# goalheart/ionic-mpnn

Hardware: AMD Instinct MI355X
Metric: molecule-graph pairs/sec (fwd), batch 4096 per MI355X (higher is better)
Workload: dtype f32 (bf16x9 emulation)

## Files before the change

### ionic_mpnn_amd/csrc/common.h

```cpp
#pragma once

#include <hip/hip_runtime.h>

#include <cstdarg>
#include <cstdint>
#include <cstdio>

#include "../../include/impnn.h"

namespace impnn {

char* error_buffer();
int fail(int code, const char* fmt, ...);

inline hipStream_t as_stream(impnn_stream_t s) { return reinterpret_cast<hipStream_t>(s); }

inline int check_launch(const char* what) {
  hipError_t e = hipGetLastError();
  if (e != hipSuccess) return fail(IMPNN_E_LAUNCH, "%s: %s", what, hipGetErrorString(e));
  return IMPNN_OK;
}

inline bool aligned16(const void* p) { return (reinterpret_cast<uintptr_t>(p) & 15u) == 0; }

// ... 92 lines not shown
struct GatedUpdateCall {
  const char* entry;
  GatedUpdateForm form;
  const float *h, *agg, *Wz, *bz, *Wr, *br, *Wh, *bh, *gamma;
  const float* beta;
  float eps;
  float* out;
  const float* dout;
  float *dh, *dagg, *dparams, *workspace;
  int64_t workspace_floats;
  bool accumulate;
  const int32_t *row_index, *n_rows;
  int64_t rows;
  int D;
  float* saved;
  bool dropout;
  DropoutArgs drop;
  hipStream_t stream;
};

template <class F>
int with_dropout_pack(const GatedUpdateCall& c, F&& f) {
  return c.dropout ? f(c.drop) : f();
}

constexpr int kMaxTypes = 4096;
struct TypedMessageCall {
  const char* entry;
  const float* h;
  const int32_t *bond_ids, *conn;
  const float* type_mats;
  float* messages;
  const float* grad;
  float *dh, *dtype_mats;
  float* edge_scratch;
  void* workspace;
  int64_t workspace_bytes;
  int B, N, E, D, Vb;
  bool sort_ready;
  bool zero_rows_ready;
  bool from_agg;
  hipStream_t stream;
};

struct EdgeSortView {
  int32_t *cnt, *start, *cursor, *segbase, *order;
  EdgeSortView(void* workspace, int Vb)
      : cnt(static_cast<int32_t*>(workspace)), start(cnt + Vb + 1), cursor(start + Vb + 1), segbase(cursor + Vb + 1),
        order(segbase + Vb + 1) {}
};

constexpr int kHeadMaxX = 128;
constexpr int kHeadMaxDim = 64;
inline int head_widths_covered(const char* what, int D, int F, int Mx) {
  if (D > kHeadMaxX || F > kHeadMaxDim || Mx > kHeadMaxDim)
    return fail(IMPNN_E_UNSUPPORTED, "%s: dims D=%d (<= %d) F=%d Mx=%d (<= %d)", what, D, kHeadMaxX, F, Mx, kHeadMaxDim);
  return IMPNN_OK;
}

struct ModelHeadCall {
  const char* entry;
  int kind;
  const float *pc, *pa, *T;
  const float* w;
  const float* const* weights;
  float* const* dweights;
  const float* dout;
  float *out, *dpc, *dpa;
  const float *l2, *y, *dloss;
  const float* sample_weight;
  float *loss, *workspace;
  int64_t workspace_floats;
  int B, D, F, Mx;
  hipStream_t stream;
};
int64_t model_head_loss_workspace_floats(int B);
int64_t model_head_bwd_max_floats();
int launch_model_head(const ModelHeadCall& c);
int launch_model_head_tensors(const ModelHeadCall& c);
int launch_model_head_bwd(const ModelHeadCall& c);

int launch_embed_gather(const int32_t* ids, const float* table, float* out, int64_t rows, int vocab,
                        int dim, hipStream_t s);
int launch_bmm_message(const float* h, const float* bs, const int32_t* conn, const float* W, float* m,
                       float* agg, int B, int N, int E, int D, int K, hipStream_t s);
int launch_bond_type_matrices(const float* tb, const float* W, float* out, int Vb, int K, int D,
                              hipStream_t s);
int launch_bmm_message_typed(const float* h, const int32_t* bond_ids, const int32_t* conn,
                             const float* type_mats, float* m, int B, int N, int E, int D, int Vb,
                             hipStream_t s);
int launch_reduce_scatter_add(const float* m, const int32_t* tgt, int tgt_stride, float* agg, int B,
                              int N, int E, int D, hipStream_t s, int accumulate = 0);
int launch_gated_update(const GatedUpdateCall& c);
int launch_kept_rows(const int32_t* atom_ids, const int32_t* bond_ids, const int32_t* conn, int32_t* rows_out, int B,
                     int N, int E, int Vb, hipStream_t s);
int launch_row_index_fill(const int32_t* r, const int32_t* incl, int32_t* idx, int32_t* count, int B, int N,
                          hipStream_t s);
int launch_global_sum_pool(const float* h, const int32_t* ids, float* out, int B, int N, int D,
                           hipStream_t s);
constexpr int kThTensors = 18;
struct TransferHeadCall {
  const float *pc, *pa;
  const float* const* weights;
  float* const* dweights;
  const float* l2;
  float *moving_mean, *moving_var;
  float bn_momentum, bn_eps;
  bool bn_batch;
  const float* y;
  const float* sample_weight;
  int loss_kind;
  float delta;
  const float* dloss;
  bool dropout;
  DropoutArgs drop;
  float* saved;
  float *out, *loss, *workspace;
  float *dpc, *dpa;
  int B, D, F, Mx;
  hipStream_t stream;
};
int64_t transfer_head_saved_floats(int B, int F, int Mx);
int64_t transfer_head_bwd_workspace_floats(int B, int F, int Mx);
int64_t transfer_head_loss_workspace_floats(int B);
int launch_transfer_head(const TransferHeadCall& c);
int launch_transfer_head_bwd(const TransferHeadCall& c);
int launch_gather_rows(int n, const void* const* src, void* const* dst, const int64_t* row_bytes, const int64_t* rows,
                       int n_rows, hipStream_t s);
int launch_validate_indices(const int32_t* conn, const int32_t* atom_ids, const int32_t* bond_ids,
                            int32_t* counts, int B, int N, int E, int Va, int Vb, hipStream_t s);

int launch_head_ion_mix(int kind, int ion, const float* pooled, const float* w, float* mix, int M, int D, int F, int Mx,
                        hipStream_t s);
int head_grid_max_temperatures();

struct GridOperands {
  int family, kind;
  const float *mix_cat, *mix_an, *T, *w;
  int C, A, nT, D, F, Mx;
  hipStream_t stream;
  int M;
  float kappa;
};
int launch_head_grid(const GridOperands& g, float* out, float* params);

int64_t transfer_grid_image_floats();
int launch_transfer_grid_prepare(const float* const* weights, const float* moving_mean, const float* moving_var,
                                 float bn_eps, float* image, hipStream_t s);
int launch_transfer_ion_half(int ion, const float* pooled, const float* const* weights, float* u, int M, int D, int F,
                             int Mx, hipStream_t s);
int launch_transfer_head_grid(const GridOperands& g, float* out);

constexpr int kSelectMaxK = 1024;
constexpr int kSelectMaxT = 4;
struct GridTopkCall {
  GridOperands g;
  int k, largest;
  float* values;
  int32_t *cation, *anion;
  void* workspace;
  int workgroups;
  bool masked;
  const uint32_t* where;
};
int grid_topk_workgroups(int family, int C, int A, int workgroups);
size_t grid_topk_workspace_bytes(int family, int C, int A, int nT, int k, int workgroups);
int launch_grid_topk(const GridTopkCall& c);
int launch_grid_topk_merge(const unsigned long long* ws, int G, int nT, int k, int largest, int A, float* values,
                           int32_t* cation, int32_t* anion, hipStream_t s);

struct GridMaskCall {
  GridOperands g;
  float lo, hi;
  uint32_t* words;
};
int64_t grid_mask_row_words(int A);
int launch_grid_mask(const GridMaskCall& c);

struct DomainGridCall {
  const float *mix_cat, *mix_an, *ref;
  float* distance;
  int32_t* nearest;
  uint32_t* words;
  float lo, hi;
  int C, A, R, Mx;
  hipStream_t stream;
};
struct DomainRowsCall {
  const float *z, *ref;
  bool exclude_self;
  float* distance;
  int32_t* nearest;
  int Q, R, Mx;
  hipStream_t stream;
};
int domain_reference_chunk();
int launch_domain_grid(const DomainGridCall& c);
int launch_domain_rows(const DomainRowsCall& c);

int ensemble_grid_max_members();
int ensemble_grid_max_temperatures(int kind, int M);
int ensemble_grid_topk_max_temperatures(int M);
int64_t ensemble_grid_tail_floats(int kind, int F, int Mx);
int launch_ensemble_grid(const GridOperands& g, float* mean, float* std, float* score);
int launch_ensemble_grid_mask(const GridMaskCall& c);
int launch_ensemble_grid_topk(const GridTopkCall& c);

constexpr int kPartnersMaxM = 8;
struct GridPartnersCall {
  GridOperands g;
  const uint32_t* where;
  int m, largest;
  float* cat_values;
  int32_t* cat_partner;
  float* an_values;
  int32_t* an_partner;
  void* workspace;
};
size_t grid_partners_workspace_bytes(int family, int C, int A, int nT, int m);
int launch_grid_partners(const GridPartnersCall& c);

constexpr int kRankDigitBits = 8;
constexpr int kRankBins = 1 << kRankDigitBits;
constexpr int64_t kRankMaxPairs = ((int64_t)1 << 32) - 2;
struct GridRankCall {
  GridOperands g;
  int64_t k;
  int largest;
  const uint32_t* where;
  float* values;
  int32_t *cation, *anion;
  int64_t* count;
  uint32_t* mask_words;
  void* workspace;
  int workgroups;
};
int grid_rank_passes(int64_t pairs);
int grid_rank_workgroups(int family, int C, int A, int workgroups);
size_t grid_rank_workspace_bytes(int family, int C, int A, int nT, int workgroups);
int launch_grid_rank(const GridRankCall& c);

int64_t bmm_message_typed_bwd_workspace_ints(int B, int E, int Vb);
int launch_bmm_message_typed_sorted(const TypedMessageCall& c);
int launch_bmm_message_typed_bwd(const TypedMessageCall& c);

int launch_embed_gather_bwd(const int32_t* ids, const float* dout, float* dtable, int64_t rows, int vocab, int dim,
                            hipStream_t s);
int launch_reduce_scatter_bwd(const float* dagg, const int32_t* tgt, int tgt_stride, float* dm, int B, int N, int E,
                              int D, hipStream_t s);
int launch_global_sum_pool_bwd(const float* dp, const int32_t* ids, float* dh, int B, int N, int D, hipStream_t s);
int launch_strided_gemm(const float* A, const float* B, float* out, int64_t rows, int M, int N, int64_t a_rs,
                        int64_t a_cs, int64_t b_rs, int64_t b_cs, hipStream_t s);
int launch_bond_type_matrices_multi(const float* tb, const float* const* W, float* const* out, int n, int Vb, int K,
                                    int D, hipStream_t s);
int launch_bond_type_matrices_multi_bwd(const float* tb, const float* const* W, const float* const* dA,
                                        float* const* dW, float* dtb, int n, int Vb, int K, int D, int accumulate,
                                        hipStream_t s, float* workspace = nullptr);
int64_t bond_type_matrices_multi_bwd_workspace(int n, int Vb, int K, int D);
int launch_bond_type_matrices_bwd(const float* tb, const float* W, const float* dA, float* dW, float* dtb, int Vb,
                                  int K, int D, int accumulate, hipStream_t s);
int gated_update_bwd_blocks(int64_t rows, int D);
int64_t gated_update_param_floats(int D);
int64_t gated_update_bwd_workspace(int64_t rows, int D, bool row_list = false);
int launch_gated_update_bwd(const GatedUpdateCall& c);
int launch_dropout_step(int64_t* counter, int64_t* snapshot, hipStream_t s);
int launch_dropout_mask(const DropoutArgs& d, const int32_t* ridx, const int32_t* nrows_dev, int64_t max_rows, int D,
                        float* out, hipStream_t s);
int launch_adam_clipnorm(const void* table, const void* sizes, int n_vars, int64_t step, int64_t* step_dev, float lr,
                         float b1, float b2, float eps, float clipnorm, hipStream_t s);

int launch_batch_assemble(int n_ions, const int32_t* sample_idx, int B, int M, const int32_t* const* atom_flat,
                          const int32_t* const* atom_off, const int32_t* const* edge_flat,
                          const int32_t* const* bond_flat, const int32_t* const* edge_off, int shift, int N, int L,
                          int32_t* const* atom_ids, int32_t* const* bond_ids, int32_t* const* conn,
                          const float* t_flat, float* t_out, hipStream_t s);

void profile_record_start(hipStream_t s);
void profile_record_stop(hipStream_t s);

void* debug_stamp_buffer(size_t* bytes);

struct EncoderArgs {
  int n_ions;
  const int32_t* atom_ids[2];
  const int32_t* bond_ids[2];
  const int32_t* conn[2];
  const float* weights[2];
  const void* prepared[2];
  int mode;
  int phases;
  int nwg;
  float* pooled[2];
  const float* atom_table;
  const float* bond_table;
  int Va, Vb, B, N, E, D, K, S;
  float ln_eps;
  void* workspace;
  size_t workspace_bytes;
};
bool encoder_fused_supported(int mode, int N, int E, int D, int K, int S, int Vb);
int encoder_workgroups(int n_ions, int B, int requested, int N, int E, int mode);
size_t encoder_fused_workspace_bytes(int mode, int n_ions, int B, int N, int E, int D, int S, int Vb, int nwg);
int launch_encoder_fused(const EncoderArgs& a, hipStream_t s);
int launch_encoder_phase(const EncoderArgs& a, hipStream_t s, bool plan_phase);
size_t encoder_prepared_bytes(int mode, int D, int S, int Vb);
int launch_encoder_prepare(const float* weights, const float* bond_table, int D, int K, int S, int Vb, int mode,
                           void* prepared, hipStream_t s);
size_t encoder_prepared_bytes_atoms(int mode, int D, int S, int Va, int Vb);
int launch_encoder_prepare_atoms(const float* weights, const float* bond_table, const float* atom_table, int Va, int D,
                                 int K, int S, int Vb, int mode, void* prepared, hipStream_t s);
int ensure_lds_limit(const void* kern, int slot);
int device_compute_units();
inline int gu_wide_tile_rows(int64_t rows) { return rows < 8192 ? 16 : 64; }
bool encoder_wide_supported(int N, int E, int D, int K, int S, int Vb);
size_t encoder_wide_workspace_bytes(int n_ions, int B, int N, int E, int D, int S, int Vb, bool x3);
bool encoder_wide_batch_covered(int n_ions, int B, int N, int E, int D, int Vb);
size_t encoder_wide_prepared_bytes(int D, int S, int Vb, bool x3);
int launch_encoder_wide_prepare(const float* weights, const float* bond_table, int D, int K, int S, int Vb, bool x3,
                                void* prepared, hipStream_t s);
int launch_encoder_wide(const EncoderArgs& a, hipStream_t s);

}
```

### ionic_mpnn_amd/csrc/encoder_fused.hip

```cpp
#include <atomic>
#include <cstdlib>

#include "encoder_device.h"
#include "encoder_layout.h"

namespace impnn {
namespace enc {

namespace {

struct H8 {
  half8 hi, lo;
};
__device__ __forceinline__ H8 split8(const float* v) {
  typedef __fp16 h2_t __attribute__((ext_vector_type(2)));
  union U {
    h2_t h;
    unsigned u;
  };
  union {
    half8 v8;
    unsigned u[4];
  } hi, lo;
#pragma unroll
// ... 111 lines not shown
    lds_barrier();
    if (!p.atab_lds || p.S == 0) {
      const int row = tid >> 2, sub = tid & 3;
      const int id = r_rowatom[row];
      f32x4 v0 = {0.f, 0.f, 0.f, 0.f}, v1 = v0;
      if ((unsigned)id < (unsigned)p.Va) {
        if (p.atab_lds) {
          v0 = ld4(atab + id * kHS + 8 * sub);
          v1 = ld4(atab + id * kHS + 8 * sub + 4);
        } else {
          v0 = ld4(p.atom_table + (int64_t)id * kD + 8 * sub);
          v1 = ld4(p.atom_table + (int64_t)id * kD + 8 * sub + 4);
        }
      }
      st4(hbuf + row * kHS + 8 * sub, v0);
      st4(hbuf + row * kHS + 8 * sub + 4, v1);
    }
    if (need_image) {
#pragma unroll
      for (int i = 0; i < kPf; ++i) st4(wimg + 4 * (tid + i * kThreads), pf[i]);
    }
    image_ready = p.S > 0;
    lds_barrier();
    if (stamp && tid == 0) {
      const unsigned long long t = __builtin_amdgcn_s_memtime();
      t_pro += t - t_mark;
      t_mark = t;
    }

    for (int s = 0; s < p.S; ++s) {
      const bool g0 = p.atab_lds && s == 0;
      const int src_shift = g0 ? 20 : 8;
      const int src_base = (g0 ? (int)(atab - smem) : (int)(hbuf - smem)) + 4 * q;
      const int sn = (s + 1) < p.S ? (s + 1) : 0;
      const float* nxt = img_g + (int64_t)sn * kImgSlot;
      bool pf_issued = false;

      int my_tile = -1;
      {
        const int grp = wave & 3, slot = wave >> 2, q4 = ntiles >> 2, r4 = ntiles & 3;
        const int heavy = (4 - r4) * q4;
        if (grp >= r4) {
          if (slot < q4) my_tile = slot * (4 - r4) + (grp - r4);
        } else if (slot <= q4) {
          my_tile = heavy + slot * r4 + grp;
        }
      }
      const bool has_tile = my_tile >= 0 && my_tile < ntiles;
      const int tile = has_tile ? my_tile : 0;
      const int row = tile * 16 + a;
      float G[kKMax][8];
      if (has_tile) {
        __builtin_amdgcn_s_setprio(3);

        const int p0 = r_rowptr[row];
        const int deg = r_rowptr[row + 1] - p0;
        const int maxdeg = __builtin_amdgcn_readfirstlane(r_tilemax[tile]);
        {
          const uint32_t ent = deg > 0 ? r_ent[p0] : 0u;
          const int bid = ent & 0xffu;
          const int soff = (int)(__builtin_amdgcn_ubfe(ent, src_shift, 12) * 4u) + src_base;
          const f32x4 x0 = ld4(smem + soff);
          const f32x4 x1 = ld4(smem + soff + 16);
          f32x4 c0 = ld4(tbl + bid * kKMax);
          f32x4 c1 = ld4(tbl + bid * kKMax + 4);
          if (deg <= 0) {
            c0 = f32x4{0.f, 0.f, 0.f, 0.f};
            c1 = c0;
          }
  #pragma unroll
          for (int k = 0; k < kKMax; ++k) {
            const float ck = k < 4 ? c0[k & 3] : c1[k & 3];
  #pragma unroll
            for (int i = 0; i < 4; ++i) {
              G[k][i] = ck * x0[i];
              G[k][4 + i] = ck * x1[i];
            }
          }
        }
        for (int d = 1; d < maxdeg; ++d) {
          if (d < deg) {
            const uint32_t ent = r_ent[p0 + d];
            const int bid = ent & 0xffu;
            const int soff = (int)(__builtin_amdgcn_ubfe(ent, src_shift, 12) * 4u) + src_base;
            const f32x4 x0 = ld4(smem + soff);
            const f32x4 x1 = ld4(smem + soff + 16);
            const f32x4 c0 = ld4(tbl + bid * kKMax);
            const f32x4 c1 = ld4(tbl + bid * kKMax + 4);
  #pragma unroll
            for (int k = 0; k < kKMax; ++k) {
              const float ck = k < 4 ? c0[k & 3] : c1[k & 3];
  #pragma unroll
              for (int i = 0; i < 4; ++i) {
                G[k][i] = fmaf(ck, x0[i], G[k][i]);
                G[k][4 + i] = fmaf(ck, x1[i], G[k][4 + i]);
              }
            }
          }
        }
        __builtin_amdgcn_s_setprio(2);
        if (!g0) lds_barrier();
        int own = row;
        if (g0) {
          const int id = r_rowatom[row];
          own = (unsigned)id < (unsigned)p.Va ? id : p.Va;
        }
        own = own * kHS + src_base;
        const f32x4 h0 = ld4(smem + own);
        const f32x4 h1 = ld4(smem + own + 16);

        f32x4 agg0 = {0.f, 0.f, 0.f, 0.f}, agg1 = {0.f, 0.f, 0.f, 0.f};
        if constexpr (SPLIT) {
  #pragma unroll
          for (int k = 0; k < kKMax; ++k) {
            if (k < K) {
              const H8 g = split8(G[k]);
              mma3(agg0, hmsg + (k * 2 + 0) * 1024, lane, g);
              mma3(agg1, hmsg + (k * 2 + 1) * 1024, lane, g);
            }
          }
          agg0 *= (kSX / kAcc);
          agg1 *= (kSX / kAcc);
        } else {
  #pragma unroll
          for (int k = 0; k < kKMax; ++k) {
            if (k < K) {
  #pragma unroll
              for (int u = 0; u < 2; ++u) {
                const f32x4 A0 = ld4(wmsg + (k * kD + a) * kMsgRS + 16 * u + 4 * q);
                const f32x4 A1 = ld4(wmsg + (k * kD + 16 + a) * kMsgRS + 16 * u + 4 * q);
  #pragma unroll
                for (int r = 0; r < 4; ++r) {
                  agg0 = mfma4(A0[r], G[k][4 * u + r], agg0);
                  agg1 = mfma4(A1[r], G[k][4 * u + r], agg1);
                }
              }
            }
          }
        }
        __builtin_amdgcn_s_setprio(1);
        if (!pf_issued) {
  #pragma unroll
          for (int i = 0; i < kPf; ++i) pf[i] = ld4(nxt + 4 * (tid + i * kThreads));
          pf_issued = true;
        }

        f32x4 z0 = ld4(wvec + 0 * kD + 4 * q), z1 = ld4(wvec + 0 * kD + 16 + 4 * q);
        f32x4 r0 = ld4(wvec + 1 * kD + 4 * q), r1 = ld4(wvec + 1 * kD + 16 + 4 * q);
        f32x4 t0 = ld4(wvec + 2 * kD + 4 * q), t1 = ld4(wvec + 2 * kD + 16 + 4 * q);
        f32x4 rh0, rh1;
        if constexpr (SPLIT) {
          const f32x4 hs0 = h0 * kSX, hs1 = h1 * kSX;
          const H8 sh = split8(hs0, hs1);
          const H8 sa = split8(agg0, agg1);
          mma3(z0, hupd + ((0 * 2 + 0) * 2 + 0) * 1024, lane, sh);
          mma3(z1, hupd + ((0 * 2 + 1) * 2 + 0) * 1024, lane, sh);
          mma3(r0, hupd + ((1 * 2 + 0) * 2 + 0) * 1024, lane, sh);
          mma3(r1, hupd + ((1 * 2 + 1) * 2 + 0) * 1024, lane, sh);
          mma3(z0, hupd + ((0 * 2 + 0) * 2 + 1) * 1024, lane, sa);
          mma3(z1, hupd + ((0 * 2 + 1) * 2 + 1) * 1024, lane, sa);
          mma3(r0, hupd + ((1 * 2 + 0) * 2 + 1) * 1024, lane, sa);
          mma3(r1, hupd + ((1 * 2 + 1) * 2 + 1) * 1024, lane, sa);
          z0 = sigmoid4<true>(z0);
          z1 = sigmoid4<true>(z1);
          const f32x4 rs0 = sigmoid4<true>(r0) * hs0, rs1 = sigmoid4<true>(r1) * hs1;
          const H8 srh = split8(rs0, rs1);
          mma3(t0, hupd + ((2 * 2 + 0) * 2 + 0) * 1024, lane, srh);
          mma3(t1, hupd + ((2 * 2 + 1) * 2 + 0) * 1024, lane, srh);
          mma3(t0, hupd + ((2 * 2 + 0) * 2 + 1) * 1024, lane, sa);
          mma3(t1, hupd + ((2 * 2 + 1) * 2 + 1) * 1024, lane, sa);
        } else {
  #pragma unroll
          for (int half = 0; half < 2; ++half) {
  #pragma unroll
            for (int u = 0; u < 2; ++u) {
              const int col = 32 * half + 16 * u + 4 * q;
              const f32x4 Az0 = ld4(wupd + (0 * kD + a) * kUpdRS + col);
              const f32x4 Az1 = ld4(wupd + (0 * kD + 16 + a) * kUpdRS + col);
              const f32x4 Ar0 = ld4(wupd + (1 * kD + a) * kUpdRS + col);
              const f32x4 Ar1 = ld4(wupd + (1 * kD + 16 + a) * kUpdRS + col);
              const f32x4 Bv = half == 0 ? (u == 0 ? h0 : h1) : (u == 0 ? agg0 : agg1);
  #pragma unroll
              for (int r = 0; r < 4; ++r) {
                z0 = mfma4(Az0[r], Bv[r], z0);
                z1 = mfma4(Az1[r], Bv[r], z1);
                r0 = mfma4(Ar0[r], Bv[r], r0);
                r1 = mfma4(Ar1[r], Bv[r], r1);
              }
            }
          }
          z0 = sigmoid4<false>(z0);
          z1 = sigmoid4<false>(z1);
          rh0 = sigmoid4<false>(r0) * h0;
          rh1 = sigmoid4<false>(r1) * h1;
  #pragma unroll
          for (int half = 0; half < 2; ++half) {
  #pragma unroll
            for (int u = 0; u < 2; ++u) {
              const int col = 32 * half + 16 * u + 4 * q;
              const f32x4 Ah0 = ld4(wupd + (2 * kD + a) * kUpdRS + col);
              const f32x4 Ah1 = ld4(wupd + (2 * kD + 16 + a) * kUpdRS + col);
              const f32x4 Bv = half == 0 ? (u == 0 ? rh0 : rh1) : (u == 0 ? agg0 : agg1);
  #pragma unroll
              for (int r = 0; r < 4; ++r) {
                t0 = mfma4(Ah0[r], Bv[r], t0);
                t1 = mfma4(Ah1[r], Bv[r], t1);
              }
            }
          }
        }
        __builtin_amdgcn_s_setprio(0);
        f32x4 n0 = z0 * (tanh4<SPLIT>(t0) - h0) + h0;
        f32x4 n1 = z1 * (tanh4<SPLIT>(t1) - h1) + h1;
        const f32x4 s4 = n0 + n1;
        float sum = (s4[0] + s4[1]) + (s4[2] + s4[3]);
        sum += __shfl_xor(sum, 16);
        sum += __shfl_xor(sum, 32);
        const float mean = sum * (1.0f / kD);
        n0 -= mean;
        n1 -= mean;
        const f32x4 q4 = n0 * n0 + n1 * n1;
        float var = (q4[0] + q4[1]) + (q4[2] + q4[3]);
        var += __shfl_xor(var, 16);
        var += __shfl_xor(var, 32);
        const float inv = __builtin_amdgcn_rsqf(var * (1.0f / kD) + p.ln_eps);
        const f32x4 g0 = ld4(wvec + 3 * kD + 4 * q), g1 = ld4(wvec + 3 * kD + 16 + 4 * q);
        const f32x4 b0 = ld4(wvec + 4 * kD + 4 * q), b1 = ld4(wvec + 4 * kD + 16 + 4 * q);
        const f32x4 o0 = n0 * (g0 * inv) + (b0 + h0);
        const f32x4 o1 = n1 * (g1 * inv) + (b1 + h1);
        st4(hbuf + row * kHS + 4 * q, o0);
        st4(hbuf + row * kHS + 16 + 4 * q, o1);

      }
      if (!pf_issued) {
        if (!g0) lds_barrier();
#pragma unroll
        for (int i = 0; i < kPf; ++i) pf[i] = ld4(nxt + 4 * (tid + i * kThreads));
      }
      const bool wstamp = stamp && c == c_begin && s == 1;
      if (wstamp && lane == 0) stamp[16 + wave] = __builtin_amdgcn_s_memtime();
      __syncthreads();
      if (wstamp && tid == 0) stamp[13] = __builtin_amdgcn_s_memtime();
#pragma unroll
      for (int i = 0; i < kPf; ++i) st4(wimg + 4 * (tid + i * kThreads), pf[i]);
      if (stamp && c == c_begin && s < 2 && tid == 0) stamp[14 + s] = __builtin_amdgcn_s_memtime();
    }
    if (stamp && tid == 0) {
      const unsigned long long t = __builtin_amdgcn_s_memtime();
      t_steps += t - t_mark;
      t_mark = t;
    }

    const float* hfin = hbuf;
    float* out_g = p.pooled[g];
    for (int t0 = 0; t0 < M * 64; t0 += kThreads) {
      const int t = t0 + tid;
      const int part = t & 7, f4 = (t >> 3) & 7, m = t >> 6;
      f32x4 acc = {0.f, 0.f, 0.f, 0.f};
      if (m < M) {
        const int nr = r_molrows[m], mo = r_moloff[m];
        for (int n = part; n < nr; n += 8) {
          const int pr = r_poolrow[mo + n];
          if (pr & 0x8000) acc += ld4(hfin + (pr & 0xff) * kHS + 4 * f4);
        }
      }
#pragma unroll
      for (int i = 0; i < 4; ++i) {
        float v = acc[i];
        v += __builtin_bit_cast(float, __builtin_amdgcn_update_dpp(0, __builtin_bit_cast(int, v), 0xb1, 0xf, 0xf, true));
        v += __builtin_bit_cast(float, __builtin_amdgcn_update_dpp(0, __builtin_bit_cast(int, v), 0x4e, 0xf, 0xf, true));
        v += __builtin_bit_cast(float, __builtin_amdgcn_update_dpp(0, __builtin_bit_cast(int, v), 0x141, 0xf, 0xf, true));
        acc[i] = v;
      }
      if (m < M && part == 0) st4(out_g + (int64_t)(m0 + m) * kD + 4 * f4, acc);
    }
    (void)N; (void)ids_g;
    lds_barrier();
    if (stamp && tid == 0) {
      const unsigned long long t = __builtin_amdgcn_s_memtime();
      t_pool += t - t_mark;
      t_mark = t;
    }
  }
  if (stamp && tid == 0) {
    stamp[1] = t_pro;
    stamp[2] = t_steps;
    stamp[3] = t_pool;
    stamp[4] = (unsigned long long)(c_end - c_begin);
    stamp[7] = __builtin_amdgcn_s_memtime();
  }
}

}

}

bool encoder_typed_supported(int N, int E, int D, int S, int Vb);
size_t encoder_typed_prepared_bytes(int S, int Vb, bool x3);
int launch_encoder_typed_prepare(const float* weights, const float* bond_table, int K, int S, int Vb, bool x3,
                                 void* prepared, hipStream_t s);
size_t encoder_typed_prepared_bytes_atoms(int S, int Va, int Vb, bool x3);
int launch_encoder_typed_prepare_atoms(const float* weights, const float* bond_table, const float* atom_table, int Va,
                                       int K, int S, int Vb, bool x3, void* prepared, hipStream_t s);
int launch_encoder_typed_run(const EncoderArgs& a, const enc::Ws& w, hipStream_t s);

bool encoder_fused_supported(int mode, int N, int E, int D, int K, int S, int Vb) {
  using namespace enc;
  if ((mode == 2 || mode == 3) && D != kD) return encoder_wide_supported(N, E, D, K, S, Vb);
  if (mode == 2 || mode == 3) return K >= 1 && encoder_typed_supported(N, E, D, S, Vb);
  if (mode != 0 && mode != 1) return false;
  if (D != kD || K < 1 || K > kKMax || S < 0) return false;
  if (N < 1 || N > 0xffff || E < 0) return false;
  if (Vb < 1 || Vb > 0xffff || (int64_t)Vb * kKMax > kTbCapFloats) return false;
  const int vrmax = vr_max_of(N, E);
  if (vrmax > kRCap / 2) return false;
  return true;
}

int device_compute_units() {
  static std::atomic<int> cache[64];
  int dev = 0;
  if (hipGetDevice(&dev) != hipSuccess || dev < 0 || dev >= 64) dev = 0;
  int n = cache[dev].load(std::memory_order_relaxed);
  if (n == 0) {
    if (hipDeviceGetAttribute(&n, hipDeviceAttributeMultiprocessorCount, dev) != hipSuccess || n <= 0) n = 256;
    n = n > 1024 ? 1024 : n;
    cache[dev].store(n, std::memory_order_relaxed);
  }
  return n;
}

int ensure_lds_limit(const void* kern, int slot) {
  static std::atomic<uint64_t> done[16];
  int dev = 0;
  if (hipGetDevice(&dev) != hipSuccess || dev < 0 || dev >= 64) dev = 0;
  const uint64_t bit = 1ull << dev;
  if (done[slot].load(std::memory_order_acquire) & bit) return IMPNN_OK;
  hipError_t e = hipFuncSetAttribute(kern, hipFuncAttributeMaxDynamicSharedMemorySize, 160 * 1024);
  if (e != hipSuccess) return fail(IMPNN_E_LAUNCH, "encoder: cannot raise LDS limit: %s", hipGetErrorString(e));
  done[slot].fetch_or(bit, std::memory_order_release);
  return IMPNN_OK;
}

int encoder_workgroups(int n_ions, int B, int requested, int N, int E, int mode) {
  int cus = device_compute_units();
  int want = requested;
  if (want <= 0) {
    static const int env_want = [] {
      const char* e = getenv("IMPNN_ENCODER_WORKGROUPS");
      return e ? atoi(e) : 0;
    }();
    want = env_want;
  }
  if (want > 0) cus = want < 16 ? 16 : (want > cus ? cus : want);
  int f = 1;
  while ((int64_t)2 * n_ions * B / ((int64_t)cus * f) + 64 > enc::kShareCap ||
         enc::ws_layout(n_ions, B, N, E, 1, 1, cus * f, mode >= 2, mode == 3).max_sub > enc::kMaxHops)
    ++f;
  return cus * f;
}

size_t encoder_fused_workspace_bytes(int mode, int n_ions, int B, int N, int E, int D, int S, int Vb, int nwg) {
  if (D != enc::kD) return encoder_wide_workspace_bytes(n_ions, B, N, E, D, S, Vb, mode == 3);
  return enc::ws_layout(n_ions, B, N, E, S, Vb, nwg, mode >= 2, mode == 3).total;
}

size_t encoder_prepared_bytes(int mode, int D, int S, int Vb) {
  if (D != enc::kD) return encoder_wide_prepared_bytes(D, S, Vb, mode == 3);
  if (mode >= 2) return encoder_typed_prepared_bytes(S, Vb, mode == 3);
  return (size_t)(S > 0 ? S : 1) * enc::kImgSlot * sizeof(float);
}

int launch_encoder_prepare(const float* weights, const float* bond_table, int D, int K, int S, int Vb, int mode,
                           void* prepared, hipStream_t s) {
  if (S <= 0) return IMPNN_OK;
  if (D != enc::kD) return launch_encoder_wide_prepare(weights, bond_table, D, K, S, Vb, mode == 3, prepared, s);
  if (mode >= 2) return launch_encoder_typed_prepare(weights, bond_table, K, S, Vb, mode == 3, prepared, s);
  enc::ImageParams ip{};
  ip.weights = weights;
  ip.img = static_cast<float*>(prepared);
  ip.K = K;
  ip.mode = mode == 1 ? 1 : 0;
  ip.step_floats = impnn_encoder_step_floats(D, K);
  return enc::launch_weight_image(ip, S, s);
}

size_t encoder_prepared_bytes_atoms(int mode, int D, int S, int Va, int Vb) {
  if (D == enc::kD && mode >= 2) return encoder_typed_prepared_bytes_atoms(S, Va, Vb, mode == 3);
  return encoder_prepared_bytes(mode, D, S, Vb);
}

int launch_encoder_prepare_atoms(const float* weights, const float* bond_table, const float* atom_table, int Va, int D,
                                 int K, int S, int Vb, int mode, void* prepared, hipStream_t s) {
  if (S > 0 && D == enc::kD && mode >= 2)
    return launch_encoder_typed_prepare_atoms(weights, bond_table, atom_table, Va, K, S, Vb, mode == 3, prepared, s);
  return launch_encoder_prepare(weights, bond_table, D, K, S, Vb, mode, prepared, s);
}

int launch_encoder_fused(const EncoderArgs& a, hipStream_t s) {
  if (a.D != enc::kD) return launch_encoder_wide(a, s);
  if (a.phases & 1)
    if (int rc = launch_encoder_phase(a, s, true)) return rc;
  if (a.phases & 2)
    if (int rc = launch_encoder_phase(a, s, false)) return rc;
  return IMPNN_OK;
}

int launch_encoder_phase(const EncoderArgs& a, hipStream_t s, bool plan_phase) {
  using namespace enc;
  const bool typed = a.mode >= 2;
  const Ws w = ws_layout(a.n_ions, a.B, a.N, a.E, a.S, a.Vb, a.nwg, typed, a.mode == 3);
  if (!aligned16(a.workspace)) return fail(IMPNN_E_BADARG, "encoder_fused: workspace must be 16B aligned");
  if (!plan_phase && !aligned16(a.atom_table)) return fail(IMPNN_E_BADARG, "encoder_fused: atom_table must be 16B aligned");
  char* base = static_cast<char*>(a.workspace);
  const int mode = a.mode == 1 ? 1 : 0;
  PlanParams pp{};
  EncParams ep{};
  for (int g = 0; g < a.n_ions; ++g) {
    if (plan_phase && (reinterpret_cast<uintptr_t>(a.conn[g]) & 7u) != 0)
      return fail(IMPNN_E_BADARG, "encoder_fused: connectivity must be 8B aligned");
    pp.atom_ids[g] = ep.atom_ids[g] = a.atom_ids[g];
    pp.bond_ids[g] = a.bond_ids[g];
    pp.conn[g] = a.conn[g];
    ep.pooled[g] = a.pooled[g];
    if (plan_phase || typed) continue;
    if (a.prepared[g]) {
      if (!aligned16(a.prepared[g])) return fail(IMPNN_E_BADARG, "encoder_fused: prepared weights must be 16B aligned");
      ep.img[g] = static_cast<const float*>(a.prepared[g]);
    } else {
      float* img = reinterpret_cast<float*>(base + w.img_off) + (size_t)g * (a.S > 0 ? a.S : 1) * kImgSlot;
      if (int rc = launch_encoder_prepare(a.weights[g], a.bond_table, a.D, a.K, a.S, a.Vb, mode, img, s)) return rc;
      ep.img[g] = img;
    }
  }
  pp.rows = reinterpret_cast<int32_t*>(base + w.rows_off);
  pp.vr = reinterpret_cast<int32_t*>(base + w.vr_off);
  pp.partial = reinterpret_cast<int32_t*>(base + w.partial_off);
  pp.nsub = reinterpret_cast<int32_t*>(base + w.nsub_off);
  pp.desc = reinterpret_cast<int32_t*>(base + w.desc_off);
  pp.rec = reinterpret_cast<unsigned char*>(base + w.rec_off);
  pp.slist = reinterpret_cast<uint32_t*>(base + w.slist_off);
  pp.header = reinterpret_cast<PlanHeader*>(base);
  pp.typed = typed ? 1 : 0;
  pp.ecap = tecap_of(a.E);
  pp.vmin = plan_vmin(a.n_ions, a.B, vr_max_of(a.N, a.E, typed), w.nwg);
  pp.n_ions = a.n_ions; pp.B = a.B; pp.N = a.N; pp.E = a.E; pp.Va = a.Va; pp.Vb = a.Vb;
  {
    const int per_cu = typed ? 4 : 5;
    pp.grid_sub = w.max_sub < per_cu ? w.max_sub : per_cu;
  }
  pp.nwg = w.nwg;
  pp.max_sub = w.max_sub;
  pp.nblk = w.nblk;
  pp.stamps = nullptr;
  {
    size_t sb = 0;
    void* sp = debug_stamp_buffer(&sb);
    if (sp && sb >= ((size_t)w.nwg * 32 + 16) * sizeof(unsigned long long))
      pp.stamps = static_cast<unsigned long long*>(sp) + (size_t)w.nwg * 32;
  }
  if (plan_phase) return launch_plan(pp, s);
  if (typed) return launch_encoder_typed_run(a, w, s);

  ep.atom_table = a.atom_table;
  ep.bond_table = a.bond_table;
  ep.nsub = pp.nsub; ep.desc = pp.desc; ep.rec = pp.rec; ep.max_sub = w.max_sub;
  ep.header = pp.header;
  ep.n_ions = a.n_ions; ep.B = a.B; ep.N = a.N; ep.K = a.K; ep.S = a.S;
  ep.Va = a.Va; ep.Vb = a.Vb; ep.ln_eps = a.ln_eps;
  ep.stamps = nullptr;
  {
    size_t sb = 0;
    void* sp = debug_stamp_buffer(&sb);
    if (sp && sb >= (size_t)w.nwg * 32 * sizeof(unsigned long long)) ep.stamps = static_cast<unsigned long long*>(sp);
  }
  const int variant = (a.K == 8 ? 1 : 0) + 2 * mode;
  void (*kern)(EncParams) = variant == 0   ? encoder_fused_kernel<0, false>
                            : variant == 1 ? encoder_fused_kernel<8, false>
                            : variant == 2 ? encoder_fused_kernel<0, true>
                                           : encoder_fused_kernel<8, true>;
  if (int rc = ensure_lds_limit((const void*)kern, variant)) return rc;
  profile_record_start(s);
  size_t lds = kLdsFixedBytes + align_up((size_t)a.Vb * kKMax * sizeof(float), 512);
  const size_t atab_bytes = ((size_t)a.Va + 1) * kHS * sizeof(float);
  ep.atab_lds = a.Va <= kEntMaxAtom && lds + atab_bytes <= 156 * 1024;
  if (ep.atab_lds) lds += atab_bytes;
  kern<<<w.nwg, kThreads, lds, s>>>(ep);
  profile_record_stop(s);
  return check_launch("encoder_fused");
}

}
```

### ionic_mpnn_amd/csrc/encoder_layout.h

```cpp
#pragma once

#include "common.h"

namespace impnn {
namespace enc {

typedef float f32x4 __attribute__((ext_vector_type(4)));
typedef _Float16 half8 __attribute__((ext_vector_type(8)));

constexpr float kSW = 256.0f;
constexpr float kSX = 16.0f;
constexpr float kAcc = kSW * kSX;

constexpr int kD = 32;
constexpr int kKMax = 8;
constexpr int kRCap = 256;
constexpr int kECap = 1024;
constexpr int kHS = 36;
constexpr int kMsgRS = 36;
constexpr int kUpdRS = 68;
constexpr int kThreads = 1024;
constexpr int kWaves = kThreads / 64;
constexpr int kTbCapFloats = 2048;

__host__ __device__ constexpr int img_msg_floats(int K) { return K * kD * kMsgRS; }
__host__ __device__ constexpr int img_upd_floats() { return 3 * kD * kUpdRS; }
__host__ __device__ constexpr int img_vec_floats() { return 5 * kD; }
__host__ __device__ constexpr int img_floats(int K) {
  return img_msg_floats(K) + img_upd_floats() + img_vec_floats();
}
__host__ __device__ constexpr int img16_msg_halfs(int K) { return K * 2 * 2 * 512; }
__host__ __device__ constexpr int img16_upd_halfs() { return 3 * 2 * 2 * 2 * 512; }
__host__ __device__ constexpr int img16_vec_float_off(int K) { return (img16_msg_halfs(K) + img16_upd_halfs()) / 2; }
__host__ __device__ constexpr int feat_of(int q, int j) { return 16 * (j >> 2) + 4 * q + (j & 3); }
constexpr int kPf = 4;
constexpr int kImgSlot = kPf * kThreads * 4;
static_assert(kThreads == 4 * kRCap, "prologue maps 4 threads to a row");
static_assert(img_floats(kKMax) <= kImgSlot, "weight image does not fit its slot");
static_assert(img16_vec_float_off(kKMax) + img_vec_floats() <= kImgSlot, "split weight image does not fit");

constexpr int kRecRowptr = 0;
constexpr int kRecTilemax = 528;
constexpr int kRecMoloff = 544;
constexpr int kRecMolrows = 1072;
constexpr int kRecPoolrow = 1584;
constexpr int kRecRowatom = 2096;
constexpr int kEntMaxAtom = 454;
constexpr int kRecEnt = 3136;
constexpr int kRecBytes = 8192;
static_assert(kRecEnt + 4 * kECap <= kRecBytes && kRecEnt % 16 == 0, "record layout");

constexpr int kTECap = 512;
constexpr int kTECapBig = 640;
__host__ __device__ constexpr int tecap_of(int E) { return E > kTECap ? kTECapBig : kTECap; }
constexpr int kTVbMax = 256;
constexpr int kTHS = 36;
constexpr int kTAS = 32;
constexpr int kTRecRowdeg = 0;
constexpr int kTRecTilemax = 528;
constexpr int kTRecMoloff = 544;
constexpr int kTRecMolrows = 1072;
constexpr int kTRecPoolrow = 1584;
constexpr int kTRecRowatom = 2096;
constexpr int kTRecCounts = 3120;
constexpr int kTRecJdptr = 3136;
constexpr int kTRecNrun = 3664;
constexpr int kTRecGrp = 3712;
constexpr int kTRunTarget = 32;
__host__ __device__ constexpr int tgrp_cap(int Vb, int ecap) { return ecap / 4 + (Vb < kTVbMax ? Vb : kTVbMax); }
__host__ __device__ constexpr int trec_runs_off(int Vb, int ecap) { return kTRecGrp + 16 * tgrp_cap(Vb, ecap); }
__host__ __device__ constexpr int trec_used_bytes(int Vb, int ecap) {
  return (trec_runs_off(Vb, ecap) + 2 * (Vb + 2 + kTRunTarget) + 15) & ~15;
}
constexpr int kTRecBytes = 12288;
constexpr int kTRecPart1 = 8192;
__host__ __device__ constexpr int trec_lds_bytes(int Vb, int ecap) { return trec_used_bytes(Vb, ecap); }
static_assert(kTRecGrp % 16 == 0 && trec_used_bytes(kTVbMax, kTECapBig) <= kTRecBytes, "typed record layout");
__host__ __device__ constexpr int tmsg_floats(int ecap) { return (ecap + 2) * kD; }
__host__ __device__ constexpr int tmsg_off(int s, int u) { return s * kD + ((u ^ ((s >> 1) & 7)) << 2); }
__host__ __device__ constexpr int tmsg_key(int s) { return s * kD + (((s >> 1) & 7) << 2); }
static_assert(tmsg_key(kTECapBig + 1) < 65536, "message keys travel as 16 bits");
constexpr uint32_t kSrcIdNone = 0xffffffu;
__host__ __device__ constexpr uint32_t tsrc_word(int type, int atom_id) {
  return ((uint32_t)type << 24) | ((uint32_t)atom_id < kSrcIdNone ? (uint32_t)atom_id : kSrcIdNone);
}
static_assert(kTECap % 8 == 0 && kTECapBig % 8 == 0, "the encoder moves step-0 messages in granules of 8 slots");
constexpr int kTUpdBlocks = 24;
constexpr int kTVecFloatOff = kTUpdBlocks * 256;
constexpr int kTUpdFloats = kTVecFloatOff + 5 * kD;
constexpr int kTUpdSlot = 2 * kThreads * 4;
constexpr int kTUpdLds = 6400;
static_assert(kTUpdFloats <= kTUpdLds && kTUpdLds <= kTUpdSlot, "typed update image");
constexpr int kXUpdHalfs = 3 * 2 * 2 * 3 * 512;
constexpr int kXVecFloatOff = kXUpdHalfs / 2;
constexpr int kXUpdFloats = kXVecFloatOff + 5 * kD;
constexpr int kXUpdSlot = 3 * kThreads * 4;
constexpr int kXUpdLds = 9472;
static_assert(kXUpdFloats <= kXUpdLds && kXUpdLds <= kXUpdSlot, "x3 update image");
constexpr int kTMatFloats = kD * kD;
inline size_t typed_prepared_floats(int S, int Vb, bool x3 = false) {
  const size_t s = S > 0 ? S : 1;
  return s * (x3 ? kXUpdSlot : kTUpdSlot) + s * (size_t)Vb * kTMatFloats + (size_t)Vb * kTMatFloats;
}

constexpr int32_t kM0Magic = 0x6d30746d;
constexpr size_t kM0CapBytes = (size_t)2 << 20;
struct M0Header {
  int32_t magic, Va, Vb, S;
};
inline size_t m0_table_floats(int S, int Va, int Vb) {
  if (S < 1 || Va < 1 || Vb < 1) return 0;
  const size_t n = (size_t)Vb * ((size_t)Va + 1) * kD;
  return n * sizeof(float) <= kM0CapBytes ? n : 0;
}

constexpr int kShareCap = kECap;
inline int plan_vmin(int n_ions, int B, int vrmax, int nwg) {
  const int64_t span = 2 * (int64_t)n_ions * B * vrmax / (nwg > 0 ? nwg : 1) + vrmax;
  const int64_t v = (span + kShareCap - 2) / (kShareCap - 1);
  return (int)(v < 1 ? 1 : (v > kRCap ? kRCap : v));
}
constexpr int kMaxHops = 128;

constexpr int kPB = 16;

struct Ws {
  size_t img_off, rows_off, vr_off, partial_off, share_off, nsub_off, desc_off, rec_off, slist_off, total;
  int nwg;
  int max_sub;
  int nblk;
  int rec_bytes;
};

inline size_t align_up(size_t x, size_t a) { return (x + a - 1) / a * a; }

__host__ __device__ constexpr int tvr_of_edges(int edges, int ecap) { return (edges * kRCap + ecap - 1) / ecap; }

inline int vr_max_of(int N, int E, bool typed = false) {
  int v = typed ? (E > 4 * kTECapBig ? kRCap + 1 : tvr_of_edges(E, tecap_of(E))) : (E + 3) / 4;
  int m = N > v ? N : v;
  m = m < 1 ? 1 : m;
  return typed && m > kRCap ? kRCap : m;
}

struct PlanHeader {
  int32_t magic, kind, n_ions, B, N, E, nwg, max_sub;
  int32_t overflow;
};
constexpr int32_t kPlanMagic = 0x696d706e;
constexpr int32_t kPlanBadBit = 1 << 30;

inline Ws ws_layout(int n_ions, int B, int N, int E, int S, int Vb, int nwg, bool typed, bool x3 = false) {
  Ws w{};
  const int vrmax = vr_max_of(N, E, typed);
  w.rec_bytes = typed ? kTRecBytes : kRecBytes;
  const int win = kRCap - vrmax + 1;
  w.nwg = nwg;
  w.nblk = (B + kPB - 1) / kPB;
  const int64_t share_rows = (2 * (int64_t)n_ions * B * vrmax) / nwg + vrmax;
  const int64_t by_win = win >= 1 ? share_rows / win + 2 : (int64_t)1 << 40;
  const int64_t by_pairs = 2 * share_rows / (kRCap + 1) + 2;
  w.max_sub = (int)(by_win < by_pairs ? by_win : by_pairs);
  size_t off = 256;
  w.img_off = off;
  off = align_up(off + (typed ? (size_t)n_ions * typed_prepared_floats(S, Vb, x3)
                              : (size_t)n_ions * (S > 0 ? S : 1) * kImgSlot) * sizeof(float), 256);
  w.rows_off = off;
  off = align_up(off + (size_t)n_ions * B * sizeof(int32_t), 256);
  w.vr_off = off;
  off = align_up(off + (size_t)n_ions * B * sizeof(int32_t), 256);
  w.partial_off = off;
  off = align_up(off + (size_t)n_ions * w.nblk * sizeof(int32_t), 256);
  w.share_off = off;
  off = align_up(off + (size_t)nwg * 4 * sizeof(int32_t), 256);
  w.nsub_off = off;
  off = align_up(off + (size_t)nwg * sizeof(int32_t), 256);
  w.desc_off = off;
  off = align_up(off + (size_t)nwg * w.max_sub * 4 * sizeof(int32_t), 256);
  w.rec_off = off;
  off = align_up(off + (size_t)nwg * w.max_sub * w.rec_bytes, 256);
  w.slist_off = off;
  if (typed) off = align_up(off + (size_t)nwg * w.max_sub * tecap_of(E) * sizeof(uint32_t), 256);
  w.total = off;
  return w;
}

struct PlanParams {
  const int32_t* atom_ids[2];
  const int32_t* bond_ids[2];
  const int32_t* conn[2];
  int32_t* rows;
  int32_t* vr;
  int32_t* partial;
  int32_t* nsub;
  int32_t* desc;
  unsigned char* rec;
  uint32_t* slist;
  int n_ions, B, N, E, Va, Vb, nwg, max_sub, nblk;
  int grid_sub;
  int typed;
  int ecap;
  int vmin;
  PlanHeader* header;
  unsigned long long* stamps;
};

struct ImageParams {
  const float* weights;
  float* img;
  int K, mode;
  int64_t step_floats;
};

struct EncParams {
  const int32_t* atom_ids[2];
  float* pooled[2];
  const float* atom_table;
  const float* bond_table;
  const float* img[2];
  const int32_t* nsub;
  const int32_t* desc;
  const unsigned char* rec;
  const PlanHeader* header;
  int n_ions, B, N, K, S, Va, Vb, max_sub;
  int atab_lds;
  float ln_eps;
  unsigned long long* stamps;
};

struct TImageParams {
  const float* weights;
  const float* bond_table;
  float* prepared;
  int K, S, Vb, x3;
  int64_t step_floats;
};

struct TEncParams {
  float* pooled[2];
  const float* atom_table;
  const float* upd[2];
  const float* tmat[2];
  const float* m0[2];
  const int32_t* nsub;
  const int32_t* desc;
  const unsigned char* rec;
  const uint32_t* slist;
  const PlanHeader* header;
  int n_ions, B, S, Va, Vb, max_sub;
  int atab_lds;
  int upd_slot;
  int rec_lds;
  int ecap;
  float ln_eps;
  unsigned long long* stamps;
};

__device__ __forceinline__ void lds_barrier() {
  asm volatile("s_waitcnt lgkmcnt(0)\n\ts_barrier" ::: "memory");
}

__device__ __forceinline__ int wave_incl_scan(int v) {
  v += __builtin_amdgcn_update_dpp(0, v, 0x111, 0xf, 0xf, true);
  v += __builtin_amdgcn_update_dpp(0, v, 0x112, 0xf, 0xf, true);
  v += __builtin_amdgcn_update_dpp(0, v, 0x114, 0xf, 0xf, true);
  v += __builtin_amdgcn_update_dpp(0, v, 0x118, 0xf, 0xf, true);
  v += __builtin_amdgcn_update_dpp(0, v, 0x142, 0xa, 0xf, true);
  v += __builtin_amdgcn_update_dpp(0, v, 0x143, 0xc, 0xf, true);
  return v;
}

__device__ __forceinline__ bool edge_valid(int s, int t, int bid, int N, int Vb) {
  return (unsigned)s - 1u < (unsigned)(N - 1) && (unsigned)t - 1u < (unsigned)(N - 1) && (unsigned)bid < (unsigned)Vb;
}

int launch_weight_image(const ImageParams& ip, int S, hipStream_t s);
int launch_plan(const PlanParams& pp, hipStream_t s);
int launch_typed_image(const TImageParams& ip, hipStream_t s);

}
}
```

### ionic_mpnn_amd/csrc/encoder_plan.hip

```cpp
#include "encoder_layout.h"

namespace impnn {
namespace enc {

namespace {

__global__ __launch_bounds__(64 * kPB) void plan_stats_kernel(PlanParams p) {
  __shared__ int vsum[kPB], vbad[kPB];
  __builtin_amdgcn_s_setprio(3);
  const int lane = threadIdx.x & 63, wv = threadIdx.x >> 6;
  const int g = blockIdx.x / p.nblk, blk = blockIdx.x - g * p.nblk;
  const int b = blk * kPB + wv;
  const bool have = b < p.B;
  const int64_t item = (int64_t)g * p.B + (have ? b : 0);
  int my_vr = 0, my_bad = 0;
  if (have) {
  const int32_t* ids = p.atom_ids[g] + (int64_t)b * p.N;
  const int32_t* cn = p.conn[g] + (int64_t)b * p.E * 2;
  const int32_t* bd = p.bond_ids[g] + (int64_t)b * p.E;
  int rmax = 0, cnt = 0;
  const int id_first = lane < p.N ? ids[lane] : 0;
  int emax = 0;
  for (int e0 = 0; e0 < p.E; e0 += 256) {
    int2 st[4];
    int bid[4];
#pragma unroll
    for (int u = 0; u < 4; ++u) {
      const int e = e0 + 64 * u + lane;
      st[u] = make_int2(0, 0);
      bid[u] = -1;
      if (e < p.E) {
        st[u] = *reinterpret_cast<const int2*>(cn + 2 * e);
        bid[u] = bd[e];
      }
    }
#pragma unroll
    for (int u = 0; u < 4; ++u) {
      const bool ok = edge_valid(st[u].x, st[u].y, bid[u], p.N, p.Vb);
      if (ok) {
        const int m = st[u].x > st[u].y ? st[u].x : st[u].y;
        emax = emax > m ? emax : m;
      }
      cnt += __builtin_popcountll(__ballot(ok));
    }
  }
  {
    const unsigned long long hit = __ballot(id_first > 0);
    if (hit) rmax = 64 - __builtin_clzll(hit);
  }
  for (int n0 = 64; n0 < p.N; n0 += 64) {
    const int n = n0 + lane;
    const unsigned long long hit = __ballot(n < p.N && ids[n] > 0);
    if (hit) rmax = n0 + 64 - __builtin_clzll(hit);
  }
  if (cnt > 0) {
    bool alive = true;
    int res = 0;
#pragma unroll
    for (int bit = 15; bit >= 0; --bit) {
      const bool one = alive && ((emax >> bit) & 1);
      if (__ballot(one)) {
        res |= 1 << bit;
        alive = one;
      }
    }
    rmax = rmax > res + 1 ? rmax : res + 1;
  }
  {
    int vr = p.typed ? tvr_of_edges(cnt < 0x100000 ? cnt : 0x100000, p.ecap) : (cnt + 3) >> 2;
    vr = vr > rmax ? vr : rmax;
    my_vr = vr < p.vmin ? p.vmin : vr;
    if (my_vr > kRCap) {
      my_vr = kRCap;
      my_bad = 1;
    }
    if (lane == 0) {
      p.rows[item] = rmax;
      p.vr[item] = my_vr;
    }
  }
  }
  if (lane == 0) {
    vsum[wv] = my_vr;
    vbad[wv] = my_bad;
  }
  lds_barrier();
  if (threadIdx.x == 0) {
    int t = 0, bad = 0;
#pragma unroll
    for (int i = 0; i < kPB; ++i) {
      t += vsum[i];
      bad |= vbad[i];
    }
    p.partial[(int64_t)g * p.nblk + blk] = t | (bad ? kPlanBadBit : 0);
    if (blockIdx.x == 0) {
      PlanHeader h;
      h.magic = kPlanMagic; h.kind = p.typed; h.n_ions = p.n_ions; h.B = p.B; h.N = p.N; h.E = p.E;
      h.nwg = p.nwg; h.max_sub = p.max_sub;
      h.overflow = 0;
      *p.header = h;
    }
  }
}


__global__ void weight_image_kernel(ImageParams p) {
  {
    const int s = blockIdx.y;
    const int t_begin = blockIdx.x * blockDim.x + threadIdx.x, t_stride = gridDim.x * blockDim.x;
    const float* w = p.weights + (int64_t)s * p.step_floats;
    const int K = p.K;
    const float* W = w;
    const float* Wz = W + (int64_t)K * kD * kD;
    const float* bz = Wz + 2 * kD * kD;
    const float* Wr = bz + kD;
    const float* br = Wr + 2 * kD * kD;
    const float* Wh = br + kD;
    const float* bh = Wh + 2 * kD * kD;
    const float* gamma = bh + kD;
    const float* beta = gamma + kD;
    float* img = p.img + (int64_t)s * kImgSlot;
    if (p.mode == 1) {
      _Float16* hi_lo = reinterpret_cast<_Float16*>(img);
      const int nm = img16_msg_halfs(K), nu = img16_upd_halfs();
      for (int t = t_begin; t < nm + nu; t += t_stride) {
        const int j = t & 7, ln = (t >> 3) & 63, part = (t >> 9) & 1;
        const int q = ln >> 4, i = ln & 15, f = feat_of(q, j);
        float wv;
        if (t < nm) {
          const int blk = t >> 10;
          const int k = blk >> 1, T = blk & 1;
          wv = W[((int64_t)k * kD + 16 * T + i) * kD + f];
        } else {
          const int blk = (t - nm) >> 10;
          const int half = blk & 1, T = (blk >> 1) & 1, gate = blk >> 2;
          const float* Wg = gate == 0 ? Wz : (gate == 1 ? Wr : Wh);
          wv = Wg[(int64_t)(half * kD + f) * kD + 16 * T + i];
        }
        wv *= kSW;
        const _Float16 hi = __builtin_amdgcn_cvt_pkrtz(wv, 0.f)[0];
        const _Float16 lo = __builtin_amdgcn_cvt_pkrtz(wv - (float)hi, 0.f)[0];
        hi_lo[t] = part == 0 ? hi : lo;
      }
      float* vec = img + img16_vec_float_off(K);
      for (int t = t_begin; t < img_vec_floats(); t += t_stride) {
        const int v = t / kD, i = t - v * kD;
        const float* src = v == 0 ? bz : v == 1 ? br : v == 2 ? bh : v == 3 ? gamma : beta;
        vec[t] = v < 3 ? src[i] * kAcc : src[i];
      }
      for (int t = img16_vec_float_off(K) + img_vec_floats() + t_begin; t < kImgSlot; t += t_stride) img[t] = 0.f;
      return;
    }
    const int nmsg = img_msg_floats(K), nupd = img_upd_floats();
    for (int t = t_begin; t < nmsg; t += t_stride) {
      const int row = t / kMsgRS, j = t - row * kMsgRS;
      img[t] = j < kD ? W[(int64_t)row * kD + j] : 0.f;
    }
    for (int t = t_begin; t < nupd; t += t_stride) {
      const int row = t / kUpdRS, jj = t - row * kUpdRS;
      const int gate = row / kD, io = row - gate * kD;
      const float* Wg = gate == 0 ? Wz : (gate == 1 ? Wr : Wh);
      img[nmsg + t] = jj < 2 * kD ? Wg[(int64_t)jj * kD + io] : 0.f;
    }
    for (int t = t_begin; t < img_vec_floats(); t += t_stride) {
      const int v = t / kD, i = t - v * kD;
      const float* src = v == 0 ? bz : v == 1 ? br : v == 2 ? bh : v == 3 ? gamma : beta;
      img[nmsg + nupd + t] = src[i];
    }
    for (int t = img_floats(K) + t_begin; t < kImgSlot; t += t_stride) img[t] = 0.f;
  }
}


__global__ void typed_image_kernel(TImageParams p, int s) {
  const int t_begin = blockIdx.x * blockDim.x + threadIdx.x, t_stride = gridDim.x * blockDim.x;
  const int S = p.S > 0 ? p.S : 1;
  const size_t uslot = p.x3 ? kXUpdSlot : kTUpdSlot;
  float* upd = p.prepared + (size_t)s * uslot;
  float* tmat = p.prepared + (size_t)S * uslot + (size_t)s * p.Vb * kTMatFloats;
  const float* canon = p.prepared + (size_t)S * uslot + (size_t)S * p.Vb * kTMatFloats;
  const float* w = p.weights + (int64_t)s * p.step_floats;
  const float* Wz = w + (int64_t)p.K * kD * kD;
  const float* bz = Wz + 2 * kD * kD;
  const float* Wr = bz + kD;
  const float* br = Wr + 2 * kD * kD;
  const float* Wh = br + kD;
  const float* bh = Wh + 2 * kD * kD;
  const float* gamma = bh + kD;
  const float* beta = gamma + kD;
  const int nmat = p.Vb * kTMatFloats;
  for (int t = t_begin; t < nmat; t += t_stride) {
    const int v = t >> 10, rem = t & 1023, kq = rem >> 7, r = (rem >> 2) & 31, c = rem & 3;
    tmat[t] = canon[(size_t)v * kTMatFloats + r * kD + 4 * kq + c];
  }
  if (p.x3) {
    unsigned short* planes = reinterpret_cast<unsigned short*>(upd);
    for (int t = t_begin; t < kXUpdHalfs / 3; t += t_stride) {
      const int j = t & 7, ln = (t >> 3) & 63, blk = t >> 9;
      const int q = ln >> 4, i = ln & 15, f = feat_of(q, j);
      const int half = blk & 1, T = (blk >> 1) & 1, gate = blk >> 2;
      const float* Wg = gate == 0 ? Wz : (gate == 1 ? Wr : Wh);
      const float wv = Wg[(int64_t)(half * kD + f) * kD + 16 * T + i];
      const unsigned u0 = __float_as_uint(wv) & 0xffff0000u;
      const float r1 = wv - __uint_as_float(u0);
      const unsigned u1 = __float_as_uint(r1) & 0xffff0000u;
      const float r2 = r1 - __uint_as_float(u1);
      const unsigned u2 = __float_as_uint(r2);
      const int base = (blk * 3) * 512 + ln * 8 + j;
      planes[base] = (unsigned short)(u0 >> 16);
      planes[base + 512] = (unsigned short)(u1 >> 16);
      planes[base + 1024] = (unsigned short)(u2 >> 16);
    }
    for (int t = t_begin; t < kXUpdSlot - kXVecFloatOff; t += t_stride) {
      float val = 0.f;
      if (t < 5 * kD) {
        const int v = t / kD, i = t - v * kD;
        const float* src = v == 0 ? bz : v == 1 ? br : v == 2 ? bh : v == 3 ? gamma : beta;
        val = src[i];
      }
      upd[kXVecFloatOff + t] = val;
    }
    return;
  }
  for (int t = t_begin; t < kTUpdSlot; t += t_stride) {
    float val = 0.f;
    if (t < kTVecFloatOff) {
      const int r = t & 3, ln = (t >> 2) & 63, blk = t >> 8;
      const int a = ln & 15, q = ln >> 4;
      const int u = blk & 1, half = (blk >> 1) & 1, T = (blk >> 2) & 1, gate = blk >> 3;
      const float* Wg = gate == 0 ? Wz : (gate == 1 ? Wr : Wh);
      val = Wg[(int64_t)(32 * half + 16 * u + 4 * q + r) * kD + 16 * T + a];
    } else if (t < kTVecFloatOff + 5 * kD) {
      const int v = (t - kTVecFloatOff) / kD, i = (t - kTVecFloatOff) - v * kD;
      const float* src = v == 0 ? bz : v == 1 ? br : v == 2 ? bh : v == 3 ? gamma : beta;
      val = src[i];
    }
    upd[t] = val;
  }
}

__device__ __forceinline__ int xcd_slot(int j, int nwg) {
#ifdef IMPNN_DIAG_NO_XCD_MAP
  return j;
#else
  const int lo = (nwg >> 3) * 4 + ((nwg & 7) < 4 ? (nwg & 7) : 4);
  const int r = j & 7, qd = j >> 3;
  return r < 4 ? qd * 4 + r : lo + qd * 4 + (r - 4);
#endif
}

__device__ __forceinline__ int share_bound(int tg, int jj, int nwg_g) {
  if (jj <= 0) return 0;
  if (jj >= nwg_g) return tg;
  const int t = (int)((float)tg * (float)jj * __frcp_rn((float)nwg_g));
  return t < 0 ? 0 : (t > tg ? tg : t);
}
__device__ __forceinline__ int ion_split(long long t0, long long t1, int nwg) {
  int n0 = (t0 + t1) > 0 ? (int)((float)nwg * (float)t0 * __frcp_rn((float)(t0 + t1)) + 0.5f) : nwg / 2;
  if (nwg >= 2) n0 = n0 < 1 ? 1 : (n0 > nwg - 1 ? nwg - 1 : n0);
  return n0;
}

#define CSTAMP(i) do { if (p.stamps && blockIdx.x == 0 && threadIdx.x == 0) p.stamps[i] = __builtin_amdgcn_s_memtime(); } while (0)
__device__ __forceinline__ bool resolve_share(const PlanParams& p, int j, int lane, int& g, int& k0, int& bp0,
                                              int& t_lo, int& t_hi, bool& bad) {
  const int nblk = p.nblk;
  bad = false;
  constexpr int kPU = 4;
  const int npass = (nblk + 64 * kPU - 1) / (64 * kPU);
  if (npass == 1) {
    int v[2][kPU];
    int anybad = 0;
#pragma unroll
    for (int gi = 0; gi < 2; ++gi)
#pragma unroll
      for (int i = 0; i < kPU; ++i) {
        const int k = kPU * lane + i;
        const int kk = k < nblk ? k : nblk - 1;
        const int x = gi < p.n_ions ? p.partial[(int64_t)gi * nblk + kk] : 0;
        anybad |= k < nblk ? x : 0;
        v[gi][i] = k < nblk ? (x & ~kPlanBadBit) : 0;
      }
    if (__ballot((anybad & kPlanBadBit) != 0)) bad = true;
    if (bad) return false;
    CSTAMP(10);
    int ex[2], tot[2];
#pragma unroll
    for (int gi = 0; gi < 2; ++gi) {
      const int s4 = v[gi][0] + v[gi][1] + v[gi][2] + v[gi][3];
      const int incl = wave_incl_scan(s4);
      ex[gi] = incl - s4;
      tot[gi] = __builtin_amdgcn_readlane(incl, 63);
    }
    int nwg0 = p.nwg, nwg1 = 0;
    if (p.n_ions == 2) {
      int n0 = ion_split(tot[0], tot[1], p.nwg);
      nwg0 = n0;
      nwg1 = p.nwg - n0;
    }
    const int jp = xcd_slot(j, p.nwg);
    g = jp < nwg0 ? 0 : 1;
    const int jj = jp - (g ? nwg0 : 0);
    const int nwg_g = g ? nwg1 : nwg0;
    const int tg = tot[g];
    t_lo = share_bound(tg, jj, nwg_g);
    t_hi = share_bound(tg, jj + 1, nwg_g);
    k0 = 0;
    bp0 = 0;
    if (t_hi <= t_lo) return false;
    const int e0 = g ? ex[1] : ex[0];
    const int a0 = g ? v[1][0] : v[0][0], a1 = g ? v[1][1] : v[0][1], a2 = g ? v[1][2] : v[0][2], a3 = g ? v[1][3] : v[0][3];
    const unsigned long long hit = __ballot(e0 <= t_lo && t_lo < e0 + a0 + a1 + a2 + a3);
    if (hit == 0ull) return false;
    const int src = __builtin_ctzll(hit);
    const int i_in = t_lo < e0 + a0 ? 0 : (t_lo < e0 + a0 + a1 ? 1 : (t_lo < e0 + a0 + a1 + a2 ? 2 : 3));
    const int st_in = e0 + (i_in > 0 ? a0 : 0) + (i_in > 1 ? a1 : 0) + (i_in > 2 ? a2 : 0);
    k0 = kPU * src + __builtin_amdgcn_readlane(i_in, src);
    bp0 = __builtin_amdgcn_readlane(st_in, src);
    return true;
  }
  long long tot[2] = {0, 0};
  for (int gi = 0; gi < p.n_ions; ++gi) {
    const int32_t* part = p.partial + (int64_t)gi * nblk;
    int acc = 0, anybad = 0;
    for (int k = lane; k < nblk; k += 64) {
      const int x = part[k];
      anybad |= x & kPlanBadBit;
      acc += x & ~kPlanBadBit;
    }
    if (__ballot(anybad != 0)) bad = true;
    tot[gi] = wave_incl_scan(acc);
    tot[gi] = __builtin_amdgcn_readlane((int)tot[gi], 63);
  }
  if (bad) return false;
  int nwg0 = p.nwg, nwg1 = 0;
  if (p.n_ions == 2) {
    int n0 = ion_split(tot[0], tot[1], p.nwg);
    nwg0 = n0;
    nwg1 = p.nwg - n0;
  }
  const int jp = xcd_slot(j, p.nwg);
  g = jp < nwg0 ? 0 : 1;
  const int jj = jp - (g ? nwg0 : 0);
  const int nwg_g = g ? nwg1 : nwg0;
  const int tg = (int)tot[g];
  t_lo = share_bound(tg, jj, nwg_g);
  t_hi = share_bound(tg, jj + 1, nwg_g);
  k0 = 0;
  bp0 = 0;
  if (t_hi <= t_lo) return false;
  const int32_t* part = p.partial + (int64_t)g * nblk;
  int carry = 0;
  bool found = false;
  for (int kbase = 0; kbase < nblk && !found; kbase += 64) {
    const int k = kbase + lane;
    const int v = k < nblk ? (part[k < nblk ? k : nblk - 1] & ~kPlanBadBit) : 0;
    const int incl = wave_incl_scan(v);
    const int st = carry + incl - v;
    const unsigned long long hit = __ballot(k < nblk && st <= t_lo && t_lo < st + v);
    if (hit) {
      const int src = __builtin_ctzll(hit);
      k0 = kbase + src;
      bp0 = __builtin_amdgcn_readlane(st, src);
      found = true;
    }
    carry += __builtin_amdgcn_readlane(incl, 63);
  }
  return found;
}

constexpr int kDegBins = 18;

struct ShareTab {
  int32_t shst[kShareCap + 1];
  int32_t cb[kMaxHops + 1];
  int32_t vwin[256];
  int chunk_s[3];
};

__device__ __forceinline__ int fast_div(int x, int d, float rd) {
  int q = (int)((float)x * rd);
  if (q * d > x) --q;
  if ((q + 1) * d <= x) ++q;
  return q;
}

__device__ __forceinline__ void resolve_chain(const PlanParams& p, int j, int slot_i, int lane, ShareTab& T) {
  int gg = 0, w_lo = 0;
  {
    const int half = p.n_ions == 2 ? (p.nwg >> 1 > 0 ? p.nwg >> 1 : 1) : p.nwg;
    const int jp = xcd_slot(j, p.nwg);
    gg = (p.n_ions == 2 && jp >= half) ? 1 : 0;
    const int jj = jp - (gg ? half : 0);
    const int nw = gg ? (p.nwg - half > 0 ? p.nwg - half : 1) : half;
    w_lo = (int)((float)jj * (float)p.B / (float)nw) - 64;
    w_lo = w_lo < 0 ? 0 : w_lo;
    w_lo &= ~15;
  }
  int vw[4];
  {
    const int32_t* vrg = p.vr + (int64_t)gg * p.B;
#pragma unroll
    for (int i = 0; i < 4; ++i) {
      const int m = w_lo + 64 * i + lane;
      vw[i] = vrg[m < p.B ? m : p.B - 1];
    }
  }
  int g = 0, k0 = 0, bp0 = 0, t_lo = 0, t_hi = 0;
  bool bad = false;
  const bool have = resolve_share(p, j, lane, g, k0, bp0, t_lo, t_hi, bad);
  CSTAMP(11);
#pragma unroll
  for (int i = 0; i < 4; ++i) T.vwin[64 * i + lane] = vw[i];
  if (!have) {
    if (lane == 0) {
      T.chunk_s[0] = -1; T.chunk_s[1] = 0; T.chunk_s[2] = 0;
      if (slot_i == 0) p.nsub[j] = 0;
      if (bad && blockIdx.x == 0) p.header->overflow = 1;
    }
    return;
  }
  const int32_t* vrg = p.vr + (int64_t)g * p.B;
  int run = bp0;
  int first = -1, nsh = 0;
  int end_row = -1;
  __builtin_amdgcn_s_waitcnt(0xc07f);
  auto vr_at = [&](int mbase) {
    const int rel = mbase - w_lo;
    if (g == gg && rel >= 0 && rel + 64 <= 256) return T.vwin[rel + lane];
    const int m = mbase + lane;
    return vrg[m < p.B ? m : p.B - 1];
  };
  int v_n1 = vr_at(k0 * kPB);
  for (int mbase = k0 * kPB; mbase < p.B && end_row < 0; mbase += 64) {
    const int m = mbase + lane;
    const int v = v_n1;
    v_n1 = vr_at(mbase + 64);
    const int vv = m < p.B ? v : 0;
    const int incl = wave_incl_scan(vv);
    const int st = run + incl - vv;
    const bool in = m < p.B && st >= t_lo && st < t_hi;
    const unsigned long long inb = __ballot(in);
    if (inb) {
      if (first < 0) first = mbase + __builtin_ctzll(inb);
      const int pos = nsh + __builtin_popcountll(inb & ((1ull << lane) - 1));
      if (in && pos < kShareCap) T.shst[pos] = st;
      nsh += __builtin_popcountll(inb);
    }
    const unsigned long long ge = __ballot(m < p.B && st >= t_hi);
    if (ge) end_row = __builtin_amdgcn_readlane(st, __builtin_ctzll(ge));
    run += __builtin_amdgcn_readlane(incl, 63);
  }
  if (end_row < 0) end_row = run;
  if (nsh > kShareCap) {
    if (lane == 0) p.header->overflow = 1;
    nsh = kShareCap;
  }
  if (lane == 0) T.shst[nsh] = end_row;
  __builtin_amdgcn_s_waitcnt(0xc07f);
  CSTAMP(12);
  int mb = 0, hop = 0;
  if (nsh < 64) {
    const int st_l = T.shst[lane <= nsh ? lane : nsh];
    while (mb < nsh && hop < kMaxHops) {
      const int lim = __builtin_amdgcn_readlane(st_l, mb) + kRCap;
      const unsigned long long okb = __ballot(lane > mb && lane <= nsh && st_l <= lim);
      if (lane == 0) T.cb[hop] = mb;
      ++hop;
      mb = okb ? 63 - __builtin_clzll(okb) : mb + 1;
    }
  }
  while (mb < nsh && hop < kMaxHops) {
    const int lim = T.shst[mb] + kRCap;
    int e = mb + 1;
    for (int c0 = mb + 1; c0 <= nsh; c0 += 64) {
      const int cidx = c0 + lane;
      const bool ok = cidx <= nsh && T.shst[cidx <= nsh ? cidx : nsh] <= lim;
      const unsigned long long okb = __ballot(ok);
      if (okb == 0) break;
      e = c0 + 63 - __builtin_clzll(okb);
      if (okb != ~0ull) break;
    }
    if (lane == 0) T.cb[hop] = mb;
    ++hop;
    mb = e;
  }
  if (lane == 0) {
    T.cb[hop] = nsh;
    T.chunk_s[0] = first;
    T.chunk_s[1] = hop;
    T.chunk_s[2] = g;
    if (slot_i == 0) p.nsub[j] = hop;
  }
}


__global__ __launch_bounds__(kRCap, 5) void plan_chunks_kernel(PlanParams p) {
  __shared__ int32_t moloff[kRCap + 2], molrows[kRCap], cnt[kRCap], place[kRCap], cursor[kRCap], rowptr[kRCap + 2];
  __shared__ int32_t bins[48], tilemax[16], scratch[8];
  __shared__ uint16_t atomof[kRCap];
  __shared__ uint32_t ent2[kECap + 1];
  __shared__ ShareTab T;
  __builtin_amdgcn_s_setprio(3);
  CSTAMP(0);
  const int j = blockIdx.x / p.grid_sub, slot_i = blockIdx.x - j * p.grid_sub;
  const int tid = threadIdx.x, lane = tid & 63, wave = tid >> 6;
  if (wave == 0) resolve_chain(p, j, slot_i, lane, T);
  lds_barrier();
  CSTAMP(1);
  const int first_mol = T.chunk_s[0], nhop = T.chunk_s[1], g = T.chunk_s[2];
  for (int sl = slot_i; sl < nhop; sl += p.grid_sub) {
  const int mb_local = T.cb[sl], M = T.cb[sl + 1] - mb_local, m0 = first_mol + mb_local;
  const int R = T.shst[mb_local + M] - T.shst[mb_local];
  const int idx = j * p.max_sub + sl;
  if (tid == 0) reinterpret_cast<int4*>(p.desc)[idx] = make_int4(m0, M, 0, R | (g << 16));
  const int N = p.N, E = p.E;
  const int32_t* ids_g = p.atom_ids[g];
  const int32_t* conn_g = p.conn[g];
  const int32_t* bond_g = p.bond_ids[g];
  const int32_t* rows_g = p.rows + (int64_t)g * p.B;
  unsigned char* rec = p.rec + (size_t)idx * kRecBytes;
  uint16_t* r_rowptr = reinterpret_cast<uint16_t*>(rec + kRecRowptr);
  unsigned char* r_tilemax = rec + kRecTilemax;
  uint16_t* r_moloff = reinterpret_cast<uint16_t*>(rec + kRecMoloff);
  uint16_t* r_molrows = reinterpret_cast<uint16_t*>(rec + kRecMolrows);
  uint16_t* r_poolrow = reinterpret_cast<uint16_t*>(rec + kRecPoolrow);
  int32_t* r_rowatom = reinterpret_cast<int32_t*>(rec + kRecRowatom);
  uint32_t* r_ent = reinterpret_cast<uint32_t*>(rec + kRecEnt);

  const int n_slots = M * E;
  constexpr int kSC = 4;
  int sm[kSC], se[kSC], sbid[kSC];
  int2 sst[kSC];
#pragma unroll
  for (int k = 0; k < kSC; ++k) {
    const int slot = tid + k * kRCap;
    sm[k] = 0; se[k] = 0; sbid[k] = -1; sst[k] = make_int2(0, 0);
    if (slot < n_slots) {
      sm[k] = slot / E;
      se[k] = slot - sm[k] * E;
      const int64_t b = m0 + sm[k];
      sst[k] = *reinterpret_cast<const int2*>(conn_g + (b * E + se[k]) * 2);
      sbid[k] = bond_g[b * E + se[k]];
    }
  }
  for (int m = tid; m <= M; m += kRCap) {
    const int off = T.shst[mb_local + m] - T.shst[mb_local];
    moloff[m] = off;
    r_moloff[m] = (uint16_t)off;
    if (m < M) {
      const int rr = rows_g[m0 + m];
      molrows[m] = rr;
      r_molrows[m] = (uint16_t)rr;
    }
  }
  cnt[tid] = 0;
  if (tid < 48) bins[tid] = 0;
  if (tid < 16) tilemax[tid] = 0;
  lds_barrier();
  CSTAMP(2);

#pragma unroll
  for (int k = 0; k < kSC; ++k)
    if (edge_valid(sst[k].x, sst[k].y, sbid[k], N, p.Vb)) atomicAdd(&cnt[moloff[sm[k]] + sst[k].y], 1);
  for (int slot = tid + kSC * kRCap; slot < n_slots; slot += kRCap) {
    const int m = slot / E, e = slot - m * E;
    const int64_t b = m0 + m;
    const int2 st = *reinterpret_cast<const int2*>(conn_g + (b * E + e) * 2);
    if (edge_valid(st.x, st.y, bond_g[b * E + e], N, p.Vb)) atomicAdd(&cnt[moloff[m] + st.y], 1);
  }
  int my_id = -1;
  bool my_real = false;
  if (tid < R) {
    int lo = 0, hi = M - 1;
    while (lo < hi) {
      const int mid = (lo + hi + 1) >> 1;
      if (moloff[mid] <= tid) lo = mid; else hi = mid - 1;
    }
    const int n = tid - moloff[lo];
    if (n < molrows[lo]) {
      my_real = true;
      my_id = ids_g[(int64_t)(m0 + lo) * N + n];
    }
  }
  lds_barrier();
  CSTAMP(3);

  const int my_deg = cnt[tid];
  int pos;
  {
    const int my_bin = tid >= R ? 0 : (my_deg >= 16 ? 1 : 17 - my_deg);
    atomicAdd(&bins[my_bin], 1);
    lds_barrier();
    CSTAMP(4);
    if (wave == 0) {
      const int bidx = lane < kDegBins ? (lane == kDegBins - 1 ? 0 : lane + 1) : 0;
      const int v = lane < kDegBins ? bins[bidx] : 0;
      int incl = v;
#pragma unroll
      for (int o = 1; o < 32; o <<= 1) {
        int t = __shfl_up(incl, o);
        if (lane >= o) incl += t;
      }
      if (lane < kDegBins) bins[24 + bidx] = incl - v;
    }
    lds_barrier();
    CSTAMP(5);
    pos = bins[24 + my_bin] + atomicAdd(&bins[my_bin], -1) - 1;
  }
  lds_barrier();
  place[tid] = pos;
  cursor[pos] = my_deg;
  if (my_deg > 0) atomicMax(&tilemax[pos >> 4], my_deg > 255 ? 255 : my_deg);
  r_rowatom[pos] = my_real ? my_id : -1;
  atomof[pos] = (uint16_t)((my_real && (unsigned)my_id < (unsigned)p.Va) ? my_id : p.Va);
  r_poolrow[tid] = (uint16_t)(pos | ((my_real && my_id > 0) ? 0x8000 : 0));
  lds_barrier();
  CSTAMP(6);

  {
    const int my_cnt = cursor[tid];
    int incl = my_cnt;
#pragma unroll
    for (int o = 1; o < 64; o <<= 1) {
      int t = __shfl_up(incl, o);
      if (lane >= o) incl += t;
    }
    if (lane == 63) scratch[wave] = incl;
    lds_barrier();
  CSTAMP(7);
    int off = 0;
    for (int w = 0; w < wave; ++w) off += scratch[w];
    const int excl = off + incl - my_cnt;
    rowptr[tid] = excl;
    cursor[tid] = excl;
    r_rowptr[tid] = (uint16_t)excl;
    if (tid == kRCap - 1) {
      rowptr[kRCap] = excl + my_cnt;
      r_rowptr[kRCap] = (uint16_t)(excl + my_cnt);
    }
    if (tid < 16) r_tilemax[tid] = (unsigned char)tilemax[tid];
  }
  lds_barrier();
  CSTAMP(8);

#pragma unroll
  for (int k = 0; k < kSC; ++k)
    if (edge_valid(sst[k].x, sst[k].y, sbid[k], N, p.Vb)) {
      const int mo = moloff[sm[k]];
      const int at = atomicAdd(&cursor[place[mo + sst[k].y]], 1);
      ent2[at] = ((uint32_t)se[k] << 16) | ((uint32_t)sbid[k] << 8) | (uint32_t)place[mo + sst[k].x];
    }
  for (int slot = tid + kSC * kRCap; slot < n_slots; slot += kRCap) {
    const int m = slot / E, e = slot - m * E;
    const int64_t b = m0 + m;
    const int2 st = *reinterpret_cast<const int2*>(conn_g + (b * E + e) * 2);
    const int bid = bond_g[b * E + e];
    if (edge_valid(st.x, st.y, bid, N, p.Vb)) {
      const int mo = moloff[m];
      const int at = atomicAdd(&cursor[place[mo + st.y]], 1);
      ent2[at] = ((uint32_t)e << 16) | ((uint32_t)bid << 8) | (uint32_t)place[mo + st.x];
    }
  }
  lds_barrier();
  CSTAMP(9);

  {
    const int total = rowptr[kRCap];
    for (int i = tid; i < total; i += kRCap) {
      int lo = 0, hi = kRCap - 1;
      while (lo < hi) {
        const int mid = (lo + hi + 1) >> 1;
        if (rowptr[mid] <= i) lo = mid; else hi = mid - 1;
      }
      const int b0 = rowptr[lo], b1 = rowptr[lo + 1];
      const uint32_t v = ent2[i];
      int rank = 0;
      for (int jx = b0; jx < b1; ++jx) rank += ent2[jx] < v;
      const uint32_t srow = v & 0xffu, bid = (v >> 8) & 0xffu;
      const uint32_t aid = atomof[srow] < kEntMaxAtom ? atomof[srow] : kEntMaxAtom;
      r_ent[b0 + rank] = ((aid * (kHS / 4)) << 20) | ((srow * (kHS / 4)) << 8) | bid;
    }
  }
  CSTAMP(15);
  lds_barrier();
  }
}

constexpr int kTick = 16;
__global__ __launch_bounds__(kRCap, 4) void plan_chunks_typed_kernel(PlanParams p) {
  __shared__ int32_t moloff[kRCap + 2], molrows[kRCap], cnt[kRCap + 64], place[kRCap];
  __shared__ int32_t idl[kRCap];
  __shared__ __attribute__((aligned(16))) int32_t dbins[kRCap], dstart[kRCap], dcur[kRCap];
  __shared__ __attribute__((aligned(16))) int32_t thist[kTVbMax + 64], tgb[kTVbMax], tcur[kTVbMax + 64];
  __shared__ __attribute__((aligned(16))) int32_t jdp[kRCap + 4];
  __shared__ int32_t misc[4];
  __shared__ __attribute__((aligned(16))) uint16_t tick[kRCap * kTick];
  __shared__ uint2 elist[kTECapBig];
  extern __shared__ uint4 grp[];
  __shared__ ShareTab T;
  __builtin_amdgcn_s_setprio(3);
  CSTAMP(0);
  const int j = blockIdx.x / p.grid_sub, slot_i = blockIdx.x - j * p.grid_sub;
  const int tid = threadIdx.x, lane = tid & 63, wave = tid >> 6;
  if (wave == ((blockIdx.x >> 8) & 3)) resolve_chain(p, j, slot_i, lane, T);
  lds_barrier();
  CSTAMP(1);
  const int first_mol = T.chunk_s[0], nhop = T.chunk_s[1], g = T.chunk_s[2];
  const int N = p.N, E = p.E;
  const float rE = 1.0f / (float)E;
  for (int sl = slot_i; sl < nhop; sl += p.grid_sub) {
  const int mb_local = T.cb[sl], M = T.cb[sl + 1] - mb_local, m0 = first_mol + mb_local;
  const int base = T.shst[mb_local];
  const int R = T.shst[mb_local + M] - base;
  const int idx = j * p.max_sub + sl;
  const int32_t* ids_g = p.atom_ids[g];
  const int32_t* conn_g = p.conn[g];
  const int32_t* bond_g = p.bond_ids[g];
  const int32_t* rows_g = p.rows + (int64_t)g * p.B;
  unsigned char* rec = p.rec + (size_t)idx * kTRecBytes;
  uint32_t* r_slist = p.slist + (size_t)idx * p.ecap;
  uint16_t* r_rowdeg = reinterpret_cast<uint16_t*>(rec + kTRecRowdeg);
  unsigned char* r_tilemax = rec + kTRecTilemax;
  uint16_t* r_moloff = reinterpret_cast<uint16_t*>(rec + kTRecMoloff);
  uint16_t* r_molrows = reinterpret_cast<uint16_t*>(rec + kTRecMolrows);
  uint16_t* r_poolrow = reinterpret_cast<uint16_t*>(rec + kTRecPoolrow);
  int32_t* r_rowatom = reinterpret_cast<int32_t*>(rec + kTRecRowatom);
  uint16_t* r_jd = reinterpret_cast<uint16_t*>(rec + kTRecJdptr);
  uint16_t* r_cw = reinterpret_cast<uint16_t*>(rec + kTRecCounts);

  const int n_slots = M * E;
  constexpr int kSC = 6;
  int sbid[kSC];
  int2 sst[kSC];
  const int32_t* conn_c = conn_g + (int64_t)m0 * E * 2;
  const int32_t* bond_c = bond_g + (int64_t)m0 * E;
#pragma unroll
  for (int k = 0; k < kSC; ++k) {
    const int slot = tid + k * kRCap;
    sbid[k] = -1; sst[k] = make_int2(0, 0);
    if (slot < n_slots) {
      sst[k] = *reinterpret_cast<const int2*>(conn_c + 2 * (int64_t)slot);
      sbid[k] = bond_c[slot];
    }
  }
  constexpr int kIC = 3;
  const int n_ids = M * N;
  const float rN = 1.0f / (float)N;
  const int32_t* ids_c = ids_g + (int64_t)m0 * N;
  int sid[kIC];
#pragma unroll
  for (int k = 0; k < kIC; ++k) {
    const int slot = tid + k * kRCap;
    sid[k] = slot < n_ids ? ids_c[slot] : 0;
  }
  for (int m = tid; m <= M; m += kRCap) {
    const int off = T.shst[mb_local + m] - base;
    moloff[m] = off;
    r_moloff[m] = (uint16_t)off;
    if (m < M) {
      const int rr = rows_g[m0 + m];
      molrows[m] = rr;
      r_molrows[m] = (uint16_t)rr;
    }
  }
  cnt[tid] = 0;
  dbins[tid] = 0;
  dcur[tid] = 0;
  thist[tid] = 0;
  tcur[tid] = 0;
  idl[tid] = -1;
  if (tid == 0) misc[1] = 0;
  {
    const uint4 ones = make_uint4(~0u, ~0u, ~0u, ~0u);
    reinterpret_cast<uint4*>(tick)[2 * tid] = ones;
    reinterpret_cast<uint4*>(tick)[2 * tid + 1] = ones;
  }
  lds_barrier();
  CSTAMP(2);

  auto put_id = [&](int slot, int id) {
    const int m = fast_div(slot, N, rN), n = slot - m * N;
    if (slot < n_ids && n < molrows[m]) idl[moloff[m] + n] = id;
  };
  {
    const int dq = fast_div(kRCap, N, rN), dr = kRCap - dq * N;
    int cm = fast_div(tid, N, rN), cn = tid - cm * N;
    int mr[kIC], mo[kIC], nn[kIC];
#pragma unroll
    for (int k = 0; k < kIC; ++k) {
      const int mm = tid + k * kRCap < n_ids ? cm : 0;
      mr[k] = tid + k * kRCap < n_ids ? molrows[mm] : 0;
      mo[k] = moloff[mm];
      nn[k] = cn;
      cn += dr; cm += dq;
      if (cn >= N) { cn -= N; ++cm; }
    }
#pragma unroll
    for (int k = 0; k < kIC; ++k)
      if (nn[k] < mr[k]) idl[mo[k] + nn[k]] = sid[k];
  }
  for (int slot = tid + kIC * kRCap; slot < n_ids; slot += kRCap) put_id(slot, ids_c[slot]);
  {
    unsigned okm = 0u;
#pragma unroll
    for (int k = 0; k < kSC; ++k) okm |= edge_valid(sst[k].x, sst[k].y, sbid[k], N, p.Vb) ? 1u << k : 0u;
    const int mine = __builtin_popcount(okm);
    const int incl = wave_incl_scan(mine);
    int pos = 0;
    if (lane == 63) pos = atomicAdd(&misc[1], incl);
    pos = __builtin_amdgcn_readlane(pos, 63) + incl - mine;
    const int dq = fast_div(kRCap, E, rE), dr = kRCap - dq * E;
    int cm = fast_div(tid, E, rE), ce = tid - cm * E;
#pragma unroll
    for (int k0 = 0; k0 < kSC; k0 += 3) {
      int row[3], srw[3], tk[3], es[3];
#pragma unroll
      for (int k = 0; k < 3; ++k) {
        const bool ok = (okm >> (k0 + k)) & 1u;
        const int m = cm;
        es[k] = ce;
        ce += dr; cm += dq;
        if (ce >= E) { ce -= E; ++cm; }
        const int mo = moloff[m < M ? m : 0];
        row[k] = mo + (ok ? sst[k0 + k].y : 0);
        srw[k] = mo + (ok ? sst[k0 + k].x : 0);
      }
#pragma unroll
      for (int k = 0; k < 3; ++k) {
        const bool ok = (okm >> (k0 + k)) & 1u;
        tk[k] = atomicAdd(&cnt[ok ? row[k] : kRCap + lane], 1);
        atomicAdd(&thist[ok ? sbid[k0 + k] : kTVbMax + lane], 1);
      }
#pragma unroll
      for (int k = 0; k < 3; ++k) {
        const bool ok = (okm >> (k0 + k)) & 1u;
        if (ok && tk[k] < kTick) tick[row[k] * kTick + tk[k]] = (uint16_t)es[k];
        if (ok) {
          if (pos < kTECapBig)
            elist[pos] = make_uint2((uint32_t)row[k] | ((uint32_t)srw[k] << 8) | ((uint32_t)sbid[k0 + k] << 16), (uint32_t)es[k]);
          ++pos;
        }
      }
    }
  }
  for (int s0 = kSC * kRCap; s0 < n_slots; s0 += kRCap) {
    const int slot = s0 + tid;
    int2 st = make_int2(0, 0);
    int bid = -1;
    if (slot < n_slots) {
      st = *reinterpret_cast<const int2*>(conn_c + 2 * (int64_t)slot);
      bid = bond_c[slot];
    }
    const bool ok = edge_valid(st.x, st.y, bid, N, p.Vb);
    const int m = fast_div(slot, E, rE), e = slot - m * E;
    const int mo = moloff[m < M ? m : 0];
    const int row = mo + (ok ? st.y : 0);
    int tk = kTick;
    if (ok) {
      tk = atomicAdd(&cnt[row], 1);
      atomicAdd(&thist[bid], 1);
    }
    const unsigned long long okb = __ballot(ok);
    int pos0 = 0;
    if (okb != 0ull) {
      if (lane == (int)__builtin_ctzll(okb)) pos0 = atomicAdd(&misc[1], (int)__builtin_popcountll(okb));
      pos0 = __builtin_amdgcn_readlane(pos0, (int)__builtin_ctzll(okb));
    }
    if (tk < kTick) tick[row * kTick + tk] = (uint16_t)e;
    const int pos = pos0 + (int)__builtin_popcountll(okb & ((1ull << lane) - 1));
    if (ok && pos < kTECapBig)
      elist[pos] = make_uint2((uint32_t)row | ((uint32_t)(mo + st.x) << 8) | ((uint32_t)bid << 16), (uint32_t)e);
  }
  lds_barrier();
  CSTAMP(3);

  const int my_deg = cnt[tid];
  const int dcl = my_deg > 255 ? 255 : my_deg;
  if (tid < R) {
    if (my_deg > 255) p.header->overflow = 1;
    atomicAdd(&dbins[255 - dcl], 1);
  }
  lds_barrier();
  CSTAMP(4);

  if (wave == 0) {
    const int4 h = reinterpret_cast<const int4*>(dbins)[lane];
    const int s4 = h.x + h.y + h.z + h.w;
    const int ex = wave_incl_scan(s4) - s4;
    reinterpret_cast<int4*>(dstart)[lane] = make_int4(ex, ex + h.x, ex + h.x + h.y, ex + h.x + h.y + h.z);
    __builtin_amdgcn_s_waitcnt(0xc07f);
    const int4 s = reinterpret_cast<const int4*>(dstart)[63 - lane];
    const int t4 = s.x + s.y + s.z + s.w;
    const int incl = wave_incl_scan(t4);
    const int jx = incl - t4;
    reinterpret_cast<int4*>(jdp)[lane] = make_int4(jx, jx + s.w, jx + s.w + s.z, jx + s.w + s.z + s.y);
    if (lane == 63) { jdp[kRCap] = incl; jdp[kRCap + 1] = incl; }
  } else if (wave == 1) {
    const int4 n = reinterpret_cast<const int4*>(thist)[lane];
    const int4 ng = make_int4((n.x + 3) >> 2, (n.y + 3) >> 2, (n.z + 3) >> 2, (n.w + 3) >> 2);
    const int s4 = ng.x + ng.y + ng.z + ng.w;
    const int incl = wave_incl_scan(s4);
    const int ex = incl - s4;
    reinterpret_cast<int4*>(tgb)[lane] = make_int4(ex, ex + ng.x, ex + ng.x + ng.y, ex + ng.x + ng.y + ng.z);
    const int ngrp_all = __builtin_amdgcn_readlane(incl, 63);
    int gmax = (ngrp_all + kTRunTarget - 1) / kTRunTarget;
    gmax = gmax < 2 ? 2 : gmax;
    const float rgm = 1.0f / (float)gmax;
    const int4 nr = make_int4(fast_div(ng.x + gmax - 1, gmax, rgm), fast_div(ng.y + gmax - 1, gmax, rgm),
                              fast_div(ng.z + gmax - 1, gmax, rgm), fast_div(ng.w + gmax - 1, gmax, rgm));
    const int r4 = nr.x + nr.y + nr.z + nr.w;
    const int rincl = wave_incl_scan(r4);
    int ri = rincl - r4;
    uint16_t* runs = reinterpret_cast<uint16_t*>(rec + trec_runs_off(p.Vb, p.ecap));
    for (int i = 0; i < nr.x; ++i) runs[ri++] = (uint16_t)(ex + i * gmax);
    for (int i = 0; i < nr.y; ++i) runs[ri++] = (uint16_t)(ex + ng.x + i * gmax);
    for (int i = 0; i < nr.z; ++i) runs[ri++] = (uint16_t)(ex + ng.x + ng.y + i * gmax);
    for (int i = 0; i < nr.w; ++i) runs[ri++] = (uint16_t)(ex + ng.x + ng.y + ng.z + i * gmax);
    if (lane == 63) {
      runs[rincl] = (uint16_t)incl;
      *reinterpret_cast<uint16_t*>(rec + kTRecNrun) = (uint16_t)rincl;
      misc[0] = incl;
    }
  }
  lds_barrier();
  CSTAMP(5);

  int pos = tid;
  if (tid < R) pos = dstart[255 - dcl] + atomicAdd(&dcur[255 - dcl], 1);
  place[tid] = pos;
  {
    const int my_id = idl[tid];
    r_rowatom[pos] = my_id;
    r_poolrow[tid] = (uint16_t)(pos | (my_id > 0 ? 0x8000 : 0));
    r_rowdeg[pos] = (uint16_t)my_deg;
    if ((pos & 15) == 0) r_tilemax[pos >> 4] = (unsigned char)dcl;
    r_jd[tid] = (uint16_t)jdp[tid];
    if (tid < 2) r_jd[kRCap + tid] = (uint16_t)jdp[kRCap];
    if (pos == 0) {
      r_cw[0] = (uint16_t)misc[0];
      r_cw[1] = (uint16_t)jdp[kRCap];
      r_cw[2] = (uint16_t)dcl;
    }
    if (tid == 0)
      reinterpret_cast<int4*>(p.desc)[idx] = make_int4(m0, M, jdp[kRCap] < p.ecap ? jdp[kRCap] : p.ecap, R | (g << 16));
  }
  {
    const int n_t = thist[tid];
    const int ng = (n_t + 3) >> 2, gb = tgb[tid];
    const uint32_t dump = (uint32_t)tmsg_key(p.ecap) * 0x10001u;
    for (int jg = 0; jg < ng; ++jg) {
      const int c = n_t - 4 * jg;
      grp[gb + jg] = make_uint4((uint32_t)tid | ((uint32_t)(c < 4 ? c : 4) << 8) | ((uint32_t)(ng - jg) << 24), 0u, dump, dump);
    }
  }
  lds_barrier();
  CSTAMP(6);

  {
    auto below = [](uint4 a, uint32_t ue) {
      return (int)(((a.x & 0xffffu) < ue) + ((a.x >> 16) < ue) + ((a.y & 0xffffu) < ue) + ((a.y >> 16) < ue) +
                   ((a.z & 0xffffu) < ue) + ((a.z >> 16) < ue) + ((a.w & 0xffffu) < ue) + ((a.w >> 16) < ue));
    };
    const int nval = misc[1] < kTECapBig ? misc[1] : kTECapBig;
    for (int i0 = 0; i0 < nval; i0 += 2 * kRCap) {
      bool ok[2];
      uint2 en[2];
      int row[2], srow[2], deg[2], ix[2], gb[2], rank[2];
      uint4 ta[2], tb[2];
#pragma unroll
      for (int k = 0; k < 2; ++k) {
        const int i = i0 + k * kRCap + tid;
        ok[k] = i < nval;
        en[k] = elist[ok[k] ? i : 0];
      }
#pragma unroll
      for (int k = 0; k < 2; ++k) {
        const int rt = (int)(en[k].x & 0xffu), bid = (int)(en[k].x >> 16);
        deg[k] = cnt[rt];
        ta[k] = reinterpret_cast<const uint4*>(tick)[2 * rt];
        tb[k] = reinterpret_cast<const uint4*>(tick)[2 * rt + 1];
        row[k] = place[rt];
        srow[k] = place[(en[k].x >> 8) & 0xffu];
        gb[k] = tgb[bid];
        ix[k] = atomicAdd(&tcur[ok[k] ? bid : kTVbMax + lane], 1);
      }
#pragma unroll
      for (int k = 0; k < 2; ++k) {
        rank[k] = below(ta[k], en[k].y) + below(tb[k], en[k].y);
        if (deg[k] > kTick) {
          const int rt = (int)(en[k].x & 0xffu);
          int lo = 0, hi = M - 1;
          while (lo < hi) {
            const int mid = (lo + hi + 1) >> 1;
            if (moloff[mid] <= rt) lo = mid; else hi = mid - 1;
          }
          const int t = rt - moloff[lo];
          const int32_t* cm = conn_c + 2 * (int64_t)lo * E;
          const int32_t* bm = bond_c + (int64_t)lo * E;
          rank[k] = 0;
          for (int e2 = 0; e2 < (int)en[k].y; ++e2) {
            const int2 s2 = *reinterpret_cast<const int2*>(cm + 2 * e2);
            rank[k] += (s2.y == t && edge_valid(s2.x, s2.y, bm[e2], N, p.Vb)) ? 1 : 0;
          }
        }
        rank[k] = jdp[rank[k] < 256 ? rank[k] : 255];
      }
#pragma unroll
      for (int k = 0; k < 2; ++k) {
        if (ok[k]) {
          unsigned char* ge = reinterpret_cast<unsigned char*>(&grp[gb[k] + (ix[k] >> 2)]);
          ge[4 + (ix[k] & 3)] = (unsigned char)srow[k];
          reinterpret_cast<uint16_t*>(ge + 8)[ix[k] & 3] = (uint16_t)tmsg_key(rank[k] + row[k]);
          if (rank[k] + row[k] < p.ecap)
            r_slist[rank[k] + row[k]] = tsrc_word((int)(en[k].x >> 16), idl[(en[k].x >> 8) & 0xffu]);
        }
      }
    }
  }
  lds_barrier();
  CSTAMP(9);

  {
    const int ngrp = misc[0];
    uint4* r_grp = reinterpret_cast<uint4*>(rec + kTRecGrp);
    for (int i = tid; i < ngrp; i += kRCap) r_grp[i] = grp[i];
  }
  CSTAMP(15);
  lds_barrier();
  }
}
#undef CSTAMP

}

int launch_weight_image(const ImageParams& ip, int S, hipStream_t s) {
  if (S <= 0) return IMPNN_OK;
  weight_image_kernel<<<dim3(16, S), 256, 0, s>>>(ip);
  return check_launch("weight_image");
}

int launch_typed_image(const TImageParams& ip, hipStream_t s) {
  const int S = ip.S > 0 ? ip.S : 1;
  float* canon = ip.prepared + (size_t)S * (ip.x3 ? kXUpdSlot : kTUpdSlot) + (size_t)S * ip.Vb * kTMatFloats;
  for (int st = 0; st < ip.S; ++st) {
    if (int rc = launch_bond_type_matrices(ip.bond_table, ip.weights + (int64_t)st * ip.step_floats, canon, ip.Vb, ip.K,
                                           kD, s))
      return rc;
    typed_image_kernel<<<(ip.Vb * kTMatFloats + kTUpdSlot + 255) / 256 < 256 ? (ip.Vb * kTMatFloats + kTUpdSlot + 255) / 256 : 256,
                         256, 0, s>>>(ip, st);
    if (int rc = check_launch("typed_image")) return rc;
  }
  return IMPNN_OK;
}

int launch_plan(const PlanParams& pp, hipStream_t s) {
  plan_stats_kernel<<<pp.n_ions * pp.nblk, 64 * kPB, 0, s>>>(pp);
  if (int rc = check_launch("plan_stats")) return rc;
  if ((int64_t)2 * pp.n_ions * pp.B / pp.nwg + 64 > kShareCap)
    return fail(IMPNN_E_UNSUPPORTED, "encoder plan: batch of %d molecules per ion is too large", pp.B);
  if (pp.max_sub > kMaxHops)
    return fail(IMPNN_E_UNSUPPORTED, "encoder plan: %d chunk slots per workgroup", pp.max_sub);
  if (pp.typed)
    plan_chunks_typed_kernel<<<pp.nwg * pp.grid_sub, kRCap, sizeof(uint4) * tgrp_cap(pp.Vb, pp.ecap), s>>>(pp);
  else
    plan_chunks_kernel<<<pp.nwg * pp.grid_sub, kRCap, 0, s>>>(pp);
  return check_launch("plan_chunks");
}

}
}
```

### ionic_mpnn_amd/csrc/encoder_typed.hip

```cpp
#include "encoder_device.h"
#include "encoder_layout.h"
#include "kernel_device.h"

namespace impnn {
namespace enc {

namespace {

constexpr int kOffUpd = 0;
constexpr int off_h(bool x3) { return kOffUpd + (x3 ? kXUpdLds : kTUpdLds); }
constexpr int kTHSBig3 = 32;
constexpr int off_msg(bool x3, int hs = kTHS) { return off_h(x3) + kRCap * hs; }
constexpr int off_rec(bool x3, int ecap, int hs = kTHS) { return off_msg(x3, hs) + tmsg_floats(ecap); }
constexpr size_t lds_fixed_bytes(bool x3, int Vb, int ecap, int hs = kTHS) {
  return sizeof(float) * (size_t)off_rec(x3, ecap, hs) + trec_lds_bytes(Vb, ecap);
}
static_assert(lds_fixed_bytes(true, kTVbMax, kTECap) <= 160 * 1024 && lds_fixed_bytes(false, kTVbMax, kTECapBig) <= 160 * 1024 &&
                  lds_fixed_bytes(true, kTVbMax, kTECapBig, kTHSBig3) <= 160 * 1024,
              "LDS budget");

typedef bf16x8_t bf16x8;
struct B3 {
  bf16x8 p0, p1, p2;
};
__device__ __forceinline__ B3 split8x3(f32x4 a, f32x4 b) {
  union {
    bf16x8 v;
    unsigned u[4];
  } q0, q1, q2;
  split_pair(a[0], a[1], q0.u[0], q1.u[0], q2.u[0]);
  split_pair(a[2], a[3], q0.u[1], q1.u[1], q2.u[1]);
  split_pair(b[0], b[1], q0.u[2], q1.u[2], q2.u[2]);
  split_pair(b[2], b[3], q0.u[3], q1.u[3], q2.u[3]);
  B3 r;
  r.p0 = q0.v;
  r.p1 = q1.v;
  r.p2 = q2.v;
  return r;
}
__device__ __forceinline__ void mma9x2(f32x4& c0, f32x4& c1, const __bf16* blk0, const __bf16* blk1, int lane, const B3& b) {
  const bf16x8 a00 = *reinterpret_cast<const bf16x8*>(blk0 + lane * 8);
  const bf16x8 a01 = *reinterpret_cast<const bf16x8*>(blk0 + 512 + lane * 8);
  const bf16x8 a02 = *reinterpret_cast<const bf16x8*>(blk0 + 1024 + lane * 8);
  const bf16x8 a10 = *reinterpret_cast<const bf16x8*>(blk1 + lane * 8);
  const bf16x8 a11 = *reinterpret_cast<const bf16x8*>(blk1 + 512 + lane * 8);
  const bf16x8 a12 = *reinterpret_cast<const bf16x8*>(blk1 + 1024 + lane * 8);
  c0 = mfma_bf16(a02, b.p2, c0);  c1 = mfma_bf16(a12, b.p2, c1);
  c0 = mfma_bf16(a01, b.p2, c0);  c1 = mfma_bf16(a11, b.p2, c1);
  c0 = mfma_bf16(a02, b.p1, c0);  c1 = mfma_bf16(a12, b.p1, c1);
  c0 = mfma_bf16(a00, b.p2, c0);  c1 = mfma_bf16(a10, b.p2, c1);
  c0 = mfma_bf16(a02, b.p0, c0);  c1 = mfma_bf16(a12, b.p0, c1);
  c0 = mfma_bf16(a01, b.p1, c0);  c1 = mfma_bf16(a11, b.p1, c1);
  c0 = mfma_bf16(a00, b.p1, c0);  c1 = mfma_bf16(a10, b.p1, c1);
  c0 = mfma_bf16(a01, b.p0, c0);  c1 = mfma_bf16(a11, b.p0, c1);
  c0 = mfma_bf16(a00, b.p0, c0);  c1 = mfma_bf16(a10, b.p0, c1);
}

template <int ABID>
__device__ __forceinline__ f32x4 mfma1(float a, float b, f32x4 c) {
  return __builtin_amdgcn_mfma_f32_4x4x1f32(a, b, c, 3, ABID, 0);
}

typedef float f32x2v __attribute__((ext_vector_type(2)));
typedef __attribute__((address_space(3))) void* lds_ptr_t;
__device__ __forceinline__ void glds16(const void* gsrc, const float* dst) {
  const unsigned lds_dst = __builtin_amdgcn_readfirstlane((unsigned)(uintptr_t)(lds_ptr_t)dst);
  unsigned keep;
  asm volatile("s_mov_b32 %0, m0\n\ts_mov_b32 m0, %2\n\ts_nop 0\n\tglobal_load_lds_dwordx4 %1, off\n\ts_mov_b32 m0, %0"
               : "=&s"(keep)
               : "v"(gsrc), "s"(lds_dst)
               : "memory");
}
struct Grp {
  uint4 ge;
  f32x2v aq;
};
struct Run {
  f32x4 bq[4];
  Grp first;
};

__device__ __forceinline__ void group_messages(const f32x2v aq, const f32x4 (&bq)[4], float& m01, float& m23) {
  f32x4 acc0 = {0.f, 0.f, 0.f, 0.f}, acc1 = acc0;
#ifndef IMPNN_DIAG_NO_MSG_MFMA
  acc0 = mfma1<0>(aq[0], bq[0][0], acc0);
  acc1 = mfma1<0>(aq[1], bq[0][1], acc1);
  acc0 = mfma1<1>(aq[0], bq[0][2], acc0);
  acc1 = mfma1<1>(aq[1], bq[0][3], acc1);
  acc0 = mfma1<2>(aq[0], bq[1][0], acc0);
  acc1 = mfma1<2>(aq[1], bq[1][1], acc1);
  acc0 = mfma1<3>(aq[0], bq[1][2], acc0);
  acc1 = mfma1<3>(aq[1], bq[1][3], acc1);
  acc0 = mfma1<4>(aq[0], bq[2][0], acc0);
  acc1 = mfma1<4>(aq[1], bq[2][1], acc1);
  acc0 = mfma1<5>(aq[0], bq[2][2], acc0);
  acc1 = mfma1<5>(aq[1], bq[2][3], acc1);
  acc0 = mfma1<6>(aq[0], bq[3][0], acc0);
  acc1 = mfma1<6>(aq[1], bq[3][1], acc1);
  acc0 = mfma1<7>(aq[0], bq[3][2], acc0);
  acc1 = mfma1<7>(aq[1], bq[3][3], acc1);
#else
  acc0[0] = aq[0] + bq[0][0] + bq[3][3];
  acc1[1] = aq[1] + bq[1][1] + bq[2][2];
#endif
  float x0 = acc0[0] + acc1[0], x1 = acc0[1] + acc1[1], x2 = acc0[2] + acc1[2], x3 = acc0[3] + acc1[3];
  asm volatile("s_nop 1\n\tv_permlane32_swap_b32 %0, %1\n\tv_permlane32_swap_b32 %2, %3"
               : "+v"(x0), "+v"(x1), "+v"(x2), "+v"(x3));
  m01 = x0 + x1;
  m23 = x2 + x3;
}

__global__ __launch_bounds__(256) void typed_m0_kernel(const float* tmat0, const float* atom_table, float* m0,
                                                       M0Header* hdr, int Va, int Vb, int S) {
  const int lane = threadIdx.x & 63;
  const int w = __builtin_amdgcn_readfirstlane(blockIdx.x * 4 + (threadIdx.x >> 6));
  const int nga = (Va + 4) >> 2;
  if (w < Vb * nga) {
    const int v = w / nga, a0 = 4 * (w - v * nga);
    const int kh = lane >> 5, f = lane & 31;
    const int ai = a0 + (lane & 3);
    f32x2v aq = {0.f, 0.f};
    if (ai < Va) aq = *reinterpret_cast<const f32x2v*>(atom_table + (size_t)ai * kD + 16 * kh + 2 * ((lane >> 2) & 7));
    const float* bp = tmat0 + (size_t)v * kTMatFloats + kh * 512 + f * 4;
    f32x4 bq[4];
#pragma unroll
    for (int i = 0; i < 4; ++i) bq[i] = ld4(bp + i * 128);
    float m01, m23;
    group_messages(aq, bq, m01, m23);
    float* row = m0 + (size_t)v * (Va + 1) * kD + f;
    if (a0 + kh <= Va) row[(size_t)(a0 + kh) * kD] = m01;
    if (a0 + 2 + kh <= Va) row[(size_t)(a0 + 2 + kh) * kD] = m23;
  }
  if (blockIdx.x == 0 && threadIdx.x == 0) *hdr = M0Header{kM0Magic, Va, Vb, S};
}

#ifndef IMPNN_T_PF
#define IMPNN_T_PF 0
#endif
#ifndef IMPNN_T_EARLY
#define IMPNN_T_EARLY 0
#endif
constexpr int kPfWhere = IMPNN_T_PF, kRunsEarly = IMPNN_T_EARLY;
template <int N, bool LANES>
__device__ __forceinline__ void reduce_ranks(const float* msg, const uint16_t* jdptr, int d0, int deg, int row, int q,
                                             int zero_slot, f32x4& agg0, f32x4& agg1) {
  const uint2 jd = *reinterpret_cast<const uint2*>(jdptr + d0);
  const int first[4] = {(int)(jd.x & 0xffffu), (int)(jd.x >> 16), (int)(jd.y & 0xffffu), (int)(jd.y >> 16)};
  f32x4 m0v[N], m1v[N];
#pragma unroll
  for (int j = 0; j < N; ++j) {
    const int o = tmsg_off(d0 + j < deg ? first[j] + row : zero_slot, q);
    m0v[j] = ld4(msg + o);
    m1v[j] = ld4(msg + (o ^ 16));
  }
#pragma unroll
  for (int j = 0; j < N; ++j) {
    if constexpr (LANES) {
#pragma unroll
      for (int i = 0; i < 4; ++i) {
        agg0[i] = lane1(agg0[i] + m0v[j][i]);
        agg1[i] = lane1(agg1[i] + m1v[j][i]);
      }
    } else {
      agg0 += m0v[j];
      agg1 += m1v[j];
    }
  }
}

__device__ __forceinline__ float keep1(float v) { return lane1(v); }
__device__ __forceinline__ f32x4 keep1(f32x4 v) { return v; }
template <bool LANES, class F, class... A>
__device__ __forceinline__ f32x4 quad(F f, A... a) {
  if constexpr (LANES) {
    f32x4 r;
#pragma unroll
    for (int i = 0; i < 4; ++i) r[i] = f(a[i]...);
    return r;
  } else {
    return f(a...);
  }
}

template <bool STAMPS, bool X3, int HS = kTHS>
__global__ __launch_bounds__(kThreads, kThreads / 256) void encoder_typed_kernel(TEncParams p) {
  extern __shared__ __align__(16) float smem[];
  constexpr int kUpdLds = X3 ? kXUpdLds : kTUpdLds, kUpdSlot = X3 ? kXUpdSlot : kTUpdSlot;
  constexpr int kNPf = X3 ? 3 : 2;
  float* const wupd = smem + kOffUpd;
  float* const wvec = wupd + (X3 ? kXVecFloatOff : kTVecFloatOff);
  float* const hbuf = smem + off_h(X3);
  float* const msg = smem + off_msg(X3, HS);
  const int zero_slot = p.ecap + 1;
  unsigned char* const recl = reinterpret_cast<unsigned char*>(smem + off_rec(X3, p.ecap, HS));
  const int rec_lds = p.rec_lds;
  float* const atab = reinterpret_cast<float*>(recl + rec_lds);
  const uint16_t* const r_rowdeg = reinterpret_cast<const uint16_t*>(recl + kTRecRowdeg);
  const unsigned char* const r_tilemax = recl + kTRecTilemax;
  const uint16_t* const r_moloff = reinterpret_cast<const uint16_t*>(recl + kTRecMoloff);
  const uint16_t* const r_molrows = reinterpret_cast<const uint16_t*>(recl + kTRecMolrows);
  const uint16_t* const r_poolrow = reinterpret_cast<const uint16_t*>(recl + kTRecPoolrow);
  const int32_t* const r_rowatom = reinterpret_cast<const int32_t*>(recl + kTRecRowatom);
  const uint16_t* const r_jdptr = reinterpret_cast<const uint16_t*>(recl + kTRecJdptr);
  const uint16_t* const r_runs = reinterpret_cast<const uint16_t*>(recl + trec_runs_off(p.Vb, p.ecap));
  int* const run_ctr = reinterpret_cast<int*>(recl + kTRecCounts + 8);
  const uint4* const r_grp = reinterpret_cast<const uint4*>(recl + kTRecGrp);

  const int tid = threadIdx.x, lane = tid & 63;
  const int wave = __builtin_amdgcn_readfirstlane(tid >> 6);
  const int a = lane & 15, q = lane >> 4;
  unsigned long long* stamp = STAMPS && p.stamps ? p.stamps + (size_t)blockIdx.x * 32 : nullptr;
  if (stamp && tid == 0) stamp[0] = __builtin_amdgcn_s_memtime();

  {
    const PlanHeader hd = *p.header;
    if (hd.magic != kPlanMagic || hd.kind != 1 || hd.nwg != (int)gridDim.x || hd.max_sub != p.max_sub ||
        hd.B != p.B || hd.n_ions != p.n_ions || hd.overflow != 0) {
      const float nan = __builtin_nanf("");
      for (int g = 0; g < p.n_ions; ++g)
        for (int64_t t = (int64_t)blockIdx.x * kThreads + tid; t < (int64_t)p.B * kD; t += (int64_t)gridDim.x * kThreads)
          p.pooled[g][t] = nan;
      return;
    }
  }
  const int c_begin = blockIdx.x * p.max_sub;
  const int c_end = c_begin + __builtin_amdgcn_readfirstlane(p.nsub[blockIdx.x]);
  if (c_begin >= c_end) return;

  if (p.atab_lds)
    for (int t = tid; t < (p.Va + 1) * (kTAS / 4); t += kThreads)
      st4(atab + 4 * t, t < p.Va * (kD / 4) ? ld4(p.atom_table + 4 * t) : f32x4{0.f, 0.f, 0.f, 0.f});
  if (tid < kD) msg[zero_slot * kD + tid] = 0.f;
  unsigned long long t_pro = 0, t_steps = 0, t_pool = 0, t_mark = 0, t_msg = 0;
  if (stamp && tid == 0) t_mark = __builtin_amdgcn_s_memtime();

  auto pool = [&](int M, int m0, int g) {
    float* out_g = p.pooled[g];
    for (int t0 = 0; t0 < M * 64; t0 += kThreads) {
      const int t = t0 + tid;
      const int part = t & 7, f4 = (t >> 3) & 7, m = t >> 6;
      f32x4 acc = {0.f, 0.f, 0.f, 0.f};
      if (m < M) {
        const int nr = r_molrows[m], mo = r_moloff[m];
        for (int n = part; n < nr; n += 8) {
          const int pr = r_poolrow[mo + n];
          if (pr & 0x8000) acc += ld4(hbuf + (pr & 0xff) * HS + 4 * f4);
        }
      }
#pragma unroll
      for (int i = 0; i < 4; ++i) {
        float v = acc[i];
        v += __builtin_bit_cast(float, __builtin_amdgcn_update_dpp(0, __builtin_bit_cast(int, v), 0xb1, 0xf, 0xf, true));
        v += __builtin_bit_cast(float, __builtin_amdgcn_update_dpp(0, __builtin_bit_cast(int, v), 0x4e, 0xf, 0xf, true));
        v += __builtin_bit_cast(float, __builtin_amdgcn_update_dpp(0, __builtin_bit_cast(int, v), 0x141, 0xf, 0xf, true));
        acc[i] = v;
      }
      if (m < M && part == 0) st4(out_g + (int64_t)(m0 + m) * kD + 4 * f4, acc);
    }
  };
  auto fill_h0 = [&]() {
    const int row = tid >> 2, sub = tid & 3;
    const int id = r_rowatom[row];
    f32x4 v0 = {0.f, 0.f, 0.f, 0.f}, v1 = v0;
    if ((unsigned)id < (unsigned)p.Va) {
      if (p.atab_lds) {
        v0 = ld4(atab + id * kTAS + 8 * sub);
        v1 = ld4(atab + id * kTAS + 8 * sub + 4);
      } else {
        int sb = sub;
        asm volatile("" : "+v"(sb));
        v0 = ld4(p.atom_table + (int64_t)id * kD + 8 * sb);
        v1 = ld4(p.atom_table + (int64_t)id * kD + 8 * sb + 4);
      }
    }
    st4(hbuf + row * HS + 8 * sub, v0);
    st4(hbuf + row * HS + 8 * sub + 4, v1);
  };

  if (p.S == 0) {
    for (int c = c_begin; c < c_end; ++c) {
      const unsigned char* rc = p.rec + (size_t)c * kTRecBytes;
      if (8 * tid < rec_lds) reinterpret_cast<uint2*>(recl)[tid] = reinterpret_cast<const uint2*>(rc)[tid];
      const int4 dsc = reinterpret_cast<const int4*>(p.desc)[c];
      lds_barrier();
      fill_h0();
      lds_barrier();
      pool(__builtin_amdgcn_readfirstlane(dsc.y), __builtin_amdgcn_readfirstlane(dsc.x),
           __builtin_amdgcn_readfirstlane(dsc.w) >> 16);
      lds_barrier();
    }
    return;
  }

  unsigned tabmask = 0;
  {
    const M0Header t0 = *reinterpret_cast<const M0Header*>(p.upd[0] + kUpdLds);
    if (t0.magic == kM0Magic && t0.Va == p.Va && t0.Vb == p.Vb && t0.S == p.S) tabmask |= 1u;
    if (p.n_ions > 1) {
      const M0Header t1 = *reinterpret_cast<const M0Header*>(p.upd[1] + kUpdLds);
      if (t1.magic == kM0Magic && t1.Va == p.Va && t1.Vb == p.Vb && t1.S == p.S) tabmask |= 2u;
    }
  }

  const bool rec_big = rec_lds > kTRecPart1;
  const unsigned char* rec_c = p.rec + (size_t)c_begin * kTRecBytes;
  uint2 rec_n8 = reinterpret_cast<const uint2*>(rec_c)[tid];
  uint32_t rec_n4 = rec_big ? reinterpret_cast<const uint32_t*>(rec_c + kTRecPart1)[tid] : 0u;
  int4 dsc_next = reinterpret_cast<const int4*>(p.desc)[c_begin];

  auto fetch_step0 = [&](const int4 dn, int cn) {
    const int gn = __builtin_amdgcn_readfirstlane(dn.w) >> 16;
    const float* const ug = p.upd[gn];
    static_assert(kUpdLds % 256 == 0, "whole 64-lane transfers");
    int ln = lane, wv = wave;
    asm volatile("" : "+v"(ln), "+s"(wv));
    const bool tabn = (tabmask >> gn) & 1u;
    int edges = __builtin_amdgcn_readfirstlane(dn.z);
    edges = tabn ? (edges < p.ecap ? edges : p.ecap) : 0;
    constexpr int kIt = (kTECapBig / 8 + kWaves - 1) / kWaves;
    uint32_t sw[kIt];
    if (tabn) {
      const uint32_t* const lst = p.slist + (size_t)cn * p.ecap;
#pragma unroll
      for (int i = 0; i < kIt; ++i) {
        const int sl = 8 * (wv + i * kWaves) + (ln >> 3);
        const uint32_t word = lst[sl < edges ? sl : 0];
        sw[i] = sl < edges ? word : 0u;
      }
    } else {
#pragma unroll
      for (int i = 0; i < kIt; ++i) sw[i] = 0u;
    }
    constexpr int kUIt = (kUpdLds / 256 + kWaves - 1) / kWaves;
#pragma unroll
    for (int i = 0; i < kUIt; ++i) {
      const int ub = 64 * (wv + i * kWaves);
      if (ub < kUpdLds / 4) glds16(ug + 4 * (ub + ln), wupd + 4 * ub);
    }
    static_assert(kIt == 5, "the list words are landed by name");
    asm volatile("" : "+v"(sw[0]), "+v"(sw[1]), "+v"(sw[2]), "+v"(sw[3]), "+v"(sw[4]) : : "memory");
    const float* const m0_g = p.m0[gn];
#pragma unroll
    for (int i = 0; i < kIt; ++i) {
      const int base = 8 * (wv + i * kWaves);
      if (base < edges) {
        const int sl = base + (ln >> 3);
        const unsigned type = min(sw[i] >> 24, (unsigned)p.Vb - 1u), col = min(sw[i] & kSrcIdNone, (unsigned)p.Va);
        const unsigned off = (type * (unsigned)(p.Va + 1) + col) * kD + 4u * ((ln & 7) ^ ((sl >> 1) & 7));
        glds16(m0_g + off, msg + kD * base);
      }
    }
  };
  fetch_step0(dsc_next, c_begin);

  const uint32_t* const grp_x = reinterpret_cast<const uint32_t*>(r_grp);
  const int kh = lane >> 5, f = lane & 31;
  const int boff = kh * 512 + f * 4;
  const int ysh = 8 * (lane & 3), zsh = 16 * kh;
  const int acol = 16 * kh + 2 * ((lane >> 2) & 7);

  for (int c = c_begin; c < c_end; ++c) {
    const int4 dsc = dsc_next;
    const int m0 = __builtin_amdgcn_readfirstlane(dsc.x), M = __builtin_amdgcn_readfirstlane(dsc.y);
    const int rg = __builtin_amdgcn_readfirstlane(dsc.w);
    const int R = rg & 0xffff, g = rg >> 16;
    const int ntiles = (R + 15) >> 4;
    const float* upd_g = p.upd[g];
    const float* tmat_g = p.tmat[g];
    const bool tab0 = (tabmask >> g) & 1u;
    if (8 * tid < rec_lds) reinterpret_cast<uint2*>(recl)[tid] = rec_n8;
    if (rec_big && kTRecPart1 + 4 * tid < rec_lds) reinterpret_cast<uint32_t*>(recl + kTRecPart1)[tid] = rec_n4;
    lds_barrier();
    fill_h0();
    if (tid == 0) *run_ctr = 2 * kWaves;
    asm volatile("s_waitcnt vmcnt(0) lgkmcnt(0)\n\ts_barrier" ::: "memory");
    {
      const int cn = (c + 1) < c_end ? (c + 1) : c;
      const unsigned char* rn = p.rec + (size_t)cn * kTRecBytes;
      rec_n8 = reinterpret_cast<const uint2*>(rn)[tid];
      if (rec_big) rec_n4 = reinterpret_cast<const uint32_t*>(rn + kTRecPart1)[tid];
      dsc_next = reinterpret_cast<const int4*>(p.desc)[cn];
    }
    if (stamp && tid == 0) {
      const unsigned long long t = __builtin_amdgcn_s_memtime();
      t_pro += t - t_mark;
      t_mark = t;
    }
    const int nrun = __builtin_amdgcn_readfirstlane(*reinterpret_cast<const uint16_t*>(recl + kTRecNrun));

    Run P, Q;
    int gP = 0, nP = 0, gQ = 0, nQ = 0;
    bool haveP = false, haveQ = false;
    const bool sP = wave < nrun, sQ = wave + kWaves < nrun;
    const int sgP = __builtin_amdgcn_readfirstlane(r_runs[sP ? wave : 0]);
    const int snP = __builtin_amdgcn_readfirstlane(r_runs[(sP ? wave : 0) + 1]) - sgP;
    const int sgQ = __builtin_amdgcn_readfirstlane(r_runs[sQ ? wave + kWaves : 0]);
    const int snQ = __builtin_amdgcn_readfirstlane(r_runs[(sQ ? wave + kWaves : 0) + 1]) - sgQ;
    const int soP = sP ? (__builtin_amdgcn_readfirstlane(grp_x[4 * sgP]) & 0xff) * kTMatFloats : 0;
    const int soQ = sQ ? (__builtin_amdgcn_readfirstlane(grp_x[4 * sgQ]) & 0xff) * kTMatFloats : 0;
    const int lboffP = sP ? boff : 0, lboffQ = sQ ? boff : 0;
    f32x4 pf[kNPf];
    auto fetch_pf = [&](int s_) {
#pragma unroll
      for (int i = 0; i < kNPf; ++i) pf[i] = ld4(upd_g + (int64_t)s_ * kUpdSlot + 4 * (tid + i * kThreads));
    };
    auto fetch_P = [&](int s_) {
      const float* tm = tmat_g + (size_t)s_ * p.Vb * kTMatFloats;
#pragma unroll
      for (int i = 0; i < 4; ++i) P.bq[i] = ld4(tm + soP + lboffP + i * 128);
    };
    auto fetch_Q = [&](int s_) {
      const float* tm = tmat_g + (size_t)s_ * p.Vb * kTMatFloats;
#pragma unroll
      for (int i = 0; i < 4; ++i) Q.bq[i] = ld4(tm + soQ + lboffQ + i * 128);
    };
    if (kRunsEarly >= 1) fetch_P(0);
    if (kRunsEarly >= 2) fetch_Q(0);
    if (stamp && c == c_begin && tid == 0) stamp[13] = __builtin_amdgcn_s_memtime();
    for (int s = 0; s < p.S; ++s) {
      const float* tm_s = tmat_g + (size_t)s * p.Vb * kTMatFloats;
      __builtin_amdgcn_s_setprio(2);
      const bool from_tab = tab0 && s == 0;
      if (kPfWhere == 0) {
        if (s > 0) {
          fetch_pf(s);
        } else {
#pragma unroll
          for (int i = 0; i < kNPf; ++i) pf[i] = f32x4{0.f, 0.f, 0.f, 0.f};
        }
      }
      if (!from_tab) {
        const float* const abase = hbuf + acol;
        auto load_group = [&](int e, Grp& G) {
          G.ge = r_grp[e];
          const int src = __builtin_amdgcn_ubfe(G.ge.y, ysh, 8);
          G.aq = *reinterpret_cast<const f32x2v*>(abase + src * HS);
        };
        auto compute = [&](const Grp& G, const f32x4 (&bq)[4]) {
          float m01, m23;
          group_messages(G.aq, bq, m01, m23);
          msg[__builtin_amdgcn_ubfe(G.ge.z, zsh, 16) ^ f] = m01;
          msg[__builtin_amdgcn_ubfe(G.ge.w, zsh, 16) ^ f] = m23;
        };
        auto run_type = [&](int g_, int n_, Run& Rn) {
          const int end = g_ + n_;
          Grp T;
          int e = g_;
          while (true) {
            if (e + 1 < end) load_group(e + 1, T);
            compute(Rn.first, Rn.bq);
            if (++e >= end) break;
            if (e + 1 < end) load_group(e + 1, Rn.first);
            compute(T, Rn.bq);
            if (++e >= end) break;
          }
        };
        auto fetch = [&](bool have, int r, int& g_, int& n_, Run& Rn, const float* tm) {
          const int rc = have ? r : 0;
          g_ = __builtin_amdgcn_readfirstlane(r_runs[rc]);
          n_ = __builtin_amdgcn_readfirstlane(r_runs[rc + 1]) - g_;
          const int type = have ? (__builtin_amdgcn_readfirstlane(grp_x[4 * g_]) & 0xff) : 0;
          const float* bp = tm + (size_t)type * kTMatFloats + (have ? boff : 0);
#pragma unroll
          for (int i = 0; i < 4; ++i) Rn.bq[i] = ld4(bp + i * 128);
        };
        auto next_run = [&]() {
          int r = 0;
          if (lane == 0) r = atomicAdd(run_ctr, 1);
          return __builtin_amdgcn_readfirstlane(r);
        };
        auto take = [&](int r, int& g_, int& n_, Run& Rn) {
          fetch(true, r, g_, n_, Rn, tm_s);
          load_group(g_, Rn.first);
        };
        auto landed = [](f32x4 (&b)[4]) {
          asm volatile("" : "+v"(b[0]), "+v"(b[1]), "+v"(b[2]), "+v"(b[3]) : : "memory");
        };
        if (kRunsEarly < 1) fetch_P(s);
        if (kRunsEarly < 2) fetch_Q(s);
        haveP = sP; gP = sgP; nP = snP;
        haveQ = sQ; gQ = sgQ; nQ = snQ;
        if (haveP) load_group(gP, P.first);
        if (haveQ) load_group(gQ, Q.first);
        if (haveP) {
          if (!haveQ) {
            landed(P.bq);
            run_type(gP, nP, P);
          } else {
            while (true) {
              landed(P.bq);
              run_type(gP, nP, P);
              const int rP = next_run();
              if (rP >= nrun) {
                landed(Q.bq);
                run_type(gQ, nQ, Q);
                break;
              }
              take(rP, gP, nP, P);
              landed(Q.bq);
              run_type(gQ, nQ, Q);
              const int rQ = next_run();
              if (rQ >= nrun) {
                landed(P.bq);
                run_type(gP, nP, P);
                break;
              }
              take(rQ, gQ, nQ, Q);
            }
          }
        }
        landed(P.bq);
        landed(Q.bq);
      }
      if (s > 0) {
#pragma unroll
        for (int i = 0; i < kNPf; ++i)
          if (4 * (tid + i * kThreads) < kUpdLds) st4(wupd + 4 * (tid + i * kThreads), pf[i]);
      }
      const bool mstamp = stamp && c == c_begin && s == 1;
      if (mstamp && lane == 0) stamp[16 + wave] = __builtin_amdgcn_s_memtime();
      lds_barrier();
      if (tid == 0) *run_ctr = 2 * kWaves;
      if (mstamp && tid == 0) stamp[12] = __builtin_amdgcn_s_memtime();
      if (stamp && tid == 0 && c == c_begin && s == 1) t_msg = __builtin_amdgcn_s_memtime();

      int my_tile = -1;
      {
        const int grp = wave & 3, slot = wave >> 2, q4 = ntiles >> 2, r4 = ntiles & 3;
        const int heavy = (4 - r4) * q4;
        if (grp >= r4) {
          if (slot < q4) my_tile = slot * (4 - r4) + (grp - r4);
        } else if (slot <= q4) {
          my_tile = heavy + slot * r4 + grp;
        }
      }
      const bool has_tile = my_tile >= 0 && my_tile < ntiles;
      if (has_tile) {
        const int tile = my_tile;
        const int row = tile * 16 + a;
        const int deg = r_rowdeg[row];
        const int maxdeg = __builtin_amdgcn_readfirstlane(r_tilemax[tile]);
        f32x4 h0, h1, z0, z1, r0, r1;
        [[maybe_unused]] const __bf16* const wb = reinterpret_cast<const __bf16*>(wupd);
        if constexpr (X3) {
          h0 = ld4(hbuf + row * HS + 4 * q);
          h1 = ld4(hbuf + row * HS + 16 + 4 * q);
          z0 = ld4(wvec + 0 * kD + 4 * q), z1 = ld4(wvec + 0 * kD + 16 + 4 * q);
          r0 = ld4(wvec + 1 * kD + 4 * q), r1 = ld4(wvec + 1 * kD + 16 + 4 * q);
          const B3 sh = split8x3(h0, h1);
          mma9x2(z0, z1, wb + ((0 * 2 + 0) * 2 + 0) * 1536, wb + ((0 * 2 + 1) * 2 + 0) * 1536, lane, sh);
          mma9x2(r0, r1, wb + ((1 * 2 + 0) * 2 + 0) * 1536, wb + ((1 * 2 + 1) * 2 + 0) * 1536, lane, sh);
        }
        f32x4 agg0 = {0.f, 0.f, 0.f, 0.f}, agg1 = agg0;
        if (maxdeg <= 2) {
          if (maxdeg == 1) reduce_ranks<1, X3>(msg, r_jdptr, 0, deg, row, q, zero_slot, agg0, agg1);
          if (maxdeg == 2) reduce_ranks<2, X3>(msg, r_jdptr, 0, deg, row, q, zero_slot, agg0, agg1);
        } else {
          for (int d0 = 0; d0 < maxdeg; d0 += 4) reduce_ranks<4, X3>(msg, r_jdptr, d0, deg, row, q, zero_slot, agg0, agg1);
        }
        if (mstamp && wave == 1 && lane == 0) stamp[8] = __builtin_amdgcn_s_memtime();
        __builtin_amdgcn_s_setprio(1);
        if (s + 1 < p.S) {
          if (kPfWhere == 1) fetch_pf(s + 1);
          if (kRunsEarly >= 1) fetch_P(s + 1);
          if (kRunsEarly >= 2) fetch_Q(s + 1);
        }
        if constexpr (!X3) {
          h0 = ld4(hbuf + row * HS + 4 * q);
          h1 = ld4(hbuf + row * HS + 16 + 4 * q);
          z0 = ld4(wvec + 0 * kD + 4 * q), z1 = ld4(wvec + 0 * kD + 16 + 4 * q);
          r0 = ld4(wvec + 1 * kD + 4 * q), r1 = ld4(wvec + 1 * kD + 16 + 4 * q);
        }
        f32x4 t0 = ld4(wvec + 2 * kD + 4 * q), t1 = ld4(wvec + 2 * kD + 16 + 4 * q);
        if constexpr (X3) {
          const B3 sa = split8x3(agg0, agg1);
          mma9x2(z0, z1, wb + ((0 * 2 + 0) * 2 + 1) * 1536, wb + ((0 * 2 + 1) * 2 + 1) * 1536, lane, sa);
          mma9x2(r0, r1, wb + ((1 * 2 + 0) * 2 + 1) * 1536, wb + ((1 * 2 + 1) * 2 + 1) * 1536, lane, sa);
          z0 = sigmoid4_lanes(z0);
          z1 = sigmoid4_lanes(z1);
          const f32x4 rh0 = mul4_lanes(sigmoid4_lanes(r0), h0);
          const f32x4 rh1 = mul4_lanes(sigmoid4_lanes(r1), h1);
          const B3 srh = split8x3(rh0, rh1);
          mma9x2(t0, t1, wb + ((2 * 2 + 0) * 2 + 0) * 1536, wb + ((2 * 2 + 1) * 2 + 0) * 1536, lane, srh);
          mma9x2(t0, t1, wb + ((2 * 2 + 0) * 2 + 1) * 1536, wb + ((2 * 2 + 1) * 2 + 1) * 1536, lane, sa);
        } else {
          const float* wl = wupd + 4 * lane;
#pragma unroll
          for (int half = 0; half < 2; ++half) {
#pragma unroll
            for (int u = 0; u < 2; ++u) {
              const int hu = half * 2 + u;
              const f32x4 Az0 = ld4(wl + ((0 * 2 + 0) * 4 + hu) * 256);
              const f32x4 Az1 = ld4(wl + ((0 * 2 + 1) * 4 + hu) * 256);
              const f32x4 Ar0 = ld4(wl + ((1 * 2 + 0) * 4 + hu) * 256);
              const f32x4 Ar1 = ld4(wl + ((1 * 2 + 1) * 4 + hu) * 256);
              const f32x4 Bv = half == 0 ? (u == 0 ? h0 : h1) : (u == 0 ? agg0 : agg1);
#pragma unroll
              for (int r = 0; r < 4; ++r) {
                z0 = mfma4(Az0[r], Bv[r], z0);
                z1 = mfma4(Az1[r], Bv[r], z1);
                r0 = mfma4(Ar0[r], Bv[r], r0);
                r1 = mfma4(Ar1[r], Bv[r], r1);
              }
            }
          }
          z0 = sigmoid4<false>(z0);
          z1 = sigmoid4<false>(z1);
          const f32x4 rh0 = sigmoid4<false>(r0) * h0;
          const f32x4 rh1 = sigmoid4<false>(r1) * h1;
#pragma unroll
          for (int half = 0; half < 2; ++half) {
#pragma unroll
            for (int u = 0; u < 2; ++u) {
              const int hu = half * 2 + u;
              const f32x4 Ah0 = ld4(wl + ((2 * 2 + 0) * 4 + hu) * 256);
              const f32x4 Ah1 = ld4(wl + ((2 * 2 + 1) * 4 + hu) * 256);
              const f32x4 Bv = half == 0 ? (u == 0 ? rh0 : rh1) : (u == 0 ? agg0 : agg1);
#pragma unroll
              for (int r = 0; r < 4; ++r) {
                t0 = mfma4(Ah0[r], Bv[r], t0);
                t1 = mfma4(Ah1[r], Bv[r], t1);
              }
            }
          }
        }
        __builtin_amdgcn_s_setprio(0);
        if (kPfWhere == 2 && s + 1 < p.S) {
          asm volatile("" ::: "memory");
          fetch_pf(s + 1);
        }
        if (mstamp && wave == 1 && lane == 0) stamp[9] = __builtin_amdgcn_s_memtime();
        const f32x4 gm0 = ld4(wvec + 3 * kD + 4 * q), gm1 = ld4(wvec + 3 * kD + 16 + 4 * q);
        const f32x4 bt0 = ld4(wvec + 4 * kD + 4 * q), bt1 = ld4(wvec + 4 * kD + 16 + 4 * q);
        __builtin_amdgcn_sched_barrier(0);
        const f32x4 th0 = X3 ? tanh4_lanes(t0) : tanh4<false>(t0), th1 = X3 ? tanh4_lanes(t1) : tanh4<false>(t1);
        const auto blend = [](auto z, auto th, auto h) { return keep1(z * (th - h) + h); };
        f32x4 n0 = quad<X3>(blend, z0, th0, h0), n1 = quad<X3>(blend, z1, th1, h1);
        const f32x4 s4 = quad<X3>([](auto x, auto y) { return keep1(x + y); }, n0, n1);
        const float sum = sum_xor16_xor32((s4[0] + s4[1]) + (s4[2] + s4[3]));
        const float mean = sum * (1.0f / kD);
        const auto center = [mean](auto n) { return keep1(n - mean); };
        n0 = quad<X3>(center, n0);
        n1 = quad<X3>(center, n1);
        const f32x4 q4 = quad<X3>([](auto x, auto y) { return keep1(x * x + y * y); }, n0, n1);
        const float var = sum_xor16_xor32((q4[0] + q4[1]) + (q4[2] + q4[3]));
        const float inv = __builtin_amdgcn_rsqf(var * (1.0f / kD) + p.ln_eps);
        const auto affine = [inv](auto n, auto gm, auto bt, auto h) { return keep1(n * keep1(gm * inv) + keep1(bt + h)); };
        const f32x4 o0 = quad<X3>(affine, n0, gm0, bt0, h0), o1 = quad<X3>(affine, n1, gm1, bt1, h1);
        st4(hbuf + row * HS + 4 * q, o0);
        st4(hbuf + row * HS + 16 + 4 * q, o1);
        if (mstamp && wave == 1 && lane == 0) stamp[10] = __builtin_amdgcn_s_memtime();
      }
      if (!has_tile && s + 1 < p.S) {
        if (kPfWhere != 0) fetch_pf(s + 1);
        if (kRunsEarly >= 1) fetch_P(s + 1);
        if (kRunsEarly >= 2) fetch_Q(s + 1);
      }
      if (mstamp && wave == 1 && lane == 0) stamp[11] = __builtin_amdgcn_s_memtime();
      lds_barrier();
      if (stamp && c == c_begin && s < 2 && tid == 0) stamp[14 + s] = __builtin_amdgcn_s_memtime();
    }
    if (stamp && tid == 0) {
      const unsigned long long t = __builtin_amdgcn_s_memtime();
      t_steps += t - t_mark;
      t_mark = t;
    }

    asm volatile(""
                 : "+v"(rec_n8.x), "+v"(rec_n8.y), "+v"(rec_n4), "+v"(dsc_next.x), "+v"(dsc_next.y), "+v"(dsc_next.z),
                   "+v"(dsc_next.w)
                 :
                 : "memory");
    if (c + 1 < c_end) fetch_step0(dsc_next, c + 1);
    pool(M, m0, g);
    lds_barrier();
    if (stamp && tid == 0) {
      const unsigned long long t = __builtin_amdgcn_s_memtime();
      t_pool += t - t_mark;
      t_mark = t;
    }
  }
  if (stamp && tid == 0) {
    stamp[1] = t_pro;
    stamp[2] = t_steps;
    stamp[3] = t_pool;
    stamp[4] = (unsigned long long)(c_end - c_begin);
    stamp[5] = t_msg;
    stamp[7] = __builtin_amdgcn_s_memtime();
  }
}

}
}

bool encoder_typed_supported(int N, int E, int D, int S, int Vb) {
  using namespace enc;
  if (D != kD || S < 0) return false;
  if (N < 1 || N > 0xffff || E < 0 || E > 0xffff) return false;
  if (Vb < 1 || Vb > kTVbMax) return false;
  return true;
}

size_t encoder_typed_prepared_bytes(int S, int Vb, bool x3) {
  return enc::typed_prepared_floats(S, Vb, x3) * sizeof(float);
}

int launch_encoder_typed_prepare(const float* weights, const float* bond_table, int K, int S, int Vb, bool x3,
                                 void* prepared, hipStream_t s) {
  if (S <= 0) return IMPNN_OK;
  enc::TImageParams ip{};
  ip.weights = weights;
  ip.bond_table = bond_table;
  ip.prepared = static_cast<float*>(prepared);
  ip.K = K;
  ip.S = S;
  ip.Vb = Vb;
  ip.x3 = x3 ? 1 : 0;
  ip.step_floats = impnn_encoder_step_floats(enc::kD, K);
  return enc::launch_typed_image(ip, s);
}

size_t encoder_typed_prepared_bytes_atoms(int S, int Va, int Vb, bool x3) {
  return (enc::typed_prepared_floats(S, Vb, x3) + enc::m0_table_floats(S, Va, Vb)) * sizeof(float);
}

int launch_encoder_typed_prepare_atoms(const float* weights, const float* bond_table, const float* atom_table, int Va,
                                       int K, int S, int Vb, bool x3, void* prepared, hipStream_t s) {
  using namespace enc;
  if (int rc = launch_encoder_typed_prepare(weights, bond_table, K, S, Vb, x3, prepared, s)) return rc;
  if (m0_table_floats(S, Va, Vb) == 0) return IMPNN_OK;
  float* img = static_cast<float*>(prepared);
  const size_t uslot = x3 ? kXUpdSlot : kTUpdSlot;
  const int waves = Vb * ((Va + 4) >> 2);
  typed_m0_kernel<<<(waves + 3) / 4, 256, 0, s>>>(img + (size_t)S * uslot, atom_table, img + typed_prepared_floats(S, Vb, x3),
                                                  reinterpret_cast<M0Header*>(img + (x3 ? kXUpdLds : kTUpdLds)), Va, Vb, S);
  return check_launch("typed_m0");
}

int launch_encoder_typed_run(const EncoderArgs& a, const enc::Ws& w, hipStream_t s) {
  using namespace enc;
  char* base = static_cast<char*>(a.workspace);
  TEncParams ep{};
  const size_t S1 = a.S > 0 ? a.S : 1;
  const bool x3 = a.mode == 3;
  const size_t uslot = x3 ? kXUpdSlot : kTUpdSlot;
  for (int g = 0; g < a.n_ions; ++g) {
    const float* prep;
    if (a.prepared[g]) {
      if (!aligned16(a.prepared[g])) return fail(IMPNN_E_BADARG, "encoder_fused: prepared weights must be 16B aligned");
      prep = static_cast<const float*>(a.prepared[g]);
    } else {
      float* img = reinterpret_cast<float*>(base + w.img_off) + (size_t)g * typed_prepared_floats(a.S, a.Vb, x3);
      if (int rc = launch_encoder_typed_prepare(a.weights[g], a.bond_table, a.K, a.S, a.Vb, x3, img, s)) return rc;
      prep = img;
    }
    ep.upd[g] = prep;
    ep.tmat[g] = prep + S1 * uslot;
    ep.m0[g] = prep + typed_prepared_floats(a.S, a.Vb, x3);
    ep.pooled[g] = a.pooled[g];
  }
  ep.atom_table = a.atom_table;
  ep.nsub = reinterpret_cast<const int32_t*>(base + w.nsub_off);
  ep.desc = reinterpret_cast<const int32_t*>(base + w.desc_off);
  ep.rec = reinterpret_cast<const unsigned char*>(base + w.rec_off);
  ep.slist = reinterpret_cast<const uint32_t*>(base + w.slist_off);
  ep.header = reinterpret_cast<const PlanHeader*>(base);
  ep.n_ions = a.n_ions; ep.B = a.B; ep.S = a.S; ep.Va = a.Va; ep.Vb = a.Vb; ep.max_sub = w.max_sub;
  ep.ln_eps = a.ln_eps;
  ep.stamps = nullptr;
  {
    size_t sb = 0;
    void* sp = debug_stamp_buffer(&sb);
    if (sp && sb >= (size_t)w.nwg * 32 * sizeof(unsigned long long)) ep.stamps = static_cast<unsigned long long*>(sp);
  }
  ep.upd_slot = (int)uslot;
  ep.ecap = tecap_of(a.E);
  ep.rec_lds = trec_lds_bytes(a.Vb, ep.ecap);
  const bool big3 = x3 && ep.ecap == kTECapBig;
  void (*kern)(TEncParams) =
      big3 ? (ep.stamps ? encoder_typed_kernel<true, true, kTHSBig3> : encoder_typed_kernel<false, true, kTHSBig3>)
      : x3 ? (ep.stamps ? encoder_typed_kernel<true, true> : encoder_typed_kernel<false, true>)
           : (ep.stamps ? encoder_typed_kernel<true, false> : encoder_typed_kernel<false, false>);
  if (int rc = ensure_lds_limit((const void*)kern, big3 ? (ep.stamps ? 10 : 9) : (ep.stamps ? 5 : 4) + (x3 ? 2 : 0))) return rc;
  size_t lds = lds_fixed_bytes(x3, a.Vb, ep.ecap, big3 ? kTHSBig3 : kTHS);
  const size_t atab_bytes = ((size_t)a.Va + 1) * kTAS * sizeof(float);
  ep.atab_lds = lds + atab_bytes <= 160 * 1024;
  if (ep.atab_lds) lds += atab_bytes;
  profile_record_start(s);
  kern<<<w.nwg, kThreads, lds, s>>>(ep);
  profile_record_stop(s);
  return check_launch("encoder_typed");
}

}
```

Measured before the change: 39.59 million.

## Fuse per-chunk plan construction into the typed encoder kernel preamble

When both phases run in typed mode, the separate plan-chunks kernel is replaced by a stats-only plan launch. Each encoder workgroup then resolves its own chain and builds its chunk records in LDS before running the encoder. This removes a kernel launch and the global-memory handoff of plan data between the two kernels. In exchange the encoder kernel carries a larger preamble and possibly a bigger LDS requirement, which may lower occupancy, and the planning work is serialised inside each workgroup ahead of the main compute.

```diff
diff --git a/ionic_mpnn_amd/csrc/common.h b/ionic_mpnn_amd/csrc/common.h
--- a/ionic_mpnn_amd/csrc/common.h
+++ b/ionic_mpnn_amd/csrc/common.h
@@ -418,7 +418,7 @@
 int encoder_workgroups(int n_ions, int B, int requested, int N, int E, int mode);
 size_t encoder_fused_workspace_bytes(int mode, int n_ions, int B, int N, int E, int D, int S, int Vb, int nwg);
 int launch_encoder_fused(const EncoderArgs& a, hipStream_t s);
-int launch_encoder_phase(const EncoderArgs& a, hipStream_t s, bool plan_phase);
+int launch_encoder_phase(const EncoderArgs& a, hipStream_t s, bool plan_phase, bool plan_in_encoder = false);
 size_t encoder_prepared_bytes(int mode, int D, int S, int Vb);
 int launch_encoder_prepare(const float* weights, const float* bond_table, int D, int K, int S, int Vb, int mode,
                            void* prepared, hipStream_t s);
diff --git a/ionic_mpnn_amd/csrc/encoder_fused.hip b/ionic_mpnn_amd/csrc/encoder_fused.hip
--- a/ionic_mpnn_amd/csrc/encoder_fused.hip
+++ b/ionic_mpnn_amd/csrc/encoder_fused.hip
@@ -437,7 +437,7 @@
 size_t encoder_typed_prepared_bytes_atoms(int S, int Va, int Vb, bool x3);
 int launch_encoder_typed_prepare_atoms(const float* weights, const float* bond_table, const float* atom_table, int Va,
                                        int K, int S, int Vb, bool x3, void* prepared, hipStream_t s);
-int launch_encoder_typed_run(const EncoderArgs& a, const enc::Ws& w, hipStream_t s);
+int launch_encoder_typed_run(const EncoderArgs& a, const enc::Ws& w, hipStream_t s, const enc::PlanParams* plan = nullptr);
 
 bool encoder_fused_supported(int mode, int N, int E, int D, int K, int S, int Vb) {
   using namespace enc;
@@ -532,8 +532,17 @@
   return launch_encoder_prepare(weights, bond_table, D, K, S, Vb, mode, prepared, s);
 }
 
+static bool plan_fused_enabled() {
+  static const bool on = [] {
+    const char* e = getenv("IMPNN_PLAN_FUSED");
+    return !(e && e[0] == '0' && e[1] == 0);
+  }();
+  return on;
+}
+
 int launch_encoder_fused(const EncoderArgs& a, hipStream_t s) {
   if (a.D != enc::kD) return launch_encoder_wide(a, s);
+  if ((a.phases & 3) == 3 && a.mode >= 2 && plan_fused_enabled()) return launch_encoder_phase(a, s, true, true);
   if (a.phases & 1)
     if (int rc = launch_encoder_phase(a, s, true)) return rc;
   if (a.phases & 2)
@@ -541,12 +550,13 @@
   return IMPNN_OK;
 }
 
-int launch_encoder_phase(const EncoderArgs& a, hipStream_t s, bool plan_phase) {
+int launch_encoder_phase(const EncoderArgs& a, hipStream_t s, bool plan_phase, bool plan_in_encoder) {
   using namespace enc;
   const bool typed = a.mode >= 2;
+  const bool running = !plan_phase || plan_in_encoder;
   const Ws w = ws_layout(a.n_ions, a.B, a.N, a.E, a.S, a.Vb, a.nwg, typed, a.mode == 3);
   if (!aligned16(a.workspace)) return fail(IMPNN_E_BADARG, "encoder_fused: workspace must be 16B aligned");
-  if (!plan_phase && !aligned16(a.atom_table)) return fail(IMPNN_E_BADARG, "encoder_fused: atom_table must be 16B aligned");
+  if (running && !aligned16(a.atom_table)) return fail(IMPNN_E_BADARG, "encoder_fused: atom_table must be 16B aligned");
   char* base = static_cast<char*>(a.workspace);
   const int mode = a.mode == 1 ? 1 : 0;
   PlanParams pp{};
@@ -594,6 +604,10 @@
     if (sp && sb >= ((size_t)w.nwg * 32 + 16) * sizeof(unsigned long long))
       pp.stamps = static_cast<unsigned long long*>(sp) + (size_t)w.nwg * 32;
   }
+  if (plan_in_encoder) {
+    if (int rc = launch_plan(pp, s, true)) return rc;
+    return launch_encoder_typed_run(a, w, s, &pp);
+  }
   if (plan_phase) return launch_plan(pp, s);
   if (typed) return launch_encoder_typed_run(a, w, s);
 
diff --git a/ionic_mpnn_amd/csrc/encoder_layout.h b/ionic_mpnn_amd/csrc/encoder_layout.h
--- a/ionic_mpnn_amd/csrc/encoder_layout.h
+++ b/ionic_mpnn_amd/csrc/encoder_layout.h
@@ -252,6 +252,7 @@
   int upd_slot;
   int rec_lds;
   int ecap;
+  int plan_here;
   float ln_eps;
   unsigned long long* stamps;
 };
@@ -275,7 +276,7 @@
 }
 
 int launch_weight_image(const ImageParams& ip, int S, hipStream_t s);
-int launch_plan(const PlanParams& pp, hipStream_t s);
+int launch_plan(const PlanParams& pp, hipStream_t s, bool stats_only = false);
 int launch_typed_image(const TImageParams& ip, hipStream_t s);
 
 }
diff --git a/ionic_mpnn_amd/csrc/encoder_plan.hip b/ionic_mpnn_amd/csrc/encoder_plan.hip
--- a/ionic_mpnn_amd/csrc/encoder_plan.hip
+++ b/ionic_mpnn_amd/csrc/encoder_plan.hip
@@ -1,4 +1,5 @@
 #include "encoder_layout.h"
+#include "encoder_plan_device.h"
 
 namespace impnn {
 namespace enc {
@@ -239,260 +240,6 @@
   }
 }
 
-__device__ __forceinline__ int xcd_slot(int j, int nwg) {
-#ifdef IMPNN_DIAG_NO_XCD_MAP
-  return j;
-#else
-  const int lo = (nwg >> 3) * 4 + ((nwg & 7) < 4 ? (nwg & 7) : 4);
-  const int r = j & 7, qd = j >> 3;
-  return r < 4 ? qd * 4 + r : lo + qd * 4 + (r - 4);
-#endif
-}
-
-__device__ __forceinline__ int share_bound(int tg, int jj, int nwg_g) {
-  if (jj <= 0) return 0;
-  if (jj >= nwg_g) return tg;
-  const int t = (int)((float)tg * (float)jj * __frcp_rn((float)nwg_g));
-  return t < 0 ? 0 : (t > tg ? tg : t);
-}
-__device__ __forceinline__ int ion_split(long long t0, long long t1, int nwg) {
-  int n0 = (t0 + t1) > 0 ? (int)((float)nwg * (float)t0 * __frcp_rn((float)(t0 + t1)) + 0.5f) : nwg / 2;
-  if (nwg >= 2) n0 = n0 < 1 ? 1 : (n0 > nwg - 1 ? nwg - 1 : n0);
-  return n0;
-}
-
-#define CSTAMP(i) do { if (p.stamps && blockIdx.x == 0 && threadIdx.x == 0) p.stamps[i] = __builtin_amdgcn_s_memtime(); } while (0)
-__device__ __forceinline__ bool resolve_share(const PlanParams& p, int j, int lane, int& g, int& k0, int& bp0,
-                                              int& t_lo, int& t_hi, bool& bad) {
-  const int nblk = p.nblk;
-  bad = false;
-  constexpr int kPU = 4;
-  const int npass = (nblk + 64 * kPU - 1) / (64 * kPU);
-  if (npass == 1) {
-    int v[2][kPU];
-    int anybad = 0;
-#pragma unroll
-    for (int gi = 0; gi < 2; ++gi)
-#pragma unroll
-      for (int i = 0; i < kPU; ++i) {
-        const int k = kPU * lane + i;
-        const int kk = k < nblk ? k : nblk - 1;
-        const int x = gi < p.n_ions ? p.partial[(int64_t)gi * nblk + kk] : 0;
-        anybad |= k < nblk ? x : 0;
-        v[gi][i] = k < nblk ? (x & ~kPlanBadBit) : 0;
-      }
-    if (__ballot((anybad & kPlanBadBit) != 0)) bad = true;
-    if (bad) return false;
-    CSTAMP(10);
-    int ex[2], tot[2];
-#pragma unroll
-    for (int gi = 0; gi < 2; ++gi) {
-      const int s4 = v[gi][0] + v[gi][1] + v[gi][2] + v[gi][3];
-      const int incl = wave_incl_scan(s4);
-      ex[gi] = incl - s4;
-      tot[gi] = __builtin_amdgcn_readlane(incl, 63);
-    }
-    int nwg0 = p.nwg, nwg1 = 0;
-    if (p.n_ions == 2) {
-      int n0 = ion_split(tot[0], tot[1], p.nwg);
-      nwg0 = n0;
-      nwg1 = p.nwg - n0;
-    }
-    const int jp = xcd_slot(j, p.nwg);
-    g = jp < nwg0 ? 0 : 1;
-    const int jj = jp - (g ? nwg0 : 0);
-    const int nwg_g = g ? nwg1 : nwg0;
-    const int tg = tot[g];
-    t_lo = share_bound(tg, jj, nwg_g);
-    t_hi = share_bound(tg, jj + 1, nwg_g);
-    k0 = 0;
-    bp0 = 0;
-    if (t_hi <= t_lo) return false;
-    const int e0 = g ? ex[1] : ex[0];
-    const int a0 = g ? v[1][0] : v[0][0], a1 = g ? v[1][1] : v[0][1], a2 = g ? v[1][2] : v[0][2], a3 = g ? v[1][3] : v[0][3];
-    const unsigned long long hit = __ballot(e0 <= t_lo && t_lo < e0 + a0 + a1 + a2 + a3);
-    if (hit == 0ull) return false;
-    const int src = __builtin_ctzll(hit);
-    const int i_in = t_lo < e0 + a0 ? 0 : (t_lo < e0 + a0 + a1 ? 1 : (t_lo < e0 + a0 + a1 + a2 ? 2 : 3));
-    const int st_in = e0 + (i_in > 0 ? a0 : 0) + (i_in > 1 ? a1 : 0) + (i_in > 2 ? a2 : 0);
-    k0 = kPU * src + __builtin_amdgcn_readlane(i_in, src);
-    bp0 = __builtin_amdgcn_readlane(st_in, src);
-    return true;
-  }
-  long long tot[2] = {0, 0};
-  for (int gi = 0; gi < p.n_ions; ++gi) {
-    const int32_t* part = p.partial + (int64_t)gi * nblk;
-    int acc = 0, anybad = 0;
-    for (int k = lane; k < nblk; k += 64) {
-      const int x = part[k];
-      anybad |= x & kPlanBadBit;
-      acc += x & ~kPlanBadBit;
-    }
-    if (__ballot(anybad != 0)) bad = true;
-    tot[gi] = wave_incl_scan(acc);
-    tot[gi] = __builtin_amdgcn_readlane((int)tot[gi], 63);
-  }
-  if (bad) return false;
-  int nwg0 = p.nwg, nwg1 = 0;
-  if (p.n_ions == 2) {
-    int n0 = ion_split(tot[0], tot[1], p.nwg);
-    nwg0 = n0;
-    nwg1 = p.nwg - n0;
-  }
-  const int jp = xcd_slot(j, p.nwg);
-  g = jp < nwg0 ? 0 : 1;
-  const int jj = jp - (g ? nwg0 : 0);
-  const int nwg_g = g ? nwg1 : nwg0;
-  const int tg = (int)tot[g];
-  t_lo = share_bound(tg, jj, nwg_g);
-  t_hi = share_bound(tg, jj + 1, nwg_g);
-  k0 = 0;
-  bp0 = 0;
-  if (t_hi <= t_lo) return false;
-  const int32_t* part = p.partial + (int64_t)g * nblk;
-  int carry = 0;
-  bool found = false;
-  for (int kbase = 0; kbase < nblk && !found; kbase += 64) {
-    const int k = kbase + lane;
-    const int v = k < nblk ? (part[k < nblk ? k : nblk - 1] & ~kPlanBadBit) : 0;
-    const int incl = wave_incl_scan(v);
-    const int st = carry + incl - v;
-    const unsigned long long hit = __ballot(k < nblk && st <= t_lo && t_lo < st + v);
-    if (hit) {
-      const int src = __builtin_ctzll(hit);
-      k0 = kbase + src;
-      bp0 = __builtin_amdgcn_readlane(st, src);
-      found = true;
-    }
-    carry += __builtin_amdgcn_readlane(incl, 63);
-  }
-  return found;
-}
-
-constexpr int kDegBins = 18;
-
-struct ShareTab {
-  int32_t shst[kShareCap + 1];
-  int32_t cb[kMaxHops + 1];
-  int32_t vwin[256];
-  int chunk_s[3];
-};
-
-__device__ __forceinline__ int fast_div(int x, int d, float rd) {
-  int q = (int)((float)x * rd);
-  if (q * d > x) --q;
-  if ((q + 1) * d <= x) ++q;
-  return q;
-}
-
-__device__ __forceinline__ void resolve_chain(const PlanParams& p, int j, int slot_i, int lane, ShareTab& T) {
-  int gg = 0, w_lo = 0;
-  {
-    const int half = p.n_ions == 2 ? (p.nwg >> 1 > 0 ? p.nwg >> 1 : 1) : p.nwg;
-    const int jp = xcd_slot(j, p.nwg);
-    gg = (p.n_ions == 2 && jp >= half) ? 1 : 0;
-    const int jj = jp - (gg ? half : 0);
-    const int nw = gg ? (p.nwg - half > 0 ? p.nwg - half : 1) : half;
-    w_lo = (int)((float)jj * (float)p.B / (float)nw) - 64;
-    w_lo = w_lo < 0 ? 0 : w_lo;
-    w_lo &= ~15;
-  }
-  int vw[4];
-  {
-    const int32_t* vrg = p.vr + (int64_t)gg * p.B;
-#pragma unroll
-    for (int i = 0; i < 4; ++i) {
-      const int m = w_lo + 64 * i + lane;
-      vw[i] = vrg[m < p.B ? m : p.B - 1];
-    }
-  }
-  int g = 0, k0 = 0, bp0 = 0, t_lo = 0, t_hi = 0;
-  bool bad = false;
-  const bool have = resolve_share(p, j, lane, g, k0, bp0, t_lo, t_hi, bad);
-  CSTAMP(11);
-#pragma unroll
-  for (int i = 0; i < 4; ++i) T.vwin[64 * i + lane] = vw[i];
-  if (!have) {
-    if (lane == 0) {
-      T.chunk_s[0] = -1; T.chunk_s[1] = 0; T.chunk_s[2] = 0;
-      if (slot_i == 0) p.nsub[j] = 0;
-      if (bad && blockIdx.x == 0) p.header->overflow = 1;
-    }
-    return;
-  }
-  const int32_t* vrg = p.vr + (int64_t)g * p.B;
-  int run = bp0;
-  int first = -1, nsh = 0;
-  int end_row = -1;
-  __builtin_amdgcn_s_waitcnt(0xc07f);
-  auto vr_at = [&](int mbase) {
-    const int rel = mbase - w_lo;
-    if (g == gg && rel >= 0 && rel + 64 <= 256) return T.vwin[rel + lane];
-    const int m = mbase + lane;
-    return vrg[m < p.B ? m : p.B - 1];
-  };
-  int v_n1 = vr_at(k0 * kPB);
-  for (int mbase = k0 * kPB; mbase < p.B && end_row < 0; mbase += 64) {
-    const int m = mbase + lane;
-    const int v = v_n1;
-    v_n1 = vr_at(mbase + 64);
-    const int vv = m < p.B ? v : 0;
-    const int incl = wave_incl_scan(vv);
-    const int st = run + incl - vv;
-    const bool in = m < p.B && st >= t_lo && st < t_hi;
-    const unsigned long long inb = __ballot(in);
-    if (inb) {
-      if (first < 0) first = mbase + __builtin_ctzll(inb);
-      const int pos = nsh + __builtin_popcountll(inb & ((1ull << lane) - 1));
-      if (in && pos < kShareCap) T.shst[pos] = st;
-      nsh += __builtin_popcountll(inb);
-    }
-    const unsigned long long ge = __ballot(m < p.B && st >= t_hi);
-    if (ge) end_row = __builtin_amdgcn_readlane(st, __builtin_ctzll(ge));
-    run += __builtin_amdgcn_readlane(incl, 63);
-  }
-  if (end_row < 0) end_row = run;
-  if (nsh > kShareCap) {
-    if (lane == 0) p.header->overflow = 1;
-    nsh = kShareCap;
-  }
-  if (lane == 0) T.shst[nsh] = end_row;
-  __builtin_amdgcn_s_waitcnt(0xc07f);
-  CSTAMP(12);
-  int mb = 0, hop = 0;
-  if (nsh < 64) {
-    const int st_l = T.shst[lane <= nsh ? lane : nsh];
-    while (mb < nsh && hop < kMaxHops) {
-      const int lim = __builtin_amdgcn_readlane(st_l, mb) + kRCap;
-      const unsigned long long okb = __ballot(lane > mb && lane <= nsh && st_l <= lim);
-      if (lane == 0) T.cb[hop] = mb;
-      ++hop;
-      mb = okb ? 63 - __builtin_clzll(okb) : mb + 1;
-    }
-  }
-  while (mb < nsh && hop < kMaxHops) {
-    const int lim = T.shst[mb] + kRCap;
-    int e = mb + 1;
-    for (int c0 = mb + 1; c0 <= nsh; c0 += 64) {
-      const int cidx = c0 + lane;
-      const bool ok = cidx <= nsh && T.shst[cidx <= nsh ? cidx : nsh] <= lim;
-      const unsigned long long okb = __ballot(ok);
-      if (okb == 0) break;
-      e = c0 + 63 - __builtin_clzll(okb);
-      if (okb != ~0ull) break;
-    }
-    if (lane == 0) T.cb[hop] = mb;
-    ++hop;
-    mb = e;
-  }
-  if (lane == 0) {
-    T.cb[hop] = nsh;
-    T.chunk_s[0] = first;
-    T.chunk_s[1] = hop;
-    T.chunk_s[2] = g;
-    if (slot_i == 0) p.nsub[j] = hop;
-  }
-}
 
 
 __global__ __launch_bounds__(kRCap, 5) void plan_chunks_kernel(PlanParams p) {
@@ -502,10 +249,11 @@
   __shared__ uint32_t ent2[kECap + 1];
   __shared__ ShareTab T;
   __builtin_amdgcn_s_setprio(3);
+  unsigned long long* const st = p.stamps && blockIdx.x == 0 && threadIdx.x == 0 ? p.stamps : nullptr;
   CSTAMP(0);
   const int j = blockIdx.x / p.grid_sub, slot_i = blockIdx.x - j * p.grid_sub;
   const int tid = threadIdx.x, lane = tid & 63, wave = tid >> 6;
-  if (wave == 0) resolve_chain(p, j, slot_i, lane, T);
+  if (wave == 0) resolve_chain(p, j, slot_i == 0, blockIdx.x == 0, lane, T, st);
   lds_barrier();
   CSTAMP(1);
   const int first_mol = T.chunk_s[0], nhop = T.chunk_s[1], g = T.chunk_s[2];
@@ -687,350 +435,23 @@
   }
 }
 
-constexpr int kTick = 16;
 __global__ __launch_bounds__(kRCap, 4) void plan_chunks_typed_kernel(PlanParams p) {
-  __shared__ int32_t moloff[kRCap + 2], molrows[kRCap], cnt[kRCap + 64], place[kRCap];
-  __shared__ int32_t idl[kRCap];
-  __shared__ __attribute__((aligned(16))) int32_t dbins[kRCap], dstart[kRCap], dcur[kRCap];
-  __shared__ __attribute__((aligned(16))) int32_t thist[kTVbMax + 64], tgb[kTVbMax], tcur[kTVbMax + 64];
-  __shared__ __attribute__((aligned(16))) int32_t jdp[kRCap + 4];
-  __shared__ int32_t misc[4];
-  __shared__ __attribute__((aligned(16))) uint16_t tick[kRCap * kTick];
-  __shared__ uint2 elist[kTECapBig];
+  __shared__ PlanTabs L;
   extern __shared__ uint4 grp[];
   __shared__ ShareTab T;
   __builtin_amdgcn_s_setprio(3);
+  unsigned long long* const st = p.stamps && blockIdx.x == 0 && threadIdx.x == 0 ? p.stamps : nullptr;
   CSTAMP(0);
   const int j = blockIdx.x / p.grid_sub, slot_i = blockIdx.x - j * p.grid_sub;
   const int tid = threadIdx.x, lane = tid & 63, wave = tid >> 6;
-  if (wave == ((blockIdx.x >> 8) & 3)) resolve_chain(p, j, slot_i, lane, T);
+  if (wave == ((blockIdx.x >> 8) & 3)) resolve_chain(p, j, slot_i == 0, blockIdx.x == 0, lane, T, st);
   lds_barrier();
   CSTAMP(1);
-  const int first_mol = T.chunk_s[0], nhop = T.chunk_s[1], g = T.chunk_s[2];
-  const int N = p.N, E = p.E;
-  const float rE = 1.0f / (float)E;
-  for (int sl = slot_i; sl < nhop; sl += p.grid_sub) {
-  const int mb_local = T.cb[sl], M = T.cb[sl + 1] - mb_local, m0 = first_mol + mb_local;
-  const int base = T.shst[mb_local];
-  const int R = T.shst[mb_local + M] - base;
-  const int idx = j * p.max_sub + sl;
-  const int32_t* ids_g = p.atom_ids[g];
-  const int32_t* conn_g = p.conn[g];
-  const int32_t* bond_g = p.bond_ids[g];
-  const int32_t* rows_g = p.rows + (int64_t)g * p.B;
-  unsigned char* rec = p.rec + (size_t)idx * kTRecBytes;
-  uint32_t* r_slist = p.slist + (size_t)idx * p.ecap;
-  uint16_t* r_rowdeg = reinterpret_cast<uint16_t*>(rec + kTRecRowdeg);
-  unsigned char* r_tilemax = rec + kTRecTilemax;
-  uint16_t* r_moloff = reinterpret_cast<uint16_t*>(rec + kTRecMoloff);
-  uint16_t* r_molrows = reinterpret_cast<uint16_t*>(rec + kTRecMolrows);
-  uint16_t* r_poolrow = reinterpret_cast<uint16_t*>(rec + kTRecPoolrow);
-  int32_t* r_rowatom = reinterpret_cast<int32_t*>(rec + kTRecRowatom);
-  uint16_t* r_jd = reinterpret_cast<uint16_t*>(rec + kTRecJdptr);
-  uint16_t* r_cw = reinterpret_cast<uint16_t*>(rec + kTRecCounts);
-
-  const int n_slots = M * E;
-  constexpr int kSC = 6;
-  int sbid[kSC];
-  int2 sst[kSC];
-  const int32_t* conn_c = conn_g + (int64_t)m0 * E * 2;
-  const int32_t* bond_c = bond_g + (int64_t)m0 * E;
-#pragma unroll
-  for (int k = 0; k < kSC; ++k) {
-    const int slot = tid + k * kRCap;
-    sbid[k] = -1; sst[k] = make_int2(0, 0);
-    if (slot < n_slots) {
-      sst[k] = *reinterpret_cast<const int2*>(conn_c + 2 * (int64_t)slot);
-      sbid[k] = bond_c[slot];
-    }
-  }
-  constexpr int kIC = 3;
-  const int n_ids = M * N;
-  const float rN = 1.0f / (float)N;
-  const int32_t* ids_c = ids_g + (int64_t)m0 * N;
-  int sid[kIC];
-#pragma unroll
-  for (int k = 0; k < kIC; ++k) {
-    const int slot = tid + k * kRCap;
-    sid[k] = slot < n_ids ? ids_c[slot] : 0;
-  }
-  for (int m = tid; m <= M; m += kRCap) {
-    const int off = T.shst[mb_local + m] - base;
-    moloff[m] = off;
-    r_moloff[m] = (uint16_t)off;
-    if (m < M) {
-      const int rr = rows_g[m0 + m];
-      molrows[m] = rr;
-      r_molrows[m] = (uint16_t)rr;
-    }
-  }
-  cnt[tid] = 0;
-  dbins[tid] = 0;
-  dcur[tid] = 0;
-  thist[tid] = 0;
-  tcur[tid] = 0;
-  idl[tid] = -1;
-  if (tid == 0) misc[1] = 0;
-  {
-    const uint4 ones = make_uint4(~0u, ~0u, ~0u, ~0u);
-    reinterpret_cast<uint4*>(tick)[2 * tid] = ones;
-    reinterpret_cast<uint4*>(tick)[2 * tid + 1] = ones;
-  }
-  lds_barrier();
-  CSTAMP(2);
-
-  auto put_id = [&](int slot, int id) {
-    const int m = fast_div(slot, N, rN), n = slot - m * N;
-    if (slot < n_ids && n < molrows[m]) idl[moloff[m] + n] = id;
-  };
-  {
-    const int dq = fast_div(kRCap, N, rN), dr = kRCap - dq * N;
-    int cm = fast_div(tid, N, rN), cn = tid - cm * N;
-    int mr[kIC], mo[kIC], nn[kIC];
-#pragma unroll
-    for (int k = 0; k < kIC; ++k) {
-      const int mm = tid + k * kRCap < n_ids ? cm : 0;
-      mr[k] = tid + k * kRCap < n_ids ? molrows[mm] : 0;
-      mo[k] = moloff[mm];
-      nn[k] = cn;
-      cn += dr; cm += dq;
-      if (cn >= N) { cn -= N; ++cm; }
-    }
-#pragma unroll
-    for (int k = 0; k < kIC; ++k)
-      if (nn[k] < mr[k]) idl[mo[k] + nn[k]] = sid[k];
-  }
-  for (int slot = tid + kIC * kRCap; slot < n_ids; slot += kRCap) put_id(slot, ids_c[slot]);
-  {
-    unsigned okm = 0u;
-#pragma unroll
-    for (int k = 0; k < kSC; ++k) okm |= edge_valid(sst[k].x, sst[k].y, sbid[k], N, p.Vb) ? 1u << k : 0u;
-    const int mine = __builtin_popcount(okm);
-    const int incl = wave_incl_scan(mine);
-    int pos = 0;
-    if (lane == 63) pos = atomicAdd(&misc[1], incl);
-    pos = __builtin_amdgcn_readlane(pos, 63) + incl - mine;
-    const int dq = fast_div(kRCap, E, rE), dr = kRCap - dq * E;
-    int cm = fast_div(tid, E, rE), ce = tid - cm * E;
-#pragma unroll
-    for (int k0 = 0; k0 < kSC; k0 += 3) {
-      int row[3], srw[3], tk[3], es[3];
-#pragma unroll
-      for (int k = 0; k < 3; ++k) {
-        const bool ok = (okm >> (k0 + k)) & 1u;
-        const int m = cm;
-        es[k] = ce;
-        ce += dr; cm += dq;
-        if (ce >= E) { ce -= E; ++cm; }
-        const int mo = moloff[m < M ? m : 0];
-        row[k] = mo + (ok ? sst[k0 + k].y : 0);
-        srw[k] = mo + (ok ? sst[k0 + k].x : 0);
-      }
-#pragma unroll
-      for (int k = 0; k < 3; ++k) {
-        const bool ok = (okm >> (k0 + k)) & 1u;
-        tk[k] = atomicAdd(&cnt[ok ? row[k] : kRCap + lane], 1);
-        atomicAdd(&thist[ok ? sbid[k0 + k] : kTVbMax + lane], 1);
-      }
-#pragma unroll
-      for (int k = 0; k < 3; ++k) {
-        const bool ok = (okm >> (k0 + k)) & 1u;
-        if (ok && tk[k] < kTick) tick[row[k] * kTick + tk[k]] = (uint16_t)es[k];
-        if (ok) {
-          if (pos < kTECapBig)
-            elist[pos] = make_uint2((uint32_t)row[k] | ((uint32_t)srw[k] << 8) | ((uint32_t)sbid[k0 + k] << 16), (uint32_t)es[k]);
-          ++pos;
-        }
-      }
-    }
-  }
-  for (int s0 = kSC * kRCap; s0 < n_slots; s0 += kRCap) {
-    const int slot = s0 + tid;
-    int2 st = make_int2(0, 0);
-    int bid = -1;
-    if (slot < n_slots) {
-      st = *reinterpret_cast<const int2*>(conn_c + 2 * (int64_t)slot);
-      bid = bond_c[slot];
-    }
-    const bool ok = edge_valid(st.x, st.y, bid, N, p.Vb);
-    const int m = fast_div(slot, E, rE), e = slot - m * E;
-    const int mo = moloff[m < M ? m : 0];
-    const int row = mo + (ok ? st.y : 0);
-    int tk = kTick;
-    if (ok) {
-      tk = atomicAdd(&cnt[row], 1);
-      atomicAdd(&thist[bid], 1);
-    }
-    const unsigned long long okb = __ballot(ok);
-    int pos0 = 0;
-    if (okb != 0ull) {
-      if (lane == (int)__builtin_ctzll(okb)) pos0 = atomicAdd(&misc[1], (int)__builtin_popcountll(okb));
-      pos0 = __builtin_amdgcn_readlane(pos0, (int)__builtin_ctzll(okb));
-    }
-    if (tk < kTick) tick[row * kTick + tk] = (uint16_t)e;
-    const int pos = pos0 + (int)__builtin_popcountll(okb & ((1ull << lane) - 1));
-    if (ok && pos < kTECapBig)
-      elist[pos] = make_uint2((uint32_t)row | ((uint32_t)(mo + st.x) << 8) | ((uint32_t)bid << 16), (uint32_t)e);
-  }
-  lds_barrier();
-  CSTAMP(3);
-
-  const int my_deg = cnt[tid];
-  const int dcl = my_deg > 255 ? 255 : my_deg;
-  if (tid < R) {
-    if (my_deg > 255) p.header->overflow = 1;
-    atomicAdd(&dbins[255 - dcl], 1);
-  }
-  lds_barrier();
-  CSTAMP(4);
-
-  if (wave == 0) {
-    const int4 h = reinterpret_cast<const int4*>(dbins)[lane];
-    const int s4 = h.x + h.y + h.z + h.w;
-    const int ex = wave_incl_scan(s4) - s4;
-    reinterpret_cast<int4*>(dstart)[lane] = make_int4(ex, ex + h.x, ex + h.x + h.y, ex + h.x + h.y + h.z);
-    __builtin_amdgcn_s_waitcnt(0xc07f);
-    const int4 s = reinterpret_cast<const int4*>(dstart)[63 - lane];
-    const int t4 = s.x + s.y + s.z + s.w;
-    const int incl = wave_incl_scan(t4);
-    const int jx = incl - t4;
-    reinterpret_cast<int4*>(jdp)[lane] = make_int4(jx, jx + s.w, jx + s.w + s.z, jx + s.w + s.z + s.y);
-    if (lane == 63) { jdp[kRCap] = incl; jdp[kRCap + 1] = incl; }
-  } else if (wave == 1) {
-    const int4 n = reinterpret_cast<const int4*>(thist)[lane];
-    const int4 ng = make_int4((n.x + 3) >> 2, (n.y + 3) >> 2, (n.z + 3) >> 2, (n.w + 3) >> 2);
-    const int s4 = ng.x + ng.y + ng.z + ng.w;
-    const int incl = wave_incl_scan(s4);
-    const int ex = incl - s4;
-    reinterpret_cast<int4*>(tgb)[lane] = make_int4(ex, ex + ng.x, ex + ng.x + ng.y, ex + ng.x + ng.y + ng.z);
-    const int ngrp_all = __builtin_amdgcn_readlane(incl, 63);
-    int gmax = (ngrp_all + kTRunTarget - 1) / kTRunTarget;
-    gmax = gmax < 2 ? 2 : gmax;
-    const float rgm = 1.0f / (float)gmax;
-    const int4 nr = make_int4(fast_div(ng.x + gmax - 1, gmax, rgm), fast_div(ng.y + gmax - 1, gmax, rgm),
-                              fast_div(ng.z + gmax - 1, gmax, rgm), fast_div(ng.w + gmax - 1, gmax, rgm));
-    const int r4 = nr.x + nr.y + nr.z + nr.w;
-    const int rincl = wave_incl_scan(r4);
-    int ri = rincl - r4;
-    uint16_t* runs = reinterpret_cast<uint16_t*>(rec + trec_runs_off(p.Vb, p.ecap));
-    for (int i = 0; i < nr.x; ++i) runs[ri++] = (uint16_t)(ex + i * gmax);
-    for (int i = 0; i < nr.y; ++i) runs[ri++] = (uint16_t)(ex + ng.x + i * gmax);
-    for (int i = 0; i < nr.z; ++i) runs[ri++] = (uint16_t)(ex + ng.x + ng.y + i * gmax);
-    for (int i = 0; i < nr.w; ++i) runs[ri++] = (uint16_t)(ex + ng.x + ng.y + ng.z + i * gmax);
-    if (lane == 63) {
-      runs[rincl] = (uint16_t)incl;
-      *reinterpret_cast<uint16_t*>(rec + kTRecNrun) = (uint16_t)rincl;
-      misc[0] = incl;
-    }
-  }
-  lds_barrier();
-  CSTAMP(5);
-
-  int pos = tid;
-  if (tid < R) pos = dstart[255 - dcl] + atomicAdd(&dcur[255 - dcl], 1);
-  place[tid] = pos;
-  {
-    const int my_id = idl[tid];
-    r_rowatom[pos] = my_id;
-    r_poolrow[tid] = (uint16_t)(pos | (my_id > 0 ? 0x8000 : 0));
-    r_rowdeg[pos] = (uint16_t)my_deg;
-    if ((pos & 15) == 0) r_tilemax[pos >> 4] = (unsigned char)dcl;
-    r_jd[tid] = (uint16_t)jdp[tid];
-    if (tid < 2) r_jd[kRCap + tid] = (uint16_t)jdp[kRCap];
-    if (pos == 0) {
-      r_cw[0] = (uint16_t)misc[0];
-      r_cw[1] = (uint16_t)jdp[kRCap];
-      r_cw[2] = (uint16_t)dcl;
-    }
-    if (tid == 0)
-      reinterpret_cast<int4*>(p.desc)[idx] = make_int4(m0, M, jdp[kRCap] < p.ecap ? jdp[kRCap] : p.ecap, R | (g << 16));
-  }
-  {
-    const int n_t = thist[tid];
-    const int ng = (n_t + 3) >> 2, gb = tgb[tid];
-    const uint32_t dump = (uint32_t)tmsg_key(p.ecap) * 0x10001u;
-    for (int jg = 0; jg < ng; ++jg) {
-      const int c = n_t - 4 * jg;
-      grp[gb + jg] = make_uint4((uint32_t)tid | ((uint32_t)(c < 4 ? c : 4) << 8) | ((uint32_t)(ng - jg) << 24), 0u, dump, dump);
-    }
-  }
-  lds_barrier();
-  CSTAMP(6);
-
-  {
-    auto below = [](uint4 a, uint32_t ue) {
-      return (int)(((a.x & 0xffffu) < ue) + ((a.x >> 16) < ue) + ((a.y & 0xffffu) < ue) + ((a.y >> 16) < ue) +
-                   ((a.z & 0xffffu) < ue) + ((a.z >> 16) < ue) + ((a.w & 0xffffu) < ue) + ((a.w >> 16) < ue));
-    };
-    const int nval = misc[1] < kTECapBig ? misc[1] : kTECapBig;
-    for (int i0 = 0; i0 < nval; i0 += 2 * kRCap) {
-      bool ok[2];
-      uint2 en[2];
-      int row[2], srow[2], deg[2], ix[2], gb[2], rank[2];
-      uint4 ta[2], tb[2];
-#pragma unroll
-      for (int k = 0; k < 2; ++k) {
-        const int i = i0 + k * kRCap + tid;
-        ok[k] = i < nval;
-        en[k] = elist[ok[k] ? i : 0];
-      }
-#pragma unroll
-      for (int k = 0; k < 2; ++k) {
-        const int rt = (int)(en[k].x & 0xffu), bid = (int)(en[k].x >> 16);
-        deg[k] = cnt[rt];
-        ta[k] = reinterpret_cast<const uint4*>(tick)[2 * rt];
-        tb[k] = reinterpret_cast<const uint4*>(tick)[2 * rt + 1];
-        row[k] = place[rt];
-        srow[k] = place[(en[k].x >> 8) & 0xffu];
-        gb[k] = tgb[bid];
-        ix[k] = atomicAdd(&tcur[ok[k] ? bid : kTVbMax + lane], 1);
-      }
-#pragma unroll
-      for (int k = 0; k < 2; ++k) {
-        rank[k] = below(ta[k], en[k].y) + below(tb[k], en[k].y);
-        if (deg[k] > kTick) {
-          const int rt = (int)(en[k].x & 0xffu);
-          int lo = 0, hi = M - 1;
-          while (lo < hi) {
-            const int mid = (lo + hi + 1) >> 1;
-            if (moloff[mid] <= rt) lo = mid; else hi = mid - 1;
-          }
-          const int t = rt - moloff[lo];
-          const int32_t* cm = conn_c + 2 * (int64_t)lo * E;
-          const int32_t* bm = bond_c + (int64_t)lo * E;
-          rank[k] = 0;
-          for (int e2 = 0; e2 < (int)en[k].y; ++e2) {
-            const int2 s2 = *reinterpret_cast<const int2*>(cm + 2 * e2);
-            rank[k] += (s2.y == t && edge_valid(s2.x, s2.y, bm[e2], N, p.Vb)) ? 1 : 0;
-          }
-        }
-        rank[k] = jdp[rank[k] < 256 ? rank[k] : 255];
-      }
-#pragma unroll
-      for (int k = 0; k < 2; ++k) {
-        if (ok[k]) {
-          unsigned char* ge = reinterpret_cast<unsigned char*>(&grp[gb[k] + (ix[k] >> 2)]);
-          ge[4 + (ix[k] & 3)] = (unsigned char)srow[k];
-          reinterpret_cast<uint16_t*>(ge + 8)[ix[k] & 3] = (uint16_t)tmsg_key(rank[k] + row[k]);
-          if (rank[k] + row[k] < p.ecap)
-            r_slist[rank[k] + row[k]] = tsrc_word((int)(en[k].x >> 16), idl[(en[k].x >> 8) & 0xffu]);
-        }
-      }
-    }
-  }
-  lds_barrier();
-  CSTAMP(9);
-
-  {
-    const int ngrp = misc[0];
-    uint4* r_grp = reinterpret_cast<uint4*>(rec + kTRecGrp);
-    for (int i = tid; i < ngrp; i += kRCap) r_grp[i] = grp[i];
-  }
-  CSTAMP(15);
-  lds_barrier();
-  }
+  const int nhop = T.chunk_s[1];
+  for (int sl = slot_i; sl < nhop; sl += p.grid_sub) plan_chunk_typed(p, j, sl, true, tid, L, grp, T, st);
 }
 #undef CSTAMP
+
 
 }
 
@@ -1054,13 +475,14 @@
   return IMPNN_OK;
 }
 
-int launch_plan(const PlanParams& pp, hipStream_t s) {
-  plan_stats_kernel<<<pp.n_ions * pp.nblk, 64 * kPB, 0, s>>>(pp);
-  if (int rc = check_launch("plan_stats")) return rc;
+int launch_plan(const PlanParams& pp, hipStream_t s, bool stats_only) {
   if ((int64_t)2 * pp.n_ions * pp.B / pp.nwg + 64 > kShareCap)
     return fail(IMPNN_E_UNSUPPORTED, "encoder plan: batch of %d molecules per ion is too large", pp.B);
   if (pp.max_sub > kMaxHops)
     return fail(IMPNN_E_UNSUPPORTED, "encoder plan: %d chunk slots per workgroup", pp.max_sub);
+  plan_stats_kernel<<<pp.n_ions * pp.nblk, 64 * kPB, 0, s>>>(pp);
+  if (int rc = check_launch("plan_stats")) return rc;
+  if (stats_only) return IMPNN_OK;
   if (pp.typed)
     plan_chunks_typed_kernel<<<pp.nwg * pp.grid_sub, kRCap, sizeof(uint4) * tgrp_cap(pp.Vb, pp.ecap), s>>>(pp);
   else
diff --git a/ionic_mpnn_amd/csrc/encoder_plan_device.h b/ionic_mpnn_amd/csrc/encoder_plan_device.h
--- /dev/null
+++ b/ionic_mpnn_amd/csrc/encoder_plan_device.h
@@ -0,0 +1,623 @@
+#pragma once
+
+#include "encoder_layout.h"
+
+namespace impnn {
+namespace enc {
+namespace {
+
+__device__ __forceinline__ int xcd_slot(int j, int nwg) {
+#ifdef IMPNN_DIAG_NO_XCD_MAP
+  return j;
+#else
+  const int lo = (nwg >> 3) * 4 + ((nwg & 7) < 4 ? (nwg & 7) : 4);
+  const int r = j & 7, qd = j >> 3;
+  return r < 4 ? qd * 4 + r : lo + qd * 4 + (r - 4);
+#endif
+}
+
+__device__ __forceinline__ int share_bound(int tg, int jj, int nwg_g) {
+  if (jj <= 0) return 0;
+  if (jj >= nwg_g) return tg;
+  const int t = (int)((float)tg * (float)jj * __frcp_rn((float)nwg_g));
+  return t < 0 ? 0 : (t > tg ? tg : t);
+}
+__device__ __forceinline__ int ion_split(long long t0, long long t1, int nwg) {
+  int n0 = (t0 + t1) > 0 ? (int)((float)nwg * (float)t0 * __frcp_rn((float)(t0 + t1)) + 0.5f) : nwg / 2;
+  if (nwg >= 2) n0 = n0 < 1 ? 1 : (n0 > nwg - 1 ? nwg - 1 : n0);
+  return n0;
+}
+
+#define CSTAMP(i) do { if (st) st[i] = __builtin_amdgcn_s_memtime(); } while (0)
+__device__ __forceinline__ bool resolve_share(const PlanParams& p, int j, int lane, int& g, int& k0, int& bp0,
+                                              int& t_lo, int& t_hi, bool& bad, unsigned long long* st) {
+  const int nblk = p.nblk;
+  bad = false;
+  constexpr int kPU = 4;
+  const int npass = (nblk + 64 * kPU - 1) / (64 * kPU);
+  if (npass == 1) {
+    int v[2][kPU];
+    int anybad = 0;
+#pragma unroll
+    for (int gi = 0; gi < 2; ++gi)
+#pragma unroll
+      for (int i = 0; i < kPU; ++i) {
+        const int k = kPU * lane + i;
+        const int kk = k < nblk ? k : nblk - 1;
+        const int x = gi < p.n_ions ? p.partial[(int64_t)gi * nblk + kk] : 0;
+        anybad |= k < nblk ? x : 0;
+        v[gi][i] = k < nblk ? (x & ~kPlanBadBit) : 0;
+      }
+    if (__ballot((anybad & kPlanBadBit) != 0)) bad = true;
+    if (bad) return false;
+    CSTAMP(10);
+    int ex[2], tot[2];
+#pragma unroll
+    for (int gi = 0; gi < 2; ++gi) {
+      const int s4 = v[gi][0] + v[gi][1] + v[gi][2] + v[gi][3];
+      const int incl = wave_incl_scan(s4);
+      ex[gi] = incl - s4;
+      tot[gi] = __builtin_amdgcn_readlane(incl, 63);
+    }
+    int nwg0 = p.nwg, nwg1 = 0;
+    if (p.n_ions == 2) {
+      int n0 = ion_split(tot[0], tot[1], p.nwg);
+      nwg0 = n0;
+      nwg1 = p.nwg - n0;
+    }
+    const int jp = xcd_slot(j, p.nwg);
+    g = jp < nwg0 ? 0 : 1;
+    const int jj = jp - (g ? nwg0 : 0);
+    const int nwg_g = g ? nwg1 : nwg0;
+    const int tg = tot[g];
+    t_lo = share_bound(tg, jj, nwg_g);
+    t_hi = share_bound(tg, jj + 1, nwg_g);
+    k0 = 0;
+    bp0 = 0;
+    if (t_hi <= t_lo) return false;
+    const int e0 = g ? ex[1] : ex[0];
+    const int a0 = g ? v[1][0] : v[0][0], a1 = g ? v[1][1] : v[0][1], a2 = g ? v[1][2] : v[0][2], a3 = g ? v[1][3] : v[0][3];
+    const unsigned long long hit = __ballot(e0 <= t_lo && t_lo < e0 + a0 + a1 + a2 + a3);
+    if (hit == 0ull) return false;
+    const int src = __builtin_ctzll(hit);
+    const int i_in = t_lo < e0 + a0 ? 0 : (t_lo < e0 + a0 + a1 ? 1 : (t_lo < e0 + a0 + a1 + a2 ? 2 : 3));
+    const int st_in = e0 + (i_in > 0 ? a0 : 0) + (i_in > 1 ? a1 : 0) + (i_in > 2 ? a2 : 0);
+    k0 = kPU * src + __builtin_amdgcn_readlane(i_in, src);
+    bp0 = __builtin_amdgcn_readlane(st_in, src);
+    return true;
+  }
+  long long tot[2] = {0, 0};
+  for (int gi = 0; gi < p.n_ions; ++gi) {
+    const int32_t* part = p.partial + (int64_t)gi * nblk;
+    int acc = 0, anybad = 0;
+    for (int k = lane; k < nblk; k += 64) {
+      const int x = part[k];
+      anybad |= x & kPlanBadBit;
+      acc += x & ~kPlanBadBit;
+    }
+    if (__ballot(anybad != 0)) bad = true;
+    tot[gi] = wave_incl_scan(acc);
+    tot[gi] = __builtin_amdgcn_readlane((int)tot[gi], 63);
+  }
+  if (bad) return false;
+  int nwg0 = p.nwg, nwg1 = 0;
+  if (p.n_ions == 2) {
+    int n0 = ion_split(tot[0], tot[1], p.nwg);
+    nwg0 = n0;
+    nwg1 = p.nwg - n0;
+  }
+  const int jp = xcd_slot(j, p.nwg);
+  g = jp < nwg0 ? 0 : 1;
+  const int jj = jp - (g ? nwg0 : 0);
+  const int nwg_g = g ? nwg1 : nwg0;
+  const int tg = (int)tot[g];
+  t_lo = share_bound(tg, jj, nwg_g);
+  t_hi = share_bound(tg, jj + 1, nwg_g);
+  k0 = 0;
+  bp0 = 0;
+  if (t_hi <= t_lo) return false;
+  const int32_t* part = p.partial + (int64_t)g * nblk;
+  int carry = 0;
+  bool found = false;
+  for (int kbase = 0; kbase < nblk && !found; kbase += 64) {
+    const int k = kbase + lane;
+    const int v = k < nblk ? (part[k < nblk ? k : nblk - 1] & ~kPlanBadBit) : 0;
+    const int incl = wave_incl_scan(v);
+    const int st = carry + incl - v;
+    const unsigned long long hit = __ballot(k < nblk && st <= t_lo && t_lo < st + v);
+    if (hit) {
+      const int src = __builtin_ctzll(hit);
+      k0 = kbase + src;
+      bp0 = __builtin_amdgcn_readlane(st, src);
+      found = true;
+    }
+    carry += __builtin_amdgcn_readlane(incl, 63);
+  }
+  return found;
+}
+
+constexpr int kDegBins = 18;
+
+struct ShareTab {
+  int32_t shst[kShareCap + 1];
+  int32_t cb[kMaxHops + 1];
+  int32_t vwin[256];
+  int chunk_s[4];
+};
+
+__device__ __forceinline__ int fast_div(int x, int d, float rd) {
+  int q = (int)((float)x * rd);
+  if (q * d > x) --q;
+  if ((q + 1) * d <= x) ++q;
+  return q;
+}
+
+__device__ __forceinline__ void resolve_chain(const PlanParams& p, int j, bool write_nsub, bool flag_bad, int lane,
+                                              ShareTab& T, unsigned long long* st) {
+  int gg = 0, w_lo = 0;
+  {
+    const int half = p.n_ions == 2 ? (p.nwg >> 1 > 0 ? p.nwg >> 1 : 1) : p.nwg;
+    const int jp = xcd_slot(j, p.nwg);
+    gg = (p.n_ions == 2 && jp >= half) ? 1 : 0;
+    const int jj = jp - (gg ? half : 0);
+    const int nw = gg ? (p.nwg - half > 0 ? p.nwg - half : 1) : half;
+    w_lo = (int)((float)jj * (float)p.B / (float)nw) - 64;
+    w_lo = w_lo < 0 ? 0 : w_lo;
+    w_lo &= ~15;
+  }
+  int vw[4];
+  {
+    const int32_t* vrg = p.vr + (int64_t)gg * p.B;
+#pragma unroll
+    for (int i = 0; i < 4; ++i) {
+      const int m = w_lo + 64 * i + lane;
+      vw[i] = vrg[m < p.B ? m : p.B - 1];
+    }
+  }
+  int g = 0, k0 = 0, bp0 = 0, t_lo = 0, t_hi = 0;
+  bool bad = false;
+  const bool have = resolve_share(p, j, lane, g, k0, bp0, t_lo, t_hi, bad, st);
+  CSTAMP(11);
+#pragma unroll
+  for (int i = 0; i < 4; ++i) T.vwin[64 * i + lane] = vw[i];
+  if (!have) {
+    if (lane == 0) {
+      T.chunk_s[0] = -1; T.chunk_s[1] = 0; T.chunk_s[2] = 0; T.chunk_s[3] = bad ? 1 : 0;
+      if (write_nsub) p.nsub[j] = 0;
+      if (bad && flag_bad) p.header->overflow = 1;
+    }
+    return;
+  }
+  const int32_t* vrg = p.vr + (int64_t)g * p.B;
+  int run = bp0;
+  int first = -1, nsh = 0;
+  int end_row = -1;
+  __builtin_amdgcn_s_waitcnt(0xc07f);
+  auto vr_at = [&](int mbase) {
+    const int rel = mbase - w_lo;
+    if (g == gg && rel >= 0 && rel + 64 <= 256) return T.vwin[rel + lane];
+    const int m = mbase + lane;
+    return vrg[m < p.B ? m : p.B - 1];
+  };
+  int v_n1 = vr_at(k0 * kPB);
+  for (int mbase = k0 * kPB; mbase < p.B && end_row < 0; mbase += 64) {
+    const int m = mbase + lane;
+    const int v = v_n1;
+    v_n1 = vr_at(mbase + 64);
+    const int vv = m < p.B ? v : 0;
+    const int incl = wave_incl_scan(vv);
+    const int st = run + incl - vv;
+    const bool in = m < p.B && st >= t_lo && st < t_hi;
+    const unsigned long long inb = __ballot(in);
+    if (inb) {
+      if (first < 0) first = mbase + __builtin_ctzll(inb);
+      const int pos = nsh + __builtin_popcountll(inb & ((1ull << lane) - 1));
+      if (in && pos < kShareCap) T.shst[pos] = st;
+      nsh += __builtin_popcountll(inb);
+    }
+    const unsigned long long ge = __ballot(m < p.B && st >= t_hi);
+    if (ge) end_row = __builtin_amdgcn_readlane(st, __builtin_ctzll(ge));
+    run += __builtin_amdgcn_readlane(incl, 63);
+  }
+  if (end_row < 0) end_row = run;
+  if (nsh > kShareCap) {
+    if (lane == 0) p.header->overflow = 1;
+    nsh = kShareCap;
+  }
+  if (lane == 0) T.shst[nsh] = end_row;
+  __builtin_amdgcn_s_waitcnt(0xc07f);
+  CSTAMP(12);
+  int mb = 0, hop = 0;
+  if (nsh < 64) {
+    const int st_l = T.shst[lane <= nsh ? lane : nsh];
+    while (mb < nsh && hop < kMaxHops) {
+      const int lim = __builtin_amdgcn_readlane(st_l, mb) + kRCap;
+      const unsigned long long okb = __ballot(lane > mb && lane <= nsh && st_l <= lim);
+      if (lane == 0) T.cb[hop] = mb;
+      ++hop;
+      mb = okb ? 63 - __builtin_clzll(okb) : mb + 1;
+    }
+  }
+  while (mb < nsh && hop < kMaxHops) {
+    const int lim = T.shst[mb] + kRCap;
+    int e = mb + 1;
+    for (int c0 = mb + 1; c0 <= nsh; c0 += 64) {
+      const int cidx = c0 + lane;
+      const bool ok = cidx <= nsh && T.shst[cidx <= nsh ? cidx : nsh] <= lim;
+      const unsigned long long okb = __ballot(ok);
+      if (okb == 0) break;
+      e = c0 + 63 - __builtin_clzll(okb);
+      if (okb != ~0ull) break;
+    }
+    if (lane == 0) T.cb[hop] = mb;
+    ++hop;
+    mb = e;
+  }
+  if (lane == 0) {
+    T.cb[hop] = nsh;
+    T.chunk_s[0] = first;
+    T.chunk_s[1] = hop;
+    T.chunk_s[2] = g;
+    T.chunk_s[3] = 0;
+    if (write_nsub) p.nsub[j] = hop;
+  }
+}
+
+constexpr int kTick = 16;
+struct PlanTabs {
+  int32_t moloff[kRCap + 2], molrows[kRCap], cnt[kRCap + 64], place[kRCap];
+  int32_t idl[kRCap];
+  __attribute__((aligned(16))) int32_t dbins[kRCap];
+  int32_t dstart[kRCap], dcur[kRCap];
+  __attribute__((aligned(16))) int32_t thist[kTVbMax + 64];
+  int32_t tgb[kTVbMax], tcur[kTVbMax + 64];
+  __attribute__((aligned(16))) int32_t jdp[kRCap + 4];
+  int32_t misc[4];
+  __attribute__((aligned(16))) uint16_t tick[kRCap * kTick];
+  uint2 elist[kTECapBig];
+};
+static_assert(sizeof(PlanTabs) % 16 == 0, "the group table follows the tables in the encoder's overlay");
+constexpr int kPlanChunkBarriers = 7;
+
+__device__ __forceinline__ void plan_chunk_typed(const PlanParams& p, int j, int sl, bool have, int tid, PlanTabs& L,
+                                                 uint4* grp, ShareTab& T, unsigned long long* st) {
+  if (!have) {
+#pragma unroll
+    for (int i = 0; i < kPlanChunkBarriers; ++i) lds_barrier();
+    return;
+  }
+  auto& moloff = L.moloff; auto& molrows = L.molrows; auto& cnt = L.cnt; auto& place = L.place; auto& idl = L.idl;
+  auto& dbins = L.dbins; auto& dstart = L.dstart; auto& dcur = L.dcur; auto& thist = L.thist; auto& tgb = L.tgb;
+  auto& tcur = L.tcur; auto& jdp = L.jdp; auto& misc = L.misc; auto& tick = L.tick; auto& elist = L.elist;
+  const int lane = tid & 63, wave = tid >> 6;
+  const int first_mol = T.chunk_s[0], g = T.chunk_s[2];
+  const int N = p.N, E = p.E;
+  const float rE = 1.0f / (float)E;
+  {
+  const int mb_local = T.cb[sl], M = T.cb[sl + 1] - mb_local, m0 = first_mol + mb_local;
+  const int base = T.shst[mb_local];
+  const int R = T.shst[mb_local + M] - base;
+  const int idx = j * p.max_sub + sl;
+  const int32_t* ids_g = p.atom_ids[g];
+  const int32_t* conn_g = p.conn[g];
+  const int32_t* bond_g = p.bond_ids[g];
+  const int32_t* rows_g = p.rows + (int64_t)g * p.B;
+  unsigned char* rec = p.rec + (size_t)idx * kTRecBytes;
+  uint32_t* r_slist = p.slist + (size_t)idx * p.ecap;
+  uint16_t* r_rowdeg = reinterpret_cast<uint16_t*>(rec + kTRecRowdeg);
+  unsigned char* r_tilemax = rec + kTRecTilemax;
+  uint16_t* r_moloff = reinterpret_cast<uint16_t*>(rec + kTRecMoloff);
+  uint16_t* r_molrows = reinterpret_cast<uint16_t*>(rec + kTRecMolrows);
+  uint16_t* r_poolrow = reinterpret_cast<uint16_t*>(rec + kTRecPoolrow);
+  int32_t* r_rowatom = reinterpret_cast<int32_t*>(rec + kTRecRowatom);
+  uint16_t* r_jd = reinterpret_cast<uint16_t*>(rec + kTRecJdptr);
+  uint16_t* r_cw = reinterpret_cast<uint16_t*>(rec + kTRecCounts);
+
+  const int n_slots = M * E;
+  constexpr int kSC = 6;
+  int sbid[kSC];
+  int2 sst[kSC];
+  const int32_t* conn_c = conn_g + (int64_t)m0 * E * 2;
+  const int32_t* bond_c = bond_g + (int64_t)m0 * E;
+#pragma unroll
+  for (int k = 0; k < kSC; ++k) {
+    const int slot = tid + k * kRCap;
+    sbid[k] = -1; sst[k] = make_int2(0, 0);
+    if (slot < n_slots) {
+      sst[k] = *reinterpret_cast<const int2*>(conn_c + 2 * (int64_t)slot);
+      sbid[k] = bond_c[slot];
+    }
+  }
+  constexpr int kIC = 3;
+  const int n_ids = M * N;
+  const float rN = 1.0f / (float)N;
+  const int32_t* ids_c = ids_g + (int64_t)m0 * N;
+  int sid[kIC];
+#pragma unroll
+  for (int k = 0; k < kIC; ++k) {
+    const int slot = tid + k * kRCap;
+    sid[k] = slot < n_ids ? ids_c[slot] : 0;
+  }
+  for (int m = tid; m <= M; m += kRCap) {
+    const int off = T.shst[mb_local + m] - base;
+    moloff[m] = off;
+    r_moloff[m] = (uint16_t)off;
+    if (m < M) {
+      const int rr = rows_g[m0 + m];
+      molrows[m] = rr;
+      r_molrows[m] = (uint16_t)rr;
+    }
+  }
+  cnt[tid] = 0;
+  dbins[tid] = 0;
+  dcur[tid] = 0;
+  thist[tid] = 0;
+  tcur[tid] = 0;
+  idl[tid] = -1;
+  if (tid == 0) misc[1] = 0;
+  {
+    const uint4 ones = make_uint4(~0u, ~0u, ~0u, ~0u);
+    reinterpret_cast<uint4*>(tick)[2 * tid] = ones;
+    reinterpret_cast<uint4*>(tick)[2 * tid + 1] = ones;
+  }
+  lds_barrier();
+  CSTAMP(2);
+
+  auto put_id = [&](int slot, int id) {
+    const int m = fast_div(slot, N, rN), n = slot - m * N;
+    if (slot < n_ids && n < molrows[m]) idl[moloff[m] + n] = id;
+  };
+  {
+    const int dq = fast_div(kRCap, N, rN), dr = kRCap - dq * N;
+    int cm = fast_div(tid, N, rN), cn = tid - cm * N;
+    int mr[kIC], mo[kIC], nn[kIC];
+#pragma unroll
+    for (int k = 0; k < kIC; ++k) {
+      const int mm = tid + k * kRCap < n_ids ? cm : 0;
+      mr[k] = tid + k * kRCap < n_ids ? molrows[mm] : 0;
+      mo[k] = moloff[mm];
+      nn[k] = cn;
+      cn += dr; cm += dq;
+      if (cn >= N) { cn -= N; ++cm; }
+    }
+#pragma unroll
+    for (int k = 0; k < kIC; ++k)
+      if (nn[k] < mr[k]) idl[mo[k] + nn[k]] = sid[k];
+  }
+  for (int slot = tid + kIC * kRCap; slot < n_ids; slot += kRCap) put_id(slot, ids_c[slot]);
+  {
+    unsigned okm = 0u;
+#pragma unroll
+    for (int k = 0; k < kSC; ++k) okm |= edge_valid(sst[k].x, sst[k].y, sbid[k], N, p.Vb) ? 1u << k : 0u;
+    const int mine = __builtin_popcount(okm);
+    const int incl = wave_incl_scan(mine);
+    int pos = 0;
+    if (lane == 63) pos = atomicAdd(&misc[1], incl);
+    pos = __builtin_amdgcn_readlane(pos, 63) + incl - mine;
+    const int dq = fast_div(kRCap, E, rE), dr = kRCap - dq * E;
+    int cm = fast_div(tid, E, rE), ce = tid - cm * E;
+#pragma unroll
+    for (int k0 = 0; k0 < kSC; k0 += 3) {
+      int row[3], srw[3], tk[3], es[3];
+#pragma unroll
+      for (int k = 0; k < 3; ++k) {
+        const bool ok = (okm >> (k0 + k)) & 1u;
+        const int m = cm;
+        es[k] = ce;
+        ce += dr; cm += dq;
+        if (ce >= E) { ce -= E; ++cm; }
+        const int mo = moloff[m < M ? m : 0];
+        row[k] = mo + (ok ? sst[k0 + k].y : 0);
+        srw[k] = mo + (ok ? sst[k0 + k].x : 0);
+      }
+#pragma unroll
+      for (int k = 0; k < 3; ++k) {
+        const bool ok = (okm >> (k0 + k)) & 1u;
+        tk[k] = atomicAdd(&cnt[ok ? row[k] : kRCap + lane], 1);
+        atomicAdd(&thist[ok ? sbid[k0 + k] : kTVbMax + lane], 1);
+      }
+#pragma unroll
+      for (int k = 0; k < 3; ++k) {
+        const bool ok = (okm >> (k0 + k)) & 1u;
+        if (ok && tk[k] < kTick) tick[row[k] * kTick + tk[k]] = (uint16_t)es[k];
+        if (ok) {
+          if (pos < kTECapBig)
+            elist[pos] = make_uint2((uint32_t)row[k] | ((uint32_t)srw[k] << 8) | ((uint32_t)sbid[k0 + k] << 16), (uint32_t)es[k]);
+          ++pos;
+        }
+      }
+    }
+  }
+  for (int s0 = kSC * kRCap; s0 < n_slots; s0 += kRCap) {
+    const int slot = s0 + tid;
+    int2 st = make_int2(0, 0);
+    int bid = -1;
+    if (slot < n_slots) {
+      st = *reinterpret_cast<const int2*>(conn_c + 2 * (int64_t)slot);
+      bid = bond_c[slot];
+    }
+    const bool ok = edge_valid(st.x, st.y, bid, N, p.Vb);
+    const int m = fast_div(slot, E, rE), e = slot - m * E;
+    const int mo = moloff[m < M ? m : 0];
+    const int row = mo + (ok ? st.y : 0);
+    int tk = kTick;
+    if (ok) {
+      tk = atomicAdd(&cnt[row], 1);
+      atomicAdd(&thist[bid], 1);
+    }
+    const unsigned long long okb = __ballot(ok);
+    int pos0 = 0;
+    if (okb != 0ull) {
+      if (lane == (int)__builtin_ctzll(okb)) pos0 = atomicAdd(&misc[1], (int)__builtin_popcountll(okb));
+      pos0 = __builtin_amdgcn_readlane(pos0, (int)__builtin_ctzll(okb));
+    }
+    if (tk < kTick) tick[row * kTick + tk] = (uint16_t)e;
+    const int pos = pos0 + (int)__builtin_popcountll(okb & ((1ull << lane) - 1));
+    if (ok && pos < kTECapBig)
+      elist[pos] = make_uint2((uint32_t)row | ((uint32_t)(mo + st.x) << 8) | ((uint32_t)bid << 16), (uint32_t)e);
+  }
+  lds_barrier();
+  CSTAMP(3);
+
+  const int my_deg = cnt[tid];
+  const int dcl = my_deg > 255 ? 255 : my_deg;
+  if (tid < R) {
+    if (my_deg > 255) {
+      p.header->overflow = 1;
+      T.chunk_s[3] = 1;
+    }
+    atomicAdd(&dbins[255 - dcl], 1);
+  }
+  lds_barrier();
+  CSTAMP(4);
+
+  if (wave == 0) {
+    const int4 h = reinterpret_cast<const int4*>(dbins)[lane];
+    const int s4 = h.x + h.y + h.z + h.w;
+    const int ex = wave_incl_scan(s4) - s4;
+    reinterpret_cast<int4*>(dstart)[lane] = make_int4(ex, ex + h.x, ex + h.x + h.y, ex + h.x + h.y + h.z);
+    __builtin_amdgcn_s_waitcnt(0xc07f);
+    const int4 s = reinterpret_cast<const int4*>(dstart)[63 - lane];
+    const int t4 = s.x + s.y + s.z + s.w;
+    const int incl = wave_incl_scan(t4);
+    const int jx = incl - t4;
+    reinterpret_cast<int4*>(jdp)[lane] = make_int4(jx, jx + s.w, jx + s.w + s.z, jx + s.w + s.z + s.y);
+    if (lane == 63) { jdp[kRCap] = incl; jdp[kRCap + 1] = incl; }
+  } else if (wave == 1) {
+    const int4 n = reinterpret_cast<const int4*>(thist)[lane];
+    const int4 ng = make_int4((n.x + 3) >> 2, (n.y + 3) >> 2, (n.z + 3) >> 2, (n.w + 3) >> 2);
+    const int s4 = ng.x + ng.y + ng.z + ng.w;
+    const int incl = wave_incl_scan(s4);
+    const int ex = incl - s4;
+    reinterpret_cast<int4*>(tgb)[lane] = make_int4(ex, ex + ng.x, ex + ng.x + ng.y, ex + ng.x + ng.y + ng.z);
+    const int ngrp_all = __builtin_amdgcn_readlane(incl, 63);
+    int gmax = (ngrp_all + kTRunTarget - 1) / kTRunTarget;
+    gmax = gmax < 2 ? 2 : gmax;
+    const float rgm = 1.0f / (float)gmax;
+    const int4 nr = make_int4(fast_div(ng.x + gmax - 1, gmax, rgm), fast_div(ng.y + gmax - 1, gmax, rgm),
+                              fast_div(ng.z + gmax - 1, gmax, rgm), fast_div(ng.w + gmax - 1, gmax, rgm));
+    const int r4 = nr.x + nr.y + nr.z + nr.w;
+    const int rincl = wave_incl_scan(r4);
+    int ri = rincl - r4;
+    uint16_t* runs = reinterpret_cast<uint16_t*>(rec + trec_runs_off(p.Vb, p.ecap));
+    for (int i = 0; i < nr.x; ++i) runs[ri++] = (uint16_t)(ex + i * gmax);
+    for (int i = 0; i < nr.y; ++i) runs[ri++] = (uint16_t)(ex + ng.x + i * gmax);
+    for (int i = 0; i < nr.z; ++i) runs[ri++] = (uint16_t)(ex + ng.x + ng.y + i * gmax);
+    for (int i = 0; i < nr.w; ++i) runs[ri++] = (uint16_t)(ex + ng.x + ng.y + ng.z + i * gmax);
+    if (lane == 63) {
+      runs[rincl] = (uint16_t)incl;
+      *reinterpret_cast<uint16_t*>(rec + kTRecNrun) = (uint16_t)rincl;
+      misc[0] = incl;
+    }
+  }
+  lds_barrier();
+  CSTAMP(5);
+
+  int pos = tid;
+  if (tid < R) pos = dstart[255 - dcl] + atomicAdd(&dcur[255 - dcl], 1);
+  place[tid] = pos;
+  {
+    const int my_id = idl[tid];
+    r_rowatom[pos] = my_id;
+    r_poolrow[tid] = (uint16_t)(pos | (my_id > 0 ? 0x8000 : 0));
+    r_rowdeg[pos] = (uint16_t)my_deg;
+    if ((pos & 15) == 0) r_tilemax[pos >> 4] = (unsigned char)dcl;
+    r_jd[tid] = (uint16_t)jdp[tid];
+    if (tid < 2) r_jd[kRCap + tid] = (uint16_t)jdp[kRCap];
+    if (pos == 0) {
+      r_cw[0] = (uint16_t)misc[0];
+      r_cw[1] = (uint16_t)jdp[kRCap];
+      r_cw[2] = (uint16_t)dcl;
+    }
+    if (tid == 0)
+      reinterpret_cast<int4*>(p.desc)[idx] = make_int4(m0, M, jdp[kRCap] < p.ecap ? jdp[kRCap] : p.ecap, R | (g << 16));
+  }
+  {
+    const int n_t = thist[tid];
+    const int ng = (n_t + 3) >> 2, gb = tgb[tid];
+    const uint32_t dump = (uint32_t)tmsg_key(p.ecap) * 0x10001u;
+    for (int jg = 0; jg < ng; ++jg) {
+      const int c = n_t - 4 * jg;
+      grp[gb + jg] = make_uint4((uint32_t)tid | ((uint32_t)(c < 4 ? c : 4) << 8) | ((uint32_t)(ng - jg) << 24), 0u, dump, dump);
+    }
+  }
+  lds_barrier();
+  CSTAMP(6);
+
+  {
+    auto below = [](uint4 a, uint32_t ue) {
+      return (int)(((a.x & 0xffffu) < ue) + ((a.x >> 16) < ue) + ((a.y & 0xffffu) < ue) + ((a.y >> 16) < ue) +
+                   ((a.z & 0xffffu) < ue) + ((a.z >> 16) < ue) + ((a.w & 0xffffu) < ue) + ((a.w >> 16) < ue));
+    };
+    const int nval = misc[1] < kTECapBig ? misc[1] : kTECapBig;
+    for (int i0 = 0; i0 < nval; i0 += 2 * kRCap) {
+      bool ok[2];
+      uint2 en[2];
+      int row[2], srow[2], deg[2], ix[2], gb[2], rank[2];
+      uint4 ta[2], tb[2];
+#pragma unroll
+      for (int k = 0; k < 2; ++k) {
+        const int i = i0 + k * kRCap + tid;
+        ok[k] = i < nval;
+        en[k] = elist[ok[k] ? i : 0];
+      }
+#pragma unroll
+      for (int k = 0; k < 2; ++k) {
+        const int rt = (int)(en[k].x & 0xffu), bid = (int)(en[k].x >> 16);
+        deg[k] = cnt[rt];
+        ta[k] = reinterpret_cast<const uint4*>(tick)[2 * rt];
+        tb[k] = reinterpret_cast<const uint4*>(tick)[2 * rt + 1];
+        row[k] = place[rt];
+        srow[k] = place[(en[k].x >> 8) & 0xffu];
+        gb[k] = tgb[bid];
+        ix[k] = atomicAdd(&tcur[ok[k] ? bid : kTVbMax + lane], 1);
+      }
+#pragma unroll
+      for (int k = 0; k < 2; ++k) {
+        rank[k] = below(ta[k], en[k].y) + below(tb[k], en[k].y);
+        if (deg[k] > kTick) {
+          const int rt = (int)(en[k].x & 0xffu);
+          int lo = 0, hi = M - 1;
+          while (lo < hi) {
+            const int mid = (lo + hi + 1) >> 1;
+            if (moloff[mid] <= rt) lo = mid; else hi = mid - 1;
+          }
+          const int t = rt - moloff[lo];
+          const int32_t* cm = conn_c + 2 * (int64_t)lo * E;
+          const int32_t* bm = bond_c + (int64_t)lo * E;
+          rank[k] = 0;
+          for (int e2 = 0; e2 < (int)en[k].y; ++e2) {
+            const int2 s2 = *reinterpret_cast<const int2*>(cm + 2 * e2);
+            rank[k] += (s2.y == t && edge_valid(s2.x, s2.y, bm[e2], N, p.Vb)) ? 1 : 0;
+          }
+        }
+        rank[k] = jdp[rank[k] < 256 ? rank[k] : 255];
+      }
+#pragma unroll
+      for (int k = 0; k < 2; ++k) {
+        if (ok[k]) {
+          unsigned char* ge = reinterpret_cast<unsigned char*>(&grp[gb[k] + (ix[k] >> 2)]);
+          ge[4 + (ix[k] & 3)] = (unsigned char)srow[k];
+          reinterpret_cast<uint16_t*>(ge + 8)[ix[k] & 3] = (uint16_t)tmsg_key(rank[k] + row[k]);
+          if (rank[k] + row[k] < p.ecap)
+            r_slist[rank[k] + row[k]] = tsrc_word((int)(en[k].x >> 16), idl[(en[k].x >> 8) & 0xffu]);
+        }
+      }
+    }
+  }
+  lds_barrier();
+  CSTAMP(9);
+
+  {
+    const int ngrp = misc[0];
+    uint4* r_grp = reinterpret_cast<uint4*>(rec + kTRecGrp);
+    for (int i = tid; i < ngrp; i += kRCap) r_grp[i] = grp[i];
+  }
+  CSTAMP(15);
+  lds_barrier();
+  }
+}
+
+}
+}
+}
diff --git a/ionic_mpnn_amd/csrc/encoder_typed.hip b/ionic_mpnn_amd/csrc/encoder_typed.hip
--- a/ionic_mpnn_amd/csrc/encoder_typed.hip
+++ b/ionic_mpnn_amd/csrc/encoder_typed.hip
@@ -1,5 +1,6 @@
 #include "encoder_device.h"
 #include "encoder_layout.h"
+#include "encoder_plan_device.h"
 #include "kernel_device.h"
 
 namespace impnn {
@@ -18,6 +19,12 @@
 static_assert(lds_fixed_bytes(true, kTVbMax, kTECap) <= 160 * 1024 && lds_fixed_bytes(false, kTVbMax, kTECapBig) <= 160 * 1024 &&
                   lds_fixed_bytes(true, kTVbMax, kTECapBig, kTHSBig3) <= 160 * 1024,
               "LDS budget");
+
+constexpr int kPlanSubs = kThreads / kRCap;
+constexpr int kPlanShareBytes = (int)((sizeof(ShareTab) + 15) & ~(size_t)15);
+constexpr int plan_set_bytes(int Vb, int ecap) { return (int)sizeof(PlanTabs) + 16 * tgrp_cap(Vb, ecap); }
+constexpr size_t plan_lds_bytes(int Vb, int ecap) { return (size_t)kPlanShareBytes + (size_t)kPlanSubs * plan_set_bytes(Vb, ecap); }
+static_assert(plan_lds_bytes(kTVbMax, kTECapBig) <= 160 * 1024, "LDS budget of the plan preamble");
 
 typedef bf16x8_t bf16x8;
 struct B3 {
@@ -183,7 +190,7 @@
 }
 
 template <bool STAMPS, bool X3, int HS = kTHS>
-__global__ __launch_bounds__(kThreads, kThreads / 256) void encoder_typed_kernel(TEncParams p) {
+__global__ __launch_bounds__(kThreads, kThreads / 256) void encoder_typed_kernel(TEncParams p, PlanParams pp) {
   extern __shared__ __align__(16) float smem[];
   constexpr int kUpdLds = X3 ? kXUpdLds : kTUpdLds, kUpdSlot = X3 ? kXUpdSlot : kTUpdSlot;
   constexpr int kNPf = X3 ? 3 : 2;
@@ -212,19 +219,47 @@
   unsigned long long* stamp = STAMPS && p.stamps ? p.stamps + (size_t)blockIdx.x * 32 : nullptr;
   if (stamp && tid == 0) stamp[0] = __builtin_amdgcn_s_memtime();
 
-  {
+  auto poison = [&]() {
+    const float nan = __builtin_nanf("");
+    for (int g = 0; g < p.n_ions; ++g)
+      for (int64_t t = (int64_t)blockIdx.x * kThreads + tid; t < (int64_t)p.B * kD; t += (int64_t)gridDim.x * kThreads)
+        p.pooled[g][t] = nan;
+  };
+  if (!p.plan_here) {
     const PlanHeader hd = *p.header;
     if (hd.magic != kPlanMagic || hd.kind != 1 || hd.nwg != (int)gridDim.x || hd.max_sub != p.max_sub ||
         hd.B != p.B || hd.n_ions != p.n_ions || hd.overflow != 0) {
-      const float nan = __builtin_nanf("");
-      for (int g = 0; g < p.n_ions; ++g)
-        for (int64_t t = (int64_t)blockIdx.x * kThreads + tid; t < (int64_t)p.B * kD; t += (int64_t)gridDim.x * kThreads)
-          p.pooled[g][t] = nan;
+      poison();
       return;
     }
   }
+  int nchunks;
+  if (p.plan_here) {
+    char* const sb = reinterpret_cast<char*>(smem);
+    ShareTab& T = *reinterpret_cast<ShareTab*>(sb);
+    const int sub = wave >> 2, set_bytes = plan_set_bytes(p.Vb, p.ecap);
+    PlanTabs& L = *reinterpret_cast<PlanTabs*>(sb + kPlanShareBytes + sub * set_bytes);
+    uint4* const grp = reinterpret_cast<uint4*>(sb + kPlanShareBytes + sub * set_bytes + sizeof(PlanTabs));
+    __builtin_amdgcn_s_setprio(3);
+    if (wave == 0) resolve_chain(pp, (int)blockIdx.x, true, true, lane, T, nullptr);
+    lds_barrier();
+    nchunks = __builtin_amdgcn_readfirstlane(T.chunk_s[1]);
+    for (int sl0 = 0; sl0 < nchunks; sl0 += kPlanSubs)
+      plan_chunk_typed(pp, (int)blockIdx.x, sl0 + sub, sl0 + sub < nchunks, tid & (kRCap - 1), L, grp, T, nullptr);
+    const int bad = __builtin_amdgcn_readfirstlane(T.chunk_s[3]);
+    __builtin_amdgcn_s_setprio(0);
+    asm volatile("s_waitcnt vmcnt(0) lgkmcnt(0)\n\ts_barrier" ::: "memory");
+    if (stamp && tid == 0) stamp[6] = __builtin_amdgcn_s_memtime();
+    if (bad) {
+      if (tid == 0) pp.header->overflow = 1;
+      poison();
+      return;
+    }
+  } else {
+    nchunks = __builtin_amdgcn_readfirstlane(p.nsub[blockIdx.x]);
+  }
   const int c_begin = blockIdx.x * p.max_sub;
-  const int c_end = c_begin + __builtin_amdgcn_readfirstlane(p.nsub[blockIdx.x]);
+  const int c_end = c_begin + nchunks;
   if (c_begin >= c_end) return;
 
   if (p.atab_lds)
@@ -737,7 +772,7 @@
   return check_launch("typed_m0");
 }
 
-int launch_encoder_typed_run(const EncoderArgs& a, const enc::Ws& w, hipStream_t s) {
+int launch_encoder_typed_run(const EncoderArgs& a, const enc::Ws& w, hipStream_t s, const enc::PlanParams* plan) {
   using namespace enc;
   char* base = static_cast<char*>(a.workspace);
   TEncParams ep{};
@@ -777,7 +812,13 @@
   ep.ecap = tecap_of(a.E);
   ep.rec_lds = trec_lds_bytes(a.Vb, ep.ecap);
   const bool big3 = x3 && ep.ecap == kTECapBig;
-  void (*kern)(TEncParams) =
+  ep.plan_here = plan ? 1 : 0;
+  PlanParams pp{};
+  if (plan) {
+    pp = *plan;
+    pp.stamps = nullptr;
+  }
+  void (*kern)(TEncParams, PlanParams) =
       big3 ? (ep.stamps ? encoder_typed_kernel<true, true, kTHSBig3> : encoder_typed_kernel<false, true, kTHSBig3>)
       : x3 ? (ep.stamps ? encoder_typed_kernel<true, true> : encoder_typed_kernel<false, true>)
            : (ep.stamps ? encoder_typed_kernel<true, false> : encoder_typed_kernel<false, false>);
@@ -786,8 +827,9 @@
   const size_t atab_bytes = ((size_t)a.Va + 1) * kTAS * sizeof(float);
   ep.atab_lds = lds + atab_bytes <= 160 * 1024;
   if (ep.atab_lds) lds += atab_bytes;
+  if (plan && plan_lds_bytes(a.Vb, ep.ecap) > lds) lds = plan_lds_bytes(a.Vb, ep.ecap);
   profile_record_start(s);
-  kern<<<w.nwg, kThreads, lds, s>>>(ep);
+  kern<<<w.nwg, kThreads, lds, s>>>(ep, pp);
   profile_record_stop(s);
   return check_launch("encoder_typed");
 }
```

Result: no change. 39.50 million (-0.2%).
